# yl4579/StyleTTS2

Measured on AMD Instinct MI355X. Metric: audio-seconds/sec (RTF^-1) end-to-end, 10 s utterance batch, higher is better.
Workload: dtype f32 (convs/linears: f16 hi/lo split, 3 MFMA products, fp32 accumulate)

## Files before the change

include/st2.h:

```cpp
#ifndef ST2_H
#define ST2_H

#include <stdint.h>

#ifdef __cplusplus
extern "C" {
#endif

#define ST2_ABI_VERSION 23

int st2_abi_version(void);
const char* st2_last_error(void);
int st2_device_info(int dev, char* name, int cap);

#define ST2_STATUS_F16_RANGE 1
#define ST2_STATUS_LSTM_TIMEOUT 2
#define ST2_STATUS_DURATION_SUM 4
#define ST2_STATUS_LSTM_RECOVERED 8
int st2_status(int clear);

enum st2_prologue {
  ST2_PRO_NONE = 0,
  ST2_PRO_LEAKY = 1,
  ST2_PRO_ADAIN_LEAKY = 2,
// ... 168 lines not shown
                    int32_t B, int32_t C, int32_t N, void* stream);
int st2_mean_tokens_len(const float* x, int64_t x_bs, int32_t x_cs, float* m, int64_t m_bs,
                        int32_t B, int32_t C, int32_t N, const int32_t* len, void* stream);
int st2_time_features(float t, const float* w, int32_t H2, int32_t B, float* out, void* stream);
int st2_tokens_to_channels(const float* e, int64_t e_bs, int32_t B, int32_t N, int32_t E, float* y, int64_t y_bs,
                           int32_t y_cs, void* stream);
int st2_broadcast_cols(const float* x, int64_t x_bs, float* y, int64_t y_bs, int32_t y_cs, int32_t B, int32_t C,
                       int32_t N, void* stream);
int st2_copy_ncl(const float* x, int64_t x_bs, int32_t x_cs, float* y, int64_t y_bs, int32_t y_cs, int32_t B, int32_t C,
                 int32_t L, void* stream);

int st2_embed_tokens(const int64_t* tokens, int32_t B, int32_t N, const float* table, int32_t V, int32_t E,
                     const float* add, const float* pos, const int32_t* len, float* y, int64_t y_bs, int32_t y_cs,
                     void* stream);
int st2_mask_tail(float* x, int64_t x_bs, int32_t x_cs, int32_t B, int32_t C, int32_t L, const int32_t* len, void* stream);

int st2_duration_head(const float* x, int64_t x_bs, int32_t x_cs, const float* w, const float* bias, int32_t B,
                      int32_t K, int32_t J, int32_t N, const int32_t* len, int32_t tail, int64_t* dur, float* dsum,
                      void* stream);
int st2_expand_by_durations(const float* x, int64_t x_bs, int32_t x_cs, const int64_t* dur, int32_t B, int32_t C,
                            int32_t N, int32_t T, int32_t shift, float* y, int64_t y_bs, int32_t y_cs, void* stream);
int st2_expand_by_durations_len(const float* x, int64_t x_bs, int32_t x_cs, const int64_t* dur, int32_t B, int32_t C,
                                int32_t N, int32_t T, int32_t shift, float* y, int64_t y_bs, int32_t y_cs, const int32_t* len,
                                void* stream);

int st2_stft_frames(const float* wave, int64_t w_bs, int32_t B, int32_t L, int32_t n_win, int32_t hop, int32_t shift,
                    float* frames, int64_t f_bs, int32_t f_cs, void* stream);
int st2_power_spectrum(const float* y, int64_t y_bs, int32_t y_cs, int32_t B, int32_t K, int32_t M, float* p,
                       int64_t p_bs, int32_t p_cs, void* stream);
int st2_log_norm(float* x, int64_t n, float eps, float mean, float stdv, void* stream);
int st2_dwconv3x3s2(const float* x, int64_t x_bs, int64_t x_hs, int32_t x_cs, const float* w, const float* bias,
                    int32_t B, int32_t C, int32_t H, int32_t W, float* y, int64_t y_bs, int64_t y_hs, int32_t y_cs,
                    void* stream);
int st2_avgpool2x2(const float* x, int64_t x_bs, int64_t x_hs, int32_t x_cs, int32_t B, int32_t C, int32_t H, int32_t W,
                   float* y, int64_t y_bs, int64_t y_hs, int32_t y_cs, void* stream);

int st2_axpbypcz(const float* x, float a, const float* y, float b, const float* z, float c,
                 float* out, int64_t n, void* stream);

typedef struct st2_engine st2_engine;

typedef struct st2_model_config {
  int32_t decoder_kind;
  int32_t dim_in;
  int32_t style_dim;
  int32_t upsample_initial_channel;
  int32_t n_upsamples;  int32_t upsample_rates[4];  int32_t upsample_kernel_sizes[4];
  int32_t n_resblock_kernels;  int32_t resblock_kernel_sizes[4];  int32_t resblock_dilations[4][3];
  int32_t gen_istft_n_fft, gen_istft_hop;
  int32_t multispeaker;
  int32_t dn_layers, dn_heads, dn_head_features, dn_multiplier;
  int32_t dn_channels;
  int32_t dn_embedding;
  int32_t dn_context_features;
  int32_t dn_max_length;
  int32_t pred_hidden;
  int32_t bert_layers;
  float bert_ln_eps;
} st2_model_config;

int st2_create(const st2_model_config* cfg, st2_engine** out);
int st2_destroy(st2_engine* e);
int st2_load_weights(st2_engine* e, const char* name, const float* data, const int64_t* shape, int32_t ndim);
int st2_finalize_weights(st2_engine* e, int32_t which);

typedef struct st2_decoder_taps {
  float* encode;
  float* front;
  float* har_source;
  float* har;
  float* stage[4];
  float* spec_phase;
} st2_decoder_taps;

int64_t st2_decoder_workspace_bytes(st2_engine* e, int32_t B, int32_t T);
int st2_decoder_forward(st2_engine* e, const float* asr, const float* f0, const float* n, const float* s,
                        const float* sine_noise, const float* har_inject, int32_t B, int32_t T, float* wave,
                        void* workspace, int64_t workspace_bytes, const st2_decoder_taps* taps, void* stream);
int st2_decoder_forward_ragged(st2_engine* e, const float* asr, const float* f0, const float* n, const float* s,
                               const float* sine_noise, const float* har_inject, const int32_t* frames, int32_t B,
                               int32_t T_max, float* wave, void* workspace, int64_t workspace_bytes,
                               const st2_decoder_taps* taps, void* stream);

#define ST2_SAMPLER_TABLE_COLS 11
int st2_sampler_table(int32_t steps, double sigma_min, double sigma_max, double rho, double sigma_data, double* table,
                      double* sigma0);
int64_t st2_sampler_workspace_bytes(st2_engine* e, int32_t B, int32_t N, int32_t steps, double embedding_scale);
int st2_sampler_run(st2_engine* e, const float* noise, const float* embedding, const float* features,
                    const float* step_noise, const int32_t* lengths, int32_t B, int32_t N, int32_t steps,
                    double embedding_scale, const double* table, double sigma0, float* out, void* workspace,
                    int64_t workspace_bytes, float* step_taps, void* stream);

int64_t st2_prosody_workspace_bytes(st2_engine* e, int32_t B, int32_t N, int32_t T);
int st2_prosody_forward(st2_engine* e, const float* d_cm, const float* t_en, const int64_t* durations, const float* s,
                        int32_t B, int32_t N, int32_t T, int32_t shift, float* asr, float* f0, float* n, void* workspace,
                        int64_t workspace_bytes, void* stream);
int st2_prosody_forward_ragged(st2_engine* e, const float* d_cm, const float* t_en, const int64_t* durations,
                               const float* s, const int32_t* frames, int32_t B, int32_t N, int32_t T_max, int32_t shift,
                               float* asr, float* f0, float* n, void* workspace, int64_t workspace_bytes, void* stream);

int64_t st2_text_workspace_bytes(st2_engine* e, int32_t B, int32_t N);
int st2_text_forward(st2_engine* e, const int64_t* tokens, const int32_t* lengths, int32_t B, int32_t N, float* t_en,
                     void* workspace, int64_t workspace_bytes, void* stream);

int64_t st2_duration_workspace_bytes(st2_engine* e, int32_t B, int32_t N);
int st2_duration_forward(st2_engine* e, const float* d_en, const float* s, const int32_t* lengths, int32_t B, int32_t N,
                         int32_t tail, float* d_cm, int64_t* durations, void* workspace, int64_t workspace_bytes,
                         void* stream);

int64_t st2_bert_workspace_bytes(st2_engine* e, int32_t B, int32_t N);
int st2_bert_forward(st2_engine* e, const int64_t* tokens, const int32_t* lengths, int32_t B, int32_t N, float* hidden_cm,
                     void* workspace, int64_t workspace_bytes, void* stream);

typedef struct st2_front_args {
  const int64_t* tokens;
  const int32_t* lengths;
  const float* noise;
  const float* step_noise;
  const float* ref_s;
  const float* s_prev;
  int32_t B, N, steps;
  int32_t tail;
  double embedding_scale;
  const double* table;
  double sigma0;
  double alpha, beta, t;
  float* t_en;
  float* d_cm;
  float* s;
  float* ref;
  float* s_pred_out;
  int64_t* durations;
  int32_t carry;
} st2_front_args;
int st2_sizeof_front_args(void);
int64_t st2_front_workspace_bytes(st2_engine* e, const st2_front_args* a);
int st2_front_forward(st2_engine* e, const st2_front_args* a, void* workspace, int64_t workspace_bytes, void* stream);

int64_t st2_style_workspace_bytes(st2_engine* e, int32_t which, int32_t B, int32_t n_mels, int32_t T);
int st2_style_forward(st2_engine* e, int32_t which, const float* mel, int32_t B, int32_t n_mels, int32_t T, float* style,
                      void* workspace, int64_t workspace_bytes, void* stream);

int st2_conv_timing(int enable);
int st2_conv_timing_read(double* rows, int32_t cap_rows);

int st2_conv_tune(int mode);
int st2_conv_tune_set(int32_t ks, int32_t C_in, int32_t C_out, int32_t L_out, int32_t B, int32_t variant);
int st2_conv_tune_read(double* rows, int32_t cap_rows);

#define ST2_HEADROOM_COLS 12
int st2_debug_headroom(int enable);
int st2_debug_headroom_read(double* rows, int32_t cap_rows);

#define ST2_CALIBRATION_COLS 5
int st2_calibrate(st2_engine* e, int32_t margin_bits, int32_t* n_clamped);
int st2_calibration_read(st2_engine* e, double* rows, int32_t cap_rows);
int st2_calibration_site_name(st2_engine* e, int32_t site, char* name, int32_t cap);
int st2_calibration_write(st2_engine* e, const float* scales, int32_t n);
float st2_calibration_scale(float max_abs, int32_t margin_bits);

int st2_probe_box(char* json, int32_t cap, int32_t level);

int st2_probe_cu_health(char* json, int32_t cap, uint32_t* mask_out, int32_t mask_words, int32_t* n_excluded);

int st2_probe_mfma_stream(int32_t kind, int32_t workgroups, int32_t iters, void* stream);

int st2_stream_create_cu_mask(const uint32_t* mask, int32_t n_words, void** stream);
int st2_stream_destroy(void* stream);

enum st2_backend_slot {
  ST2_BE_CONV1D_F16S = 0, ST2_BE_CONV1D_XS, ST2_BE_ACT_SPLIT, ST2_BE_STATS_FINALIZE, ST2_BE_CONV1D_DIRECT,
  ST2_BE_PHASE_SPLIT, ST2_BE_INSTNORM_STATS, ST2_BE_COLNORM_STATS, ST2_BE_STYLE_FC, ST2_BE_CONVT_INTERLEAVE_STATS,
  ST2_BE_ADAIN_LEAKY_POOL, ST2_BE_HAR_SOURCE, ST2_BE_STFT_MAG_PHASE, ST2_BE_ISTFT, ST2_BE_ATTENTION_KEYLEN,
  ST2_BE_ADD_CHANVEC, ST2_BE_MEAN_TOKENS_LEN, ST2_BE_AXPBYPCZ, ST2_BE_TIME_FEATURES, ST2_BE_TOKENS_TO_CHANNELS,
  ST2_BE_BROADCAST_COLS, ST2_BE_COPY_NCL, ST2_BE_EXPAND_BY_DURATIONS,
  ST2_BE_LSTM_BIDIR,
  ST2_BE_COLNORM_APPLY, ST2_BE_DURATION_HEAD, ST2_BE_MASK_TAIL, ST2_BE_EMBED_TOKENS, ST2_BE_DWCONV3X3S2, ST2_BE_AVGPOOL2X2,
  ST2_BE_DEV_ALLOC,
  ST2_BE_DEV_FREE,
  ST2_BE_UPLOAD,
  ST2_BACKEND_ENTRIES_V22,
  ST2_BE_ACT_SPLIT_LEN = ST2_BACKEND_ENTRIES_V22, ST2_BE_INSTNORM_STATS_LEN, ST2_BE_STATS_FINALIZE_LEN,
  ST2_BE_CONV1D_DIRECT_LEN, ST2_BE_ADAIN_LEAKY_POOL_LEN, ST2_BE_CONVT_INTERLEAVE_STATS_LEN, ST2_BE_HAR_SOURCE_LEN,
  ST2_BE_STFT_MAG_PHASE_LEN, ST2_BE_ISTFT_LEN, ST2_BE_RAGGED_LENGTHS, ST2_BE_EXPAND_BY_DURATIONS_LEN,
  ST2_BACKEND_ENTRIES
};
int st2_debug_set_backend(void* const* table, int32_t entries);

#ifdef __cplusplus
}
#endif
#endif
```

styletts2_amd/_lib.py:

```python
import ctypes as C
import os

import torch

_HERE = os.path.dirname(os.path.abspath(__file__))
LIB_PATH = os.path.join(_HERE, "libst2_hip.so")
ABI_VERSION = 23
HEADROOM_COLS, CALIBRATION_COLS = 12, 5

f32p = C.c_void_p

PRO_NONE, PRO_LEAKY, PRO_ADAIN_LEAKY, PRO_ADAIN_SNAKE, PRO_SNAKE, PRO_COLNORM = range(6)
STATUS_F16_RANGE, STATUS_LSTM_TIMEOUT, STATUS_DURATION_SUM, STATUS_LSTM_RECOVERED = 1, 2, 4, 8
ACT_NONE, ACT_GELU, ACT_EXP_SIN, ACT_TANH, ACT_LEAKY, ACT_GELU_TANH = range(6)


class ConvDesc(C.Structure):
    _fields_ = [
        ("B", C.c_int32), ("C_in", C.c_int32), ("C_out", C.c_int32), ("L_in", C.c_int32),
        ("L_out", C.c_int32), ("ks", C.c_int32), ("dil", C.c_int32), ("pad_left", C.c_int32),
        ("x", f32p), ("x_bs", C.c_int64), ("x_cs", C.c_int32),
        ("wt", f32p), ("w_ld", C.c_int32),
        ("bias", f32p),
        ("y", f32p), ("y_bs", C.c_int64), ("y_cs", C.c_int32),
# ... 60 lines not shown
                        "adain_leaky_pool_len", "convt_interleave_stats_len", "har_source_len", "stft_mag_phase_len",
                        "istft_len", "ragged_lengths", "expand_by_durations_len"]

_SIGNATURES = {
    "st2_abi_version": (C.c_int, []),
    "st2_last_error": (C.c_char_p, []),
    "st2_device_info": (C.c_int, [C.c_int, C.c_char_p, C.c_int]),
    "st2_sizeof_conv_desc": (C.c_int, []),
    "st2_status": (C.c_int, [C.c_int]),
    "st2_conv1d": (C.c_int, [C.POINTER(ConvDesc), C.c_void_p]),
    "st2_conv1d_f16s": (C.c_int, [C.POINTER(ConvDesc), C.c_void_p]),
    "st2_conv1d_f16s_splitk_bytes": (C.c_int64, [C.POINTER(ConvDesc)]),
    "st2_conv1d_f16s_chunk": (C.c_int, [C.c_int]),
    "st2_conv1d_f16s_co_block": (C.c_int, [C.c_int]),
    "st2_conv1d_f16s_set_variant": (None, [C.c_int]),
    "st2_conv1d_xs": (C.c_int, [C.POINTER(ConvDesc), C.c_void_p]),
    "st2_act_split": (C.c_int, [f32p, C.c_int64, C.c_int32, C.c_int32, C.c_int32, C.c_int32, C.c_int32, C.c_float,
                                f32p, f32p, f32p, C.c_int64, C.c_int32, C.c_int32, f32p, C.c_float, f32p, C.c_int32,
                                C.c_int32, C.c_int32, C.c_void_p]),
    "st2_stats_finalize": (C.c_int, [f32p, C.c_int32, C.c_int32, C.c_int32, C.c_float, f32p, C.c_int32, C.c_void_p]),
    "st2_conv1d_direct": (C.c_int, [f32p, C.c_int64, C.c_int32, f32p, f32p, f32p, C.c_int64, C.c_int32,
                                    C.c_int32, C.c_int32, C.c_int32, C.c_int32, C.c_int32, C.c_int32, C.c_int32,
                                    C.c_int32, C.c_void_p]),
    "st2_phase_split": (C.c_int, [f32p, C.c_int64, C.c_int32, C.c_int32, C.c_int32, C.c_int32, C.c_int32, C.c_int32,
                                  f32p, C.c_int64, C.c_int32, C.c_int32, C.c_void_p]),
    "st2_instnorm_stats": (C.c_int, [f32p, C.c_int64, C.c_int32, C.c_int32, C.c_int32, C.c_int32, C.c_float, f32p,
                                     C.c_void_p]),
    "st2_colnorm_stats": (C.c_int, [f32p, C.c_int64, C.c_int32, C.c_int32, C.c_int32, C.c_int32, C.c_float, f32p,
                                    C.c_void_p]),
    "st2_style_fc": (C.c_int, [f32p, C.c_int32, C.c_int32, f32p, f32p, C.c_int32, C.c_int32, f32p, C.c_void_p]),
    "st2_convt_interleave": (C.c_int, [f32p, C.c_int64, C.c_int32, C.c_int32, f32p, f32p, C.c_int64, C.c_int32,
                                       f32p, C.c_int64, C.c_int32, C.c_int32, C.c_int32, C.c_int32, C.c_int32,
                                       C.c_int32, C.c_int32, C.c_void_p]),
    "st2_convt_interleave_stats": (C.c_int, [f32p, C.c_int64, C.c_int32, C.c_int32, f32p, f32p, C.c_int64, C.c_int32,
                                             f32p, C.c_int64, C.c_int32, C.c_int32, C.c_int32, C.c_int32, C.c_int32,
                                             C.c_int32, C.c_int32, f32p, C.c_int32, C.c_void_p]),
    "st2_adain_leaky_pool": (C.c_int, [f32p, C.c_int64, C.c_int32, f32p, f32p, f32p, C.c_int64, C.c_float, f32p,
                                       f32p, f32p, C.c_int64, C.c_int32, C.c_int32, C.c_int32, C.c_int32,
                                       C.c_void_p]),
    "st2_har_source": (C.c_int, [f32p, C.c_int32, C.c_int32, C.c_int32, C.c_int32, f32p, f32p, f32p, C.c_float,
                                 C.c_float, C.c_float, C.c_float, f32p, f32p, C.c_void_p]),
    "st2_stft_mag_phase": (C.c_int, [f32p, C.c_int32, C.c_int32, C.c_int32, C.c_int32, f32p, C.c_int64, C.c_int32,
                                     C.c_void_p]),
    "st2_istft": (C.c_int, [f32p, C.c_int64, C.c_int32, C.c_int32, C.c_int32, C.c_int32, C.c_int32, f32p, C.c_int64,
                            C.c_void_p]),
    "st2_attention": (C.c_int, [f32p, f32p, f32p, C.c_int64, C.c_int32, f32p, C.c_int64, C.c_int32, C.c_int32,
                                C.c_int32, C.c_int32, C.c_int32, C.c_float, C.c_void_p]),
    "st2_attention_keylen": (C.c_int, [f32p, f32p, f32p, C.c_int64, C.c_int32, f32p, C.c_int64, C.c_int32, C.c_int32,
                                       C.c_int32, C.c_int32, C.c_int32, C.c_float, C.c_void_p, C.c_void_p]),
    "st2_colnorm_apply": (C.c_int, [f32p, C.c_int64, C.c_int32, f32p, f32p, f32p, C.c_int64, C.c_int32, C.c_int32,
                                    C.c_float, C.c_void_p, f32p, C.c_int64, C.c_int32, C.c_int32, C.c_int32, C.c_int32,
                                    C.c_void_p]),
    "st2_lstm_bidir": (C.c_int, [f32p, C.c_int64, C.c_int32, f32p, C.c_void_p, C.c_int32, C.c_int32, C.c_int32, f32p,
                                 C.c_int64, C.c_int32, C.c_void_p]),
    "st2_lstm_coop_scratch_bytes": (C.c_int64, [C.c_int32]),
    "st2_lstm_coop_set_exchange": (C.c_int, [C.c_int]),
    "st2_lstm_coop_set_spin_limit": (C.c_int, [C.c_int]),
    "st2_lstm_coop_set_block": (C.c_int, [C.c_int]),
    "st2_lstm_bidir_coop": (C.c_int, [f32p, C.c_int64, C.c_int32, f32p, C.c_void_p, C.c_int32, C.c_int32, C.c_int32,
                                      f32p, C.c_int64, C.c_int32, C.c_void_p, C.c_int64, C.c_void_p]),
    "st2_lstm_bidir_coop_recovering": (C.c_int, [f32p, C.c_int64, C.c_int32, f32p, C.c_void_p, C.c_int32, C.c_int32, C.c_int32,
                                                 f32p, C.c_int64, C.c_int32, C.c_void_p, C.c_int64, C.c_void_p]),
    "st2_add_chanvec": (C.c_int, [f32p, C.c_int64, C.c_int32, f32p, C.c_int64, f32p, C.c_int64, C.c_int32,
                                  C.c_int32, C.c_int32, C.c_int32, C.c_void_p]),
    "st2_mean_tokens": (C.c_int, [f32p, C.c_int64, C.c_int32, f32p, C.c_int64, C.c_int32, C.c_int32, C.c_int32,
                                  C.c_void_p]),
    "st2_mean_tokens_len": (C.c_int, [f32p, C.c_int64, C.c_int32, f32p, C.c_int64, C.c_int32, C.c_int32, C.c_int32,
                                      C.c_void_p, C.c_void_p]),
    "st2_time_features": (C.c_int, [C.c_float, f32p, C.c_int32, C.c_int32, f32p, C.c_void_p]),
    "st2_tokens_to_channels": (C.c_int, [f32p, C.c_int64, C.c_int32, C.c_int32, C.c_int32, f32p, C.c_int64, C.c_int32,
                                         C.c_void_p]),
    "st2_broadcast_cols": (C.c_int, [f32p, C.c_int64, f32p, C.c_int64, C.c_int32, C.c_int32, C.c_int32, C.c_int32,
                                     C.c_void_p]),
    "st2_copy_ncl": (C.c_int, [f32p, C.c_int64, C.c_int32, f32p, C.c_int64, C.c_int32, C.c_int32, C.c_int32, C.c_int32,
                               C.c_void_p]),
    "st2_duration_head": (C.c_int, [f32p, C.c_int64, C.c_int32, f32p, f32p, C.c_int32, C.c_int32, C.c_int32, C.c_int32,
                                    C.c_void_p, C.c_int32, C.c_void_p, f32p, C.c_void_p]),
    "st2_expand_by_durations": (C.c_int, [f32p, C.c_int64, C.c_int32, C.c_void_p, C.c_int32, C.c_int32, C.c_int32,
                                          C.c_int32, C.c_int32, f32p, C.c_int64, C.c_int32, C.c_void_p]),
    "st2_create": (C.c_int, [C.POINTER(ModelConfig), C.POINTER(C.c_void_p)]),
    "st2_destroy": (C.c_int, [C.c_void_p]),
    "st2_load_weights": (C.c_int, [C.c_void_p, C.c_char_p, C.c_void_p, C.POINTER(C.c_int64), C.c_int32]),
    "st2_finalize_weights": (C.c_int, [C.c_void_p, C.c_int32]),
    "st2_decoder_workspace_bytes": (C.c_int64, [C.c_void_p, C.c_int32, C.c_int32]),
    "st2_decoder_forward": (C.c_int, [C.c_void_p, f32p, f32p, f32p, f32p, f32p, f32p, C.c_int32, C.c_int32, f32p,
                                      C.c_void_p, C.c_int64, C.POINTER(DecoderTaps), C.c_void_p]),
    "st2_embed_tokens": (C.c_int, [C.c_void_p, C.c_int32, C.c_int32, f32p, C.c_int32, C.c_int32, f32p, f32p, C.c_void_p, f32p,
                                   C.c_int64, C.c_int32, C.c_void_p]),
    "st2_bert_workspace_bytes": (C.c_int64, [C.c_void_p, C.c_int32, C.c_int32]),
    "st2_bert_forward": (C.c_int, [C.c_void_p, C.c_void_p, C.c_void_p, C.c_int32, C.c_int32, f32p, C.c_void_p, C.c_int64,
                                   C.c_void_p]),
    "st2_style_workspace_bytes": (C.c_int64, [C.c_void_p, C.c_int32, C.c_int32, C.c_int32, C.c_int32]),
    "st2_style_forward": (C.c_int, [C.c_void_p, C.c_int32, f32p, C.c_int32, C.c_int32, C.c_int32, f32p, C.c_void_p, C.c_int64,
                                    C.c_void_p]),
    "st2_sizeof_front_args": (C.c_int, []),
    "st2_front_workspace_bytes": (C.c_int64, [C.c_void_p, C.POINTER(FrontArgs)]),
    "st2_front_forward": (C.c_int, [C.c_void_p, C.POINTER(FrontArgs), C.c_void_p, C.c_int64, C.c_void_p]),
    "st2_text_workspace_bytes": (C.c_int64, [C.c_void_p, C.c_int32, C.c_int32]),
    "st2_text_forward": (C.c_int, [C.c_void_p, C.c_void_p, C.c_void_p, C.c_int32, C.c_int32, f32p, C.c_void_p, C.c_int64,
                                   C.c_void_p]),
    "st2_mask_tail": (C.c_int, [f32p, C.c_int64, C.c_int32, C.c_int32, C.c_int32, C.c_int32, C.c_void_p, C.c_void_p]),
    "st2_duration_workspace_bytes": (C.c_int64, [C.c_void_p, C.c_int32, C.c_int32]),
    "st2_duration_forward": (C.c_int, [C.c_void_p, f32p, f32p, C.c_void_p, C.c_int32, C.c_int32, C.c_int32, f32p,
                                       C.c_void_p, C.c_void_p, C.c_int64, C.c_void_p]),
    "st2_decoder_forward_ragged": (C.c_int, [C.c_void_p, f32p, f32p, f32p, f32p, f32p, f32p, C.c_void_p, C.c_int32,
                                             C.c_int32, f32p, C.c_void_p, C.c_int64, C.c_void_p, C.c_void_p]),
    "st2_prosody_forward_ragged": (C.c_int, [C.c_void_p, f32p, f32p, C.c_void_p, f32p, C.c_void_p, C.c_int32, C.c_int32,
                                             C.c_int32, C.c_int32, f32p, f32p, f32p, C.c_void_p, C.c_int64, C.c_void_p]),
    "st2_act_split_len": (C.c_int, [f32p, C.c_int64, C.c_int32, C.c_int32, C.c_int32, C.c_int32, C.c_int32, C.c_float,
                                    f32p, f32p, f32p, C.c_int64, C.c_int32, C.c_int32, f32p, C.c_float, f32p, C.c_int32,
                                    C.c_int32, C.c_int32, C.c_void_p, C.c_void_p]),
    "st2_stats_finalize_len": (C.c_int, [f32p, C.c_int32, C.c_int32, C.c_int32, C.c_float, f32p, C.c_int32, C.c_void_p,
                                         C.c_int32, C.c_void_p]),
    "st2_instnorm_stats_len": (C.c_int, [f32p, C.c_int64, C.c_int32, C.c_int32, C.c_int32, C.c_int32, C.c_float, f32p,
                                         C.c_void_p, C.c_void_p]),
    "st2_conv1d_direct_len": (C.c_int, [f32p, C.c_int64, C.c_int32, f32p, f32p, f32p, C.c_int64, C.c_int32, C.c_int32,
                                        C.c_int32, C.c_int32, C.c_int32, C.c_int32, C.c_int32, C.c_int32, C.c_int32,
                                        C.c_void_p, C.c_void_p, C.c_void_p]),
    "st2_convt_interleave_stats_len": (C.c_int, [f32p, C.c_int64, C.c_int32, C.c_int32, f32p, f32p, C.c_int64, C.c_int32,
                                                 f32p, C.c_int64, C.c_int32, C.c_int32, C.c_int32, C.c_int32, C.c_int32,
                                                 C.c_int32, C.c_int32, f32p, C.c_int32, C.c_void_p, C.c_void_p,
                                                 C.c_void_p]),
    "st2_adain_leaky_pool_len": (C.c_int, [f32p, C.c_int64, C.c_int32, f32p, f32p, f32p, C.c_int64, C.c_float, f32p,
                                           f32p, f32p, C.c_int64, C.c_int32, C.c_int32, C.c_int32, C.c_int32, C.c_void_p,
                                           C.c_void_p]),
    "st2_har_source_len": (C.c_int, [f32p, C.c_int32, C.c_int32, C.c_int32, C.c_int32, f32p, f32p, f32p, C.c_float,
                                     C.c_float, C.c_float, C.c_float, f32p, f32p, C.c_void_p, C.c_void_p]),
    "st2_stft_mag_phase_len": (C.c_int, [f32p, C.c_int32, C.c_int32, C.c_int32, C.c_int32, f32p, C.c_int64, C.c_int32,
                                         C.c_void_p, C.c_void_p]),
    "st2_istft_len": (C.c_int, [f32p, C.c_int64, C.c_int32, C.c_int32, C.c_int32, C.c_int32, C.c_int32, f32p, C.c_int64,
                                C.c_void_p, C.c_void_p]),
    "st2_expand_by_durations_len": (C.c_int, [f32p, C.c_int64, C.c_int32, C.c_void_p, C.c_int32, C.c_int32, C.c_int32,
                                              C.c_int32, C.c_int32, f32p, C.c_int64, C.c_int32, C.c_void_p, C.c_void_p]),
    "st2_ragged_lengths": (C.c_int, [C.c_void_p, C.c_int32, C.c_int32, C.c_int32, C.POINTER(C.c_int32), C.c_void_p,
                                     C.c_void_p]),
    "st2_prosody_workspace_bytes": (C.c_int64, [C.c_void_p, C.c_int32, C.c_int32, C.c_int32]),
    "st2_prosody_forward": (C.c_int, [C.c_void_p, f32p, f32p, C.c_void_p, f32p, C.c_int32, C.c_int32, C.c_int32, C.c_int32,
                                      f32p, f32p, f32p, C.c_void_p, C.c_int64, C.c_void_p]),
    "st2_sampler_table": (C.c_int, [C.c_int32, C.c_double, C.c_double, C.c_double, C.c_double, C.POINTER(C.c_double),
                                    C.POINTER(C.c_double)]),
    "st2_sampler_workspace_bytes": (C.c_int64, [C.c_void_p, C.c_int32, C.c_int32, C.c_int32, C.c_double]),
    "st2_sampler_run": (C.c_int, [C.c_void_p, f32p, f32p, f32p, f32p, C.c_void_p, C.c_int32, C.c_int32, C.c_int32,
                                  C.c_double, C.POINTER(C.c_double), C.c_double, f32p, C.c_void_p, C.c_int64, f32p,
                                  C.c_void_p]),
    "st2_conv_timing": (C.c_int, [C.c_int]),
    "st2_conv_timing_read": (C.c_int, [C.POINTER(C.c_double), C.c_int32]),
    "st2_conv_tune": (C.c_int, [C.c_int]),
    "st2_conv_tune_set": (C.c_int, [C.c_int32, C.c_int32, C.c_int32, C.c_int32, C.c_int32, C.c_int32]),
    "st2_conv_tune_read": (C.c_int, [C.POINTER(C.c_double), C.c_int32]),
    "st2_probe_box": (C.c_int, [C.c_char_p, C.c_int32, C.c_int32]),
    "st2_probe_cu_health": (C.c_int, [C.c_char_p, C.c_int32, C.POINTER(C.c_uint32), C.c_int32, C.POINTER(C.c_int32)]),
    "st2_probe_mfma_stream": (C.c_int, [C.c_int32, C.c_int32, C.c_int32, C.c_void_p]),
    "st2_debug_headroom": (C.c_int, [C.c_int]),
    "st2_debug_headroom_read": (C.c_int, [C.POINTER(C.c_double), C.c_int32]),
    "st2_conv1d_xs_part_cols": (C.c_int, [C.POINTER(ConvDesc)]),
    "st2_conv1d_f16s_set_splitk": (None, [C.c_int, C.c_int]),
    "st2_calibrate": (C.c_int, [C.c_void_p, C.c_int32, C.POINTER(C.c_int32)]),
    "st2_calibration_read": (C.c_int, [C.c_void_p, C.POINTER(C.c_double), C.c_int32]),
    "st2_calibration_site_name": (C.c_int, [C.c_void_p, C.c_int32, C.c_char_p, C.c_int32]),
    "st2_calibration_write": (C.c_int, [C.c_void_p, C.POINTER(C.c_float), C.c_int32]),
    "st2_calibration_scale": (C.c_float, [C.c_float, C.c_int32]),
    "st2_stream_create_cu_mask": (C.c_int, [C.POINTER(C.c_uint32), C.c_int32, C.POINTER(C.c_void_p)]),
    "st2_stream_destroy": (C.c_int, [C.c_void_p]),
    "st2_debug_set_backend": (C.c_int, [C.POINTER(C.c_void_p), C.c_int32]),
    "st2_stft_frames": (C.c_int, [f32p, C.c_int64, C.c_int32, C.c_int32, C.c_int32, C.c_int32, C.c_int32, f32p,
                                  C.c_int64, C.c_int32, C.c_void_p]),
    "st2_power_spectrum": (C.c_int, [f32p, C.c_int64, C.c_int32, C.c_int32, C.c_int32, C.c_int32, f32p, C.c_int64,
                                     C.c_int32, C.c_void_p]),
    "st2_log_norm": (C.c_int, [f32p, C.c_int64, C.c_float, C.c_float, C.c_float, C.c_void_p]),
    "st2_dwconv3x3s2": (C.c_int, [f32p, C.c_int64, C.c_int64, C.c_int32, f32p, f32p, C.c_int32, C.c_int32, C.c_int32,
                                  C.c_int32, f32p, C.c_int64, C.c_int64, C.c_int32, C.c_void_p]),
    "st2_avgpool2x2": (C.c_int, [f32p, C.c_int64, C.c_int64, C.c_int32, C.c_int32, C.c_int32, C.c_int32, C.c_int32, f32p,
                                 C.c_int64, C.c_int64, C.c_int32, C.c_void_p]),
    "st2_axpbypcz": (C.c_int, [f32p, C.c_float, f32p, C.c_float, f32p, C.c_float, f32p, C.c_int64, C.c_void_p]),
}

EXPORTS = tuple(_SIGNATURES)
_lib = None


class St2Error(RuntimeError):
    pass


def load():
    global _lib
    if _lib is not None:
        return _lib
    if not os.path.exists(LIB_PATH):
        raise St2Error("libst2_hip.so is not built (%s missing). Run `python -m styletts2_amd._build`; "
                       "there is no CPU fallback." % LIB_PATH)
    try:
        lib = C.CDLL(LIB_PATH)
    except OSError as e:
        raise St2Error("cannot load %s: %s" % (LIB_PATH, e)) from e
    for name, (res, args) in _SIGNATURES.items():
        try:
            fn = getattr(lib, name)
        except AttributeError as e:
            raise St2Error("libst2_hip.so does not export %s" % name) from e
        fn.restype = res
        fn.argtypes = args
    if lib.st2_abi_version() != ABI_VERSION:
        raise St2Error("ABI mismatch: library %d, binding %d" % (lib.st2_abi_version(), ABI_VERSION))
    if lib.st2_sizeof_conv_desc() != C.sizeof(ConvDesc):
        raise St2Error("st2_conv_desc layout mismatch: library %d B, binding %d B"
                       % (lib.st2_sizeof_conv_desc(), C.sizeof(ConvDesc)))
    if lib.st2_sizeof_front_args() != C.sizeof(FrontArgs):
        raise St2Error("st2_front_args layout mismatch: library %d B, binding %d B"
                       % (lib.st2_sizeof_front_args(), C.sizeof(FrontArgs)))
    _lib = lib
    return lib


def check(status, what):
    if status != 0:
        msg = load().st2_last_error()
        raise St2Error("%s failed: %s" % (what, msg.decode() if msg else "unknown error"))
```

styletts2_amd/csrc/st2_actsplit.hip:

```cpp
#include "st2_common.h"
#include "st2_act.h"
#include <algorithm>
#include <cstring>
#include <type_traits>
#include <vector>

namespace {

struct ActArgs {
  const float* x; int64_t x_bs; int x_cs;
  int C, L;
  float slope;
  const float* stats; const float* gamma; const float* beta; int64_t gb_bs; int gb_seg; int gamma_plus_one;
  const float* alpha;
  float x_scale;
  st2_h8* xs; int xs_cg, Lp, halo;
  const int32_t* len;
  int* status;
};

#ifndef ST2_ACT_NT
#define ST2_ACT_NT 3
#endif
template <int PRO>
__global__ __launch_bounds__(256) void act_split_kernel(const ActArgs a) {
  const int pos = blockIdx.x * 256 + threadIdx.x;
  if (pos >= a.Lp) return;
  const int cg = blockIdx.y;
  const int b = blockIdx.z;
  const int l = pos - a.halo;
  const int Lb = a.len ? min(a.len[b], a.L) : a.L;
  const bool lok = l >= 0 && l < Lb;
  const int lc = min(max(l, 0), a.L - 1);
  const float* xb = a.x + (int64_t)b * a.x_bs + lc;
  float v[8];
#pragma unroll
  for (int e = 0; e < 8; ++e) {
    const int ci = min(cg * 8 + e, a.C - 1);
#if ST2_ACT_NT & 1
    v[e] = __builtin_nontemporal_load(&xb[(int64_t)ci * a.x_cs]);
#else
    v[e] = xb[(int64_t)ci * a.x_cs];
#endif
  }
  float cmean = 0.f, crstd = 1.f;
  if constexpr (PRO == ST2_PRO_COLNORM) {
    const float* st = a.stats + ((int64_t)b * a.L + lc) * 2;
    cmean = st[0];
    crstd = st[1];
  }
  st2_h8 hi, lo;
  bool sat = false;
#pragma unroll
  for (int e = 0; e < 8; ++e) {
    const int ci = cg * 8 + e;
    const int cc = min(ci, a.C - 1);
    float u = v[e];
    if constexpr (PRO == ST2_PRO_LEAKY) {
      u = leaky(u, a.slope);
    } else if constexpr (PRO == ST2_PRO_ADAIN_LEAKY || PRO == ST2_PRO_ADAIN_SNAKE) {
      const float* st = a.stats + ((int64_t)b * a.C + cc) * 2;
      const float g = 1.0f + a.gamma[(int64_t)b * a.gb_bs + cc];
      const float bt = a.beta[(int64_t)b * a.gb_bs + cc];
      float w = (u - st[0]) * st[1];
      w = g * w + bt;
      if constexpr (PRO == ST2_PRO_ADAIN_LEAKY) {
        u = leaky(w, a.slope);
      } else {
        const float al = a.alpha[cc];
        u = snake(w, al, 1.0f / al);
      }
    } else if constexpr (PRO == ST2_PRO_SNAKE) {
      const float al = a.alpha[cc];
      u = snake(u, al, 1.0f / al);
    } else if constexpr (PRO == ST2_PRO_COLNORM) {
      const int64_t row = a.gb_seg > 0 ? (int64_t)(lc / a.gb_seg) : (int64_t)b;
      const float g0 = a.gamma[row * a.gb_bs + cc];
      const float g = a.gamma_plus_one ? 1.0f + g0 : g0;
      const float bt = a.beta[row * a.gb_bs + cc];
      const float w = (u - cmean) * crstd;
      u = w * g + bt;
    }
    u = (lok && ci < a.C) ? u * a.x_scale : 0.f;
    const float uc = st2_clamp_f16(u);
    sat |= uc != u;
    const _Float16 h = (_Float16)uc;
    hi[e] = h;
    lo[e] = (_Float16)(uc - (float)h);
  }
  if (__any(sat) && (threadIdx.x & 63) == 0) st2_raise_status(a.status, ST2_STATUS_F16_RANGE);
  const int64_t plane = (int64_t)a.xs_cg * a.Lp;
  st2_h8* dst = a.xs + ((int64_t)b * 2 * a.xs_cg + cg) * a.Lp + pos;
#if ST2_ACT_NT & 2
  __builtin_nontemporal_store(hi, &dst[0]);
  __builtin_nontemporal_store(lo, &dst[plane]);
#else
  dst[0] = hi;
  dst[plane] = lo;
#endif
}

__global__ __launch_bounds__(256) void stats_finalize_kernel(const float* __restrict__ part, int rows, int nt, int L_max,
                                                             float eps, float* __restrict__ stats, int cols,
                                                             const int32_t* __restrict__ len, int len_div) {
  const int lane = threadIdx.x & 63;
  const int row = blockIdx.x * 4 + (threadIdx.x >> 6);
  if (row >= rows) return;
  const int L = len ? min(max(len[row / len_div], 1), L_max) : L_max;
  const float2* p = reinterpret_cast<const float2*>(part) + (int64_t)row * nt;
  const float* sh = part + (int64_t)rows * nt * 2 + (int64_t)row * nt;
  const int ns = min(nt, (L + cols - 1) / cols);
  double wsum = 0.0;
  for (int i = lane; i < ns; i += 64) {
    const int n = min(cols, L - i * cols);
    wsum += (double)n * (double)sh[i] + (double)p[i].x;
  }
  wsum = st2_wave_sum(wsum);
  const double mean = __shfl(wsum, 0, 64) / (double)L;
  double m2 = 0.0;
  for (int i = lane; i < ns; i += 64) {
    const int n = min(cols, L - i * cols);
    const double s1 = (double)p[i].x, s2 = (double)p[i].y;
    const double mi = (double)sh[i] + s1 / (double)n;
    m2 += (s2 - s1 * s1 / (double)n) + (double)n * (mi - mean) * (mi - mean);
  }
  m2 = st2_wave_sum(m2);
  if (lane == 0) {
    double var = m2 / (double)L;
    if (var < 0.0) var = 0.0;
    stats[(int64_t)row * 2 + 0] = (float)mean;
    stats[(int64_t)row * 2 + 1] = (float)(1.0 / sqrt(var + (double)eps));
  }
}

struct HeadroomSums {
  unsigned max_bits, pad;
  double su2, se2, ssub;
};
__global__ __launch_bounds__(256) void xs_probe_kernel(const st2_h8* __restrict__ xs, int64_t slots_per_item, int64_t item_stride,
                                                       HeadroomSums* out) {
  const st2_h8* hi_p = xs + (int64_t)blockIdx.y * item_stride;
  const st2_h8* lo_p = hi_p + slots_per_item;
  float m = 0.f;
  double su2 = 0.0, se2 = 0.0, ssub = 0.0;
  for (int64_t i = (int64_t)blockIdx.x * 256 + threadIdx.x; i < slots_per_item; i += (int64_t)gridDim.x * 256) {
    const st2_h8 h = hi_p[i], l = lo_p[i];
#pragma unroll
    for (int e = 0; e < 8; ++e) {
      const float hf = (float)h[e], lf = (float)l[e];
      m = fmaxf(m, fabsf(hf));
      if (hf == 0.f && lf == 0.f) continue;
      const float u = hf + lf;
      const float al = fabsf(lf);
      const bool sub = al < 6.103515625e-05f;
      int ex = -14;
      if (!sub) {
        (void)frexpf(al, &ex);
        ex -= 1;
      }
      const float ulp = ldexpf(1.0f, ex - 10);
      su2 += (double)u * u;
      se2 += (double)ulp * ulp * (1.0 / 12.0);
      if (sub) ssub += (double)u * u;
    }
  }
  for (int off = 32; off > 0; off >>= 1) m = fmaxf(m, __shfl_down(m, off, 64));
  su2 = st2_wave_sum(su2);
  se2 = st2_wave_sum(se2);
  ssub = st2_wave_sum(ssub);
  if ((threadIdx.x & 63) == 0) {
    atomicMax(&out->max_bits, __float_as_uint(m));
    atomicAdd(&out->su2, su2);
    atomicAdd(&out->se2, se2);
    atomicAdd(&out->ssub, ssub);
  }
}

struct HeadroomRecord {
  int kind, pro, B, C, L;
  float x_scale;
  const void* engine;
  int site;
};
bool g_headroom = false;
std::vector<HeadroomRecord> g_hr;
HeadroomSums* g_hr_dev = nullptr;
constexpr int HR_CAP = 4096;
void* g_hr_scratch = nullptr;
size_t g_hr_scratch_bytes = 0;
thread_local const void* t_site_engine = nullptr;
thread_local int t_site = -1;

void headroom_record(int kind, const ActArgs& a, int B, hipStream_t s) {
  if ((int)g_hr.size() >= HR_CAP || !g_hr_dev) return;
  hipStreamCaptureStatus cs = hipStreamCaptureStatusNone;
  if (hipStreamIsCapturing(s, &cs) != hipSuccess || cs != hipStreamCaptureStatusNone) {
    (void)hipGetLastError();
    return;
  }
  const int64_t plane = (int64_t)a.xs_cg * a.Lp;
  hipLaunchKernelGGL(xs_probe_kernel, dim3((unsigned)std::min<int64_t>((plane + 255) / 256, 1024), B), dim3(256), 0, s, a.xs, plane,
                     2 * plane, g_hr_dev + g_hr.size());
  g_hr.push_back({kind, 0, B, a.C, a.L, a.x_scale, t_site_engine, t_site});
}

template <int PRO>
void launch_act(const ActArgs& a, int B, hipStream_t s) {
  hipLaunchKernelGGL((act_split_kernel<PRO>), dim3(st2_cdiv(a.Lp, 256), a.xs_cg, B), dim3(256), 0, s, a);
}

}

extern "C" int st2_act_split(const float* x, int64_t x_bs, int32_t x_cs, int32_t B, int32_t C, int32_t L, int32_t pro,
                             float slope, const float* stats, const float* gamma, const float* beta, int64_t gb_bs,
                             int32_t gb_seg, int32_t gamma_plus_one, const float* alpha, float x_scale, void* xs, int32_t xs_cg,
                             int32_t Lp, int32_t halo, void* stream) {
  return st2_act_split_len(x, x_bs, x_cs, B, C, L, pro, slope, stats, gamma, beta, gb_bs, gb_seg, gamma_plus_one, alpha, x_scale,
                           xs, xs_cg, Lp, halo, nullptr, stream);
}

extern "C" int st2_act_split_len(const float* x, int64_t x_bs, int32_t x_cs, int32_t B, int32_t C, int32_t L, int32_t pro,
                                 float slope, const float* stats, const float* gamma, const float* beta, int64_t gb_bs,
                                 int32_t gb_seg, int32_t gamma_plus_one, const float* alpha, float x_scale, void* xs,
                                 int32_t xs_cg, int32_t Lp, int32_t halo, const int32_t* len, void* stream) {
  ST2_REQUIRE(x && xs && B > 0 && C > 0 && L > 0, "st2_act_split: bad arguments");
  ST2_REQUIRE(B <= 65535 && xs_cg <= 65535, "st2_act_split: grid too large");
  ST2_REQUIRE(xs_cg * 8 >= C, "st2_act_split: xs_cg=%d groups cannot hold C=%d channels", xs_cg, C);
  ST2_REQUIRE(halo >= 0 && Lp >= L + halo, "st2_act_split: Lp=%d too small for L=%d + halo=%d", Lp, L, halo);
  ST2_REQUIRE((reinterpret_cast<uintptr_t>(xs) & 15) == 0, "st2_act_split: xs must be 16-byte aligned");
  ST2_REQUIRE(pro >= ST2_PRO_NONE && pro <= ST2_PRO_COLNORM, "st2_act_split: prologue %d not supported", pro);
  if (pro == ST2_PRO_ADAIN_LEAKY || pro == ST2_PRO_ADAIN_SNAKE || pro == ST2_PRO_COLNORM)
    ST2_REQUIRE(stats && gamma && beta, "st2_act_split: prologue %d needs stats/gamma/beta", pro);
  if (pro == ST2_PRO_ADAIN_SNAKE || pro == ST2_PRO_SNAKE) ST2_REQUIRE(alpha, "st2_act_split: snake needs alpha");
  ST2_REQUIRE(x_scale > 0.f, "st2_act_split: x_scale must be set");
  ST2_REQUIRE(gb_seg >= 0 && (gb_seg == 0 || pro == ST2_PRO_COLNORM), "st2_act_split: gb_seg=%d is for ST2_PRO_COLNORM", gb_seg);
  ActArgs a;
  a.x = x; a.x_bs = x_bs; a.x_cs = x_cs; a.C = C; a.L = L; a.slope = slope;
  a.stats = stats; a.gamma = gamma; a.beta = beta; a.gb_bs = gb_bs; a.gb_seg = gb_seg; a.gamma_plus_one = gamma_plus_one;
  a.alpha = alpha; a.x_scale = x_scale;
  a.xs = reinterpret_cast<st2_h8*>(xs); a.xs_cg = xs_cg; a.Lp = Lp; a.halo = halo;
  a.len = len;
  ST2_REQUIRE(!len || pro != ST2_PRO_COLNORM, "st2_act_split_len: per-row lengths are not defined for ST2_PRO_COLNORM");
  a.status = st2_status_device_ptr();
  hipStream_t s = reinterpret_cast<hipStream_t>(stream);
  switch (pro) {
    case ST2_PRO_LEAKY: launch_act<ST2_PRO_LEAKY>(a, B, s); break;
    case ST2_PRO_ADAIN_LEAKY: launch_act<ST2_PRO_ADAIN_LEAKY>(a, B, s); break;
    case ST2_PRO_ADAIN_SNAKE: launch_act<ST2_PRO_ADAIN_SNAKE>(a, B, s); break;
    case ST2_PRO_SNAKE: launch_act<ST2_PRO_SNAKE>(a, B, s); break;
    case ST2_PRO_COLNORM: launch_act<ST2_PRO_COLNORM>(a, B, s); break;
    default: launch_act<ST2_PRO_NONE>(a, B, s); break;
  }
  ST2_CHECK_LAUNCH("st2_act_split");
  if (g_headroom) {
    headroom_record(0, a, B, s);
    if (!g_hr.empty()) g_hr.back().pro = pro;
  }
  return 0;
}

int st2_headroom_of_fused_conv(const st2_conv_desc& d, hipStream_t s) {
  if (!g_headroom || !d.x) return 0;
  {
    hipStreamCaptureStatus cs = hipStreamCaptureStatusNone;
    if (hipStreamIsCapturing(s, &cs) != hipSuccess || cs != hipStreamCaptureStatusNone) {
      (void)hipGetLastError();
      return 0;
    }
  }
  const int cg = (d.C_in + 31) / 32 * 4, halo = 0;
  const int Lp = (d.L_in + 7) / 8 * 8;
  const size_t bytes = (size_t)d.B * 2 * cg * Lp * 16;
  if (bytes > g_hr_scratch_bytes) {
    if (g_hr_scratch) (void)hipFree(g_hr_scratch);
    g_hr_scratch = nullptr;
    g_hr_scratch_bytes = 0;
    if (hipMalloc(&g_hr_scratch, bytes) != hipSuccess) {
      (void)hipGetLastError();
      return 0;
    }
    g_hr_scratch_bytes = bytes;
  }
  const size_t before = g_hr.size();
  const int rc = st2_act_split(d.x, d.x_bs, d.x_cs, d.B, d.C_in, d.L_in, d.pro, d.slope, d.stats, d.gamma, d.beta, d.gb_bs, 0,
                               d.gamma_plus_one, d.alpha, d.x_scale, g_hr_scratch, cg, Lp, halo, s);
  if (rc == 0 && g_hr.size() == before + 1) g_hr.back().kind = 1;
  return rc;
}

extern "C" int st2_debug_headroom(int enable) {
  if (enable) {
    g_hr.clear();
    if (!g_hr_dev && hipMalloc(&g_hr_dev, HR_CAP * sizeof(HeadroomSums)) != hipSuccess) {
      (void)hipGetLastError();
      g_hr_dev = nullptr;
      st2_set_error("st2_debug_headroom: cannot allocate the record buffer");
      return 1;
    }
    if (hipMemset(g_hr_dev, 0, HR_CAP * sizeof(HeadroomSums)) != hipSuccess) {
      st2_set_error("st2_debug_headroom: %s", hipGetErrorString(hipGetLastError()));
      return 1;
    }
  } else if (g_hr_scratch) {
    (void)hipDeviceSynchronize();
    (void)hipFree(g_hr_scratch);
    g_hr_scratch = nullptr;
    g_hr_scratch_bytes = 0;
  }
  g_headroom = enable != 0;
  return 0;
}

void st2_headroom_set_site(const void* engine, int site) {
  t_site_engine = engine;
  t_site = site;
}

extern "C" int st2_debug_headroom_read(double* rows, int32_t cap_rows) {
  ST2_REQUIRE(!g_headroom, "st2_debug_headroom_read: stop the recording first (st2_debug_headroom(0))");
  const int n = (int)g_hr.size();
  if (!rows || n == 0) return n;
  std::vector<HeadroomSums> h(n);
  if (hipDeviceSynchronize() != hipSuccess ||
      hipMemcpy(h.data(), g_hr_dev, n * sizeof(HeadroomSums), hipMemcpyDeviceToHost) != hipSuccess) {
    st2_set_error("st2_debug_headroom_read: %s", hipGetErrorString(hipGetLastError()));
    return -1;
  }
  for (int i = 0; i < n && i < cap_rows; ++i) {
    float m;
    memcpy(&m, &h[i].max_bits, 4);
    double* r = rows + (int64_t)i * ST2_HEADROOM_COLS;
    r[0] = g_hr[i].kind; r[1] = g_hr[i].pro; r[2] = g_hr[i].B; r[3] = g_hr[i].C; r[4] = g_hr[i].L; r[5] = g_hr[i].x_scale;
    r[6] = m; r[7] = m / 65504.0;
    r[8] = h[i].su2 > 0.0 ? sqrt(h[i].se2 / h[i].su2) : 0.0;
    r[9] = h[i].su2 > 0.0 ? h[i].ssub / h[i].su2 : 0.0;
    r[10] = g_hr[i].site;
    r[11] = (double)(uintptr_t)g_hr[i].engine;
  }
  return n;
}

extern "C" int st2_stats_finalize(const float* part, int32_t rows, int32_t nt, int32_t L, float eps, float* stats, int32_t cols,
                                  void* stream) {
  return st2_stats_finalize_len(part, rows, nt, L, eps, stats, cols, nullptr, 1, stream);
}

extern "C" int st2_stats_finalize_len(const float* part, int32_t rows, int32_t nt, int32_t L, float eps, float* stats,
                                      int32_t cols, const int32_t* len, int32_t len_div, void* stream) {
  ST2_REQUIRE(part && stats && rows > 0 && nt > 0 && L > 0, "st2_stats_finalize: bad arguments");
  ST2_REQUIRE(!len || (len_div > 0 && rows % len_div == 0), "st2_stats_finalize_len: len_div=%d does not divide rows=%d", len_div,
              rows);
  ST2_REQUIRE(cols > 0 && (int64_t)nt * cols >= L, "st2_stats_finalize: %d slots of %d columns do not cover L=%d", nt, cols, L);
  ST2_REQUIRE((reinterpret_cast<uintptr_t>(part) & 7) == 0, "st2_stats_finalize: part must be 8-byte aligned");
  hipStream_t s = reinterpret_cast<hipStream_t>(stream);
  hipLaunchKernelGGL(stats_finalize_kernel, dim3(st2_cdiv(rows, 4)), dim3(256), 0, s, part, rows, nt, L, eps, stats, cols, len,
                     len_div);
  ST2_CHECK_LAUNCH("st2_stats_finalize");
  return 0;
}
```

styletts2_amd/csrc/st2_attention.hip:

```cpp
#include "st2_common.h"

typedef float f32x16 __attribute__((ext_vector_type(16)));

namespace {

constexpr int AD = 64;
constexpr int AKT = 128;
constexpr int ALD = AKT + 1;
constexpr int AQB = 128;

__global__ __launch_bounds__(256) void attention_kernel(const float* __restrict__ q, const float* __restrict__ k,
                                                        const float* __restrict__ v, int64_t bs, int cs,
                                                        float* __restrict__ o, int64_t o_bs, int o_cs, int N,
                                                        float scale, const int* __restrict__ key_len) {
  extern __shared__ __attribute__((aligned(16))) float att_smem[];
  float* ks = att_smem;
  float* vs = att_smem + AD * ALD;
  const int tid = threadIdx.x;
  const int lane = tid & 63;
  const int wave = tid >> 6;
  const int half = lane >> 5;
  const int l31 = lane & 31;
  const int h = blockIdx.y;
  const int b = blockIdx.z;
  const int q0 = blockIdx.x * AQB + wave * 32;
  const int64_t base = (int64_t)b * bs + (int64_t)h * AD * cs;
  const int nq = q0 + l31;
  const bool wave_live = q0 < N;
  const int NK = key_len ? max(1, min(key_len[b], N)) : N;

  float qr[AD / 2];
#pragma unroll
  for (int i = 0; i < AD / 2; ++i)
    qr[i] = (wave_live && nq < N) ? q[base + (int64_t)(2 * i + half) * cs + nq] : 0.f;

  f32x16 oacc[2];
#pragma unroll
  for (int t = 0; t < 2; ++t)
#pragma unroll
    for (int r = 0; r < 16; ++r) oacc[t][r] = 0.f;
  float mx = -INFINITY, den = 0.f;

  for (int c0 = 0; c0 < NK; c0 += AKT) {
    const int ct = min(AKT, NK - c0);
    __syncthreads();
    constexpr int ST_U = 8;
    static_assert((AD * AKT) % (256 * ST_U) == 0, "whole batches");
    for (int e0 = tid; e0 < AD * AKT; e0 += 256 * ST_U) {
      float kr[ST_U], vr[ST_U];
#pragma unroll
      for (int u = 0; u < ST_U; ++u) {
        const int e = e0 + u * 256;
        const int d = e / AKT, mm = e % AKT;
        const int64_t off = base + (int64_t)d * cs + c0 + min(mm, ct - 1);
        kr[u] = k[off];
        vr[u] = v[off];
      }
#pragma unroll
      for (int u = 0; u < ST_U; ++u) {
        const int e = e0 + u * 256;
        const int d = e / AKT, mm = e % AKT;
        const bool ok = mm < ct;
        ks[d * ALD + mm] = ok ? kr[u] : 0.f;
        vs[d * ALD + mm] = ok ? vr[u] : 0.f;
      }
    }
    __syncthreads();
    if (!wave_live) continue;
    for (int m0 = 0; m0 < ct; m0 += 32) {
      f32x16 s;
#pragma unroll
      for (int r = 0; r < 16; ++r) s[r] = 0.f;
#pragma unroll
      for (int i = 0; i < AD / 2; ++i) {
        const float a = ks[(2 * i + half) * ALD + m0 + l31];
        s = __builtin_amdgcn_mfma_f32_32x32x2f32(a, qr[i], s, 0, 0, 0);
      }
      float tmx = -INFINITY;
#pragma unroll
      for (int r = 0; r < 16; ++r) {
        const int key = m0 + (r & 3) + 8 * (r >> 2) + 4 * half;
        s[r] = key < ct ? s[r] * scale : -INFINITY;
        tmx = fmaxf(tmx, s[r]);
      }
      tmx = fmaxf(tmx, __shfl_xor(tmx, 32, 64));
      const float nmx = fmaxf(mx, tmx);
      const float corr = expf(mx - nmx);
      mx = nmx;
      float psum = 0.f;
#pragma unroll
      for (int r = 0; r < 16; ++r) {
        s[r] = expf(s[r] - nmx);
        psum += s[r];
      }
      den = den * corr + psum;
#pragma unroll
      for (int t = 0; t < 2; ++t)
#pragma unroll
        for (int r = 0; r < 16; ++r) oacc[t][r] *= corr;
#pragma unroll
      for (int r = 0; r < 16; ++r) {
        const int key = m0 + (r & 3) + 8 * (r >> 2) + 4 * half;
#pragma unroll
        for (int t = 0; t < 2; ++t) {
          const float a = vs[(t * 32 + l31) * ALD + key];
          oacc[t] = __builtin_amdgcn_mfma_f32_32x32x2f32(a, s[r], oacc[t], 0, 0, 0);
        }
      }
    }
  }
  if (!wave_live) return;
  den += __shfl_xor(den, 32, 64);
  if (nq < N) {
    const float inv = 1.0f / den;
    const int64_t ob = (int64_t)b * o_bs + (int64_t)h * AD * o_cs;
#pragma unroll
    for (int t = 0; t < 2; ++t)
#pragma unroll
      for (int r = 0; r < 16; ++r) {
        const int d = t * 32 + (r & 3) + 8 * (r >> 2) + 4 * half;
        o[ob + (int64_t)d * o_cs + nq] = oacc[t][r] * inv;
      }
  }
}

}

extern "C" int st2_attention(const float* q, const float* k, const float* v, int64_t bs, int32_t cs, float* o,
                             int64_t o_bs, int32_t o_cs, int32_t B, int32_t H, int32_t D, int32_t N, float scale,
                             void* stream) {
  return st2_attention_keylen(q, k, v, bs, cs, o, o_bs, o_cs, B, H, D, N, scale, nullptr, stream);
}

extern "C" int st2_attention_keylen(const float* q, const float* k, const float* v, int64_t bs, int32_t cs, float* o,
                                    int64_t o_bs, int32_t o_cs, int32_t B, int32_t H, int32_t D, int32_t N,
                                    float scale, const int32_t* key_len, void* stream) {
  ST2_REQUIRE(q && k && v && o && B > 0 && H > 0 && N > 0, "st2_attention: bad arguments");
  ST2_REQUIRE(D == AD, "st2_attention: head_features=%d unsupported (built for %d)", D, AD);
  ST2_REQUIRE(B <= 65535 && H <= 65535, "st2_attention: grid too large");
  hipStream_t s = reinterpret_cast<hipStream_t>(stream);
  constexpr size_t smem = (size_t)2 * AD * ALD * sizeof(float);
  static std::atomic<uint64_t> attr_done{0};
  st2_once_per_device(attr_done, [&] {
    (void)hipFuncSetAttribute(reinterpret_cast<const void*>(&attention_kernel),
                              hipFuncAttributeMaxDynamicSharedMemorySize, (int)smem);
  });
  hipLaunchKernelGGL(attention_kernel, dim3(st2_cdiv(N, AQB), H, B), dim3(256), smem, s, q, k, v, bs, cs, o, o_bs,
                     o_cs, N, scale, reinterpret_cast<const int*>(key_len));
  ST2_CHECK_LAUNCH("st2_attention");
  return 0;
}
```

styletts2_amd/csrc/st2_common.h:

```cpp
#pragma once
#include <hip/hip_runtime.h>
#include <stdint.h>
#include <atomic>
#include "st2.h"

void st2_set_error(const char* fmt, ...);
int st2_stream_cu_count(void* stream);
void st2_headroom_set_site(const void* engine, int site);
int* st2_status_device_ptr();

__device__ __forceinline__ void st2_raise_status(int* status, int bit) {
  if (status) __hip_atomic_store(status + (bit == ST2_STATUS_F16_RANGE ? 0 : (bit == ST2_STATUS_LSTM_TIMEOUT ? 1 :
                                           (bit == ST2_STATUS_DURATION_SUM ? 2 : 3))), bit,
                                 __ATOMIC_RELAXED, __HIP_MEMORY_SCOPE_SYSTEM);
}

#define ST2_REQUIRE(cond, ...)            \
  do {                                    \
    if (!(cond)) {                        \
      st2_set_error(__VA_ARGS__);         \
      return 1;                           \
    }                                     \
  } while (0)

#define ST2_CHECK_LAUNCH(name)                                   \
  do {                                                           \
    hipError_t e__ = hipGetLastError();                          \
    if (e__ != hipSuccess) {                                     \
      st2_set_error("%s: %s", name, hipGetErrorString(e__));     \
      return 1;                                                  \
    }                                                            \
  } while (0)

static inline int st2_cdiv(int64_t a, int64_t b) { return (int)((a + b - 1) / b); }

template <class F>
static inline void st2_once_per_device(std::atomic<uint64_t>& mask, F&& set_attr) {
  int dev = 0;
  const bool known = hipGetDevice(&dev) == hipSuccess && dev >= 0 && dev < 64;
  if (known && (mask.load(std::memory_order_acquire) & (1ull << dev))) return;
  set_attr();
  if (known) mask.fetch_or(1ull << dev, std::memory_order_release);
}

__device__ __forceinline__ double st2_wave_sum(double v) {
#pragma unroll
  for (int off = 32; off > 0; off >>= 1) v += __shfl_down(v, off, 64);
  return v;
}
__device__ __forceinline__ float st2_wave_sum(float v) {
#pragma unroll
  for (int off = 32; off > 0; off >>= 1) v += __shfl_down(v, off, 64);
  return v;
}
```

styletts2_amd/csrc/st2_engine.hip:

```cpp
#include <math.h>
#include <stdio.h>
#include <string.h>

#include <algorithm>
#include <cmath>
#include <string>
#include <unordered_map>
#include <vector>

#include "st2_common.h"

namespace {

struct Backend {
  decltype(&st2_conv1d_f16s) conv1d_f16s;
  decltype(&st2_conv1d_xs) conv1d_xs;
  decltype(&st2_act_split) act_split;
  decltype(&st2_stats_finalize) stats_finalize;
  decltype(&st2_conv1d_direct) conv1d_direct;
  decltype(&st2_phase_split) phase_split;
  decltype(&st2_instnorm_stats) instnorm_stats;
  decltype(&st2_colnorm_stats) colnorm_stats;
  decltype(&st2_style_fc) style_fc;
  decltype(&st2_convt_interleave_stats) convt_interleave_stats;
  decltype(&st2_adain_leaky_pool) adain_leaky_pool;
  decltype(&st2_har_source) har_source;
  decltype(&st2_stft_mag_phase) stft_mag_phase;
  decltype(&st2_istft) istft;
  decltype(&st2_attention_keylen) attention_keylen;
  decltype(&st2_add_chanvec) add_chanvec;
  decltype(&st2_mean_tokens_len) mean_tokens_len;
  decltype(&st2_axpbypcz) axpbypcz;
  decltype(&st2_time_features) time_features;
  decltype(&st2_tokens_to_channels) tokens_to_channels;
  decltype(&st2_broadcast_cols) broadcast_cols;
  decltype(&st2_copy_ncl) copy_ncl;
  decltype(&st2_expand_by_durations) expand_by_durations;
  int (*lstm_bidir)(const float*, int64_t, int32_t, const float*, const int32_t*, int32_t, int32_t, int32_t, float*, int64_t,
                    int32_t, void*, int64_t, void*);
  decltype(&st2_colnorm_apply) colnorm_apply;
  decltype(&st2_duration_head) duration_head;
  decltype(&st2_mask_tail) mask_tail;
  decltype(&st2_embed_tokens) embed_tokens;
  decltype(&st2_dwconv3x3s2) dwconv3x3s2;
  decltype(&st2_avgpool2x2) avgpool2x2;
  void* (*dev_alloc)(int64_t);
  void (*dev_free)(void*);
  int (*upload)(void*, const void*, int64_t);
  decltype(&st2_act_split_len) act_split_len;
  decltype(&st2_instnorm_stats_len) instnorm_stats_len;
  decltype(&st2_stats_finalize_len) stats_finalize_len;
  decltype(&st2_conv1d_direct_len) conv1d_direct_len;
  decltype(&st2_adain_leaky_pool_len) adain_leaky_pool_len;
  decltype(&st2_convt_interleave_stats_len) convt_interleave_stats_len;
  decltype(&st2_har_source_len) har_source_len;
  decltype(&st2_stft_mag_phase_len) stft_mag_phase_len;
  decltype(&st2_istft_len) istft_len;
  decltype(&st2_ragged_lengths) ragged_lengths;
  decltype(&st2_expand_by_durations_len) expand_by_durations_len;
};

void* hip_alloc(int64_t n) {
  void* p = nullptr;
  if (hipMalloc(&p, (size_t)n) != hipSuccess) {
    (void)hipGetLastError();
    return nullptr;
  }
  return p;
}
void hip_free(void* p) { (void)hipFree(p); }
int hip_upload(void* d, const void* s, int64_t n) {
  return hipMemcpy(d, s, (size_t)n, hipMemcpyHostToDevice) == hipSuccess ? 0 : 1;
}

int hip_lstm(const float* G, int64_t g_bs, int32_t g_cs, const float* whh_t, const int32_t* lengths, int32_t B, int32_t H,
             int32_t N, float* Y, int64_t y_bs, int32_t y_cs, void* scratch, int64_t scratch_bytes, void* stream) {
  if (scratch && scratch_bytes > 0) {
    if (st2_lstm_bidir_coop_recovering(G, g_bs, g_cs, whh_t, lengths, B, H, N, Y, y_bs, y_cs, scratch, scratch_bytes, stream) == 0)
      return 0;
    const char* msg = st2_last_error();
    if (!msg || !strstr(msg, "co-resident")) return 1;
  }
  return st2_lstm_bidir(G, g_bs, g_cs, whh_t, lengths, B, H, N, Y, y_bs, y_cs, stream);
}

const Backend kHipBackend = {st2_conv1d_f16s, st2_conv1d_xs, st2_act_split, st2_stats_finalize, st2_conv1d_direct,
                             st2_phase_split, st2_instnorm_stats, st2_colnorm_stats, st2_style_fc,
                             st2_convt_interleave_stats, st2_adain_leaky_pool, st2_har_source, st2_stft_mag_phase,
                             st2_istft, st2_attention_keylen, st2_add_chanvec, st2_mean_tokens_len, st2_axpbypcz,
                             st2_time_features, st2_tokens_to_channels, st2_broadcast_cols, st2_copy_ncl,
                             st2_expand_by_durations, hip_lstm, st2_colnorm_apply, st2_duration_head, st2_mask_tail,
                             st2_embed_tokens, st2_dwconv3x3s2, st2_avgpool2x2, hip_alloc, hip_free, hip_upload,
                             st2_act_split_len, st2_instnorm_stats_len, st2_stats_finalize_len, st2_conv1d_direct_len,
                             st2_adain_leaky_pool_len, st2_convt_interleave_stats_len, st2_har_source_len,
                             st2_stft_mag_phase_len, st2_istft_len, st2_ragged_lengths, st2_expand_by_durations_len};
Backend g_be = kHipBackend;

constexpr int XS_HALO = 32;
constexpr int FUSED_MAX_C = 64, FUSED_K3_MAX_C = 128;
constexpr int XS_MIN_L = 256;
constexpr int XS_MIN_C_PLAIN = 64;
constexpr int CVT_TILE = 1024;

struct Arena {
  char* base = nullptr;
  int64_t off = 0, cap = 0, peak = 0;
  bool dry = false;
  bool overflow = false;
  void* alloc(int64_t bytes) {
    off = (off + 255) & ~(int64_t)255;
    void* p = dry ? reinterpret_cast<void*>((uintptr_t)0x10000 + (uintptr_t)off) : static_cast<void*>(base + off);
    off += bytes;
    peak = std::max(peak, off);
    if (!dry && off > cap) overflow = true;
    return p;
  }
  float* f32(int64_t n) { return static_cast<float*>(alloc(n * 4)); }
};

struct View {
  float* p = nullptr;
  int64_t bs = 0;
  int cs = 0;
  int B = 0, C = 0, L = 0;
  const int32_t* len = nullptr;
  View rows(int c0, int c1) const {
    View v = *this;
    v.p = p + (int64_t)c0 * cs;
    v.C = c1 - c0;
    return v;
  }
  bool ok() const { return p != nullptr; }
  View with_len(const int32_t* l) const {
    View v = *this;
    v.len = l;
    return v;
  }
};

int pitch_of(int L) { return (L + 31) / 32 * 32; }

struct Ctx {
  Arena a;
  void* stream = nullptr;
  int rc = 0;
  bool dry = false;
};

View new_ncl(Ctx& c, int B, int C, int L, bool padded = true) {
  View v;
  v.B = B; v.C = C; v.L = L;
  v.cs = padded ? pitch_of(L) : L;
  v.bs = (int64_t)C * v.cs;
  v.p = c.a.f32((int64_t)B * v.bs);
  return v;
}

View wrap(const float* p, int B, int C, int L) {
  View v;
  v.p = const_cast<float*>(p);
  v.B = B; v.C = C; v.L = L; v.cs = L; v.bs = (int64_t)C * L;
  return v;
}

#define RUN(c, expr)                                   \
  do {                                                 \
    if (!(c).dry && (c).rc == 0 && !(c).a.overflow) {  \
      (c).rc = (expr);                                 \
    }                                                  \
  } while (0)

struct HostTensor {
  std::vector<int64_t> shape;
  std::vector<float> data;
  int64_t numel() const { return (int64_t)data.size(); }
};

struct ConvSite {
  std::string name;
  int C_in = 0, C_out = 0, ks = 0;
};

struct Blob {
  std::vector<char> host;
  std::vector<ConvSite> sites;
  int64_t add(const void* src, int64_t bytes) {
    int64_t off = ((int64_t)host.size() + 255) & ~(int64_t)255;
    host.resize((size_t)(off + bytes));
    if (src) memcpy(host.data() + off, src, (size_t)bytes);
    return off;
  }
  int64_t add_f32(const std::vector<float>& v) { return add(v.data(), (int64_t)v.size() * 4); }
};

struct SplitW {
  int64_t wq = -1, row_scale = -1;
  int C_in = 0, C_out = 0, ks = 0, co_pad = 0, cin_pad = 0;
  int site = -1;
};

struct PConv {
  SplitW w;
  int64_t bias = -1;
  int c_out = 0, ks = 0;
};

struct PResBlock1 {
  int channels = 0, ks = 0;
  int dil[3] = {1, 3, 5};
  PConv c1[3], c2[3];
  int64_t a1[3] = {-1, -1, -1}, a2[3] = {-1, -1, -1};
  int ad1[3] = {0, 0, 0}, ad2[3] = {0, 0, 0};
};

struct PAdainResBlk {
  int dim_in = 0, dim_out = 0;
  bool upsample = false, learned_sc = false;
  PConv conv1, conv2, sc;
  int64_t pool_w = -1, pool_b = -1;
  int n1 = 0, n2 = 0;
};

int f16s_chunk(int ks) { return ks <= 3 ? 32 : 16; }
int f16s_co_block(int C_out) { return C_out > 64 ? 128 : (C_out > 32 ? 64 : 32); }

SplitW pack_split(Blob& blob, const std::string& name, const float* w, int C_out, int C_in, int ks) {
  SplitW r;
  r.C_in = C_in; r.C_out = C_out; r.ks = ks;
  r.site = (int)blob.sites.size();
  blob.sites.push_back({name, C_in, C_out, ks});
  const int cb = f16s_chunk(ks), rb = f16s_co_block(C_out);
  r.cin_pad = (C_in + cb - 1) / cb * cb;
  r.co_pad = (C_out + rb - 1) / rb * rb;
  const int n16 = r.cin_pad / 16;
  std::vector<_Float16> q((size_t)n16 * ks * 2 * r.co_pad * 16, (_Float16)0.0f);
  std::vector<float> rs((size_t)r.co_pad, 1.0f);
  for (int co = 0; co < C_out; ++co) {
    const float* wr = w + (int64_t)co * C_in * ks;
    float amax = 0.f;
    for (int i = 0; i < C_in * ks; ++i) amax = std::max(amax, fabsf(wr[i]));
    float scale = 1.0f;
    if (amax > 0.f) {
      int e = 0;
      (void)frexpf(amax, &e);
      scale = ldexpf(1.0f, std::min(14 - e, 126));
    }
    rs[co] = 1.0f / scale;
    for (int ci = 0; ci < C_in; ++ci)
      for (int t = 0; t < ks; ++t) {
        const float v = wr[(int64_t)ci * ks + t] * scale;
        const _Float16 hi = (_Float16)v;
        const _Float16 lo = (_Float16)(v - (float)hi);
        const int i16 = ci / 16, kg = (ci % 16) / 8, e8 = ci % 8;
        const size_t base = ((((size_t)i16 * ks + t) * 2 + kg) * r.co_pad + co) * 16;
        q[base + e8] = hi;
        q[base + 8 + e8] = lo;
      }
  }
  r.wq = blob.add(q.data(), (int64_t)q.size() * 2);
  r.row_scale = blob.add_f32(rs);
  return r;
}

std::vector<float> polyphase_convt(const float* w, int C_in, int C_out, int stride) {
  const int K = 2 * stride;
  std::vector<float> wp((size_t)stride * C_out * C_in * 2);
  for (int r = 0; r < stride; ++r)
    for (int co = 0; co < C_out; ++co)
      for (int ci = 0; ci < C_in; ++ci) {
        const size_t o = (((size_t)r * C_out + co) * C_in + ci) * 2;
        wp[o + 0] = w[((int64_t)ci * C_out + co) * K + r + stride];
        wp[o + 1] = w[((int64_t)ci * C_out + co) * K + r];
      }
  return wp;
}

std::vector<float> polyphase_strided(const float* w, int C_out, int C_in, int stride) {
  const int K = 2 * stride;
  std::vector<float> wp((size_t)C_out * C_in * stride * 2);
  for (int co = 0; co < C_out; ++co)
    for (int ci = 0; ci < C_in; ++ci)
      for (int r = 0; r < stride; ++r)
        for (int j = 0; j < 2; ++j)
          wp[(((size_t)co * C_in * stride) + (size_t)ci * stride + r) * 2 + j] = w[((int64_t)co * C_in + ci) * K + j * stride + r];
  return wp;
}

struct PGenerator {
  int64_t lin_w = -1, lin_b = -1;
  std::vector<SplitW> noise_wt;
  std::vector<int> noise_stride;
  std::vector<int64_t> noise_b;
  std::vector<PResBlock1> noise_res, resblocks;
  std::vector<SplitW> ups_wt;
  std::vector<int64_t> ups_b;
  PConv post;
  std::vector<int64_t> alphas;
  std::vector<int> channels;
};

// ... 266 lines not shown
  for (int i = 0; i < 4; ++i) {
    const std::string p = D + "decode." + std::to_string(i);
    const bool up = i == 3;
    d.decode[i] = pack_adain_resblk(pk, p, 1024 + 2 + 64, up ? 512 : 1024, up);
    d.decode[i].n1 = bank.add(pk, p + ".norm1", 1024 + 2 + 64);
    d.decode[i].n2 = bank.add(pk, p + ".norm2", up ? 512 : 1024);
  }
  d.f0_w = pk.vec(D + "F0_conv.weight", 3); d.f0_b = pk.vec(D + "F0_conv.bias", 1);
  d.n_w = pk.vec(D + "N_conv.weight", 3);   d.n_b = pk.vec(D + "N_conv.bias", 1);
  d.asr_res = pk.conv(D + "asr_res.0", true, 64, Cin, 1);

  PGenerator& g = d.gen;
  const std::string G = D + "generator.";
  const int nu = cfg.n_upsamples, nk = cfg.n_resblock_kernels;
  const bool ist = cfg.decoder_kind == 0;
  const int c0 = cfg.upsample_initial_channel;
  g.lin_w = pk.vec(G + "m_source.l_linear.weight", 9);
  g.lin_b = pk.vec(G + "m_source.l_linear.bias", 1);
  static const int dil135[3] = {1, 3, 5};
  for (int i = 0; i < nu; ++i) g.channels.push_back(c0 >> (i + 1));
  for (int i = 0; i < nu; ++i) {
    const bool last = i + 1 == nu;
    PResBlock1 r = pack_resblock1(pk, G + "noise_res." + std::to_string(i), g.channels[i], last ? 11 : 7, dil135);
    g.noise_res.push_back(r);
  }
  for (int i = 0; i < nu; ++i)
    for (int k = 0; k < nk; ++k) {
      PResBlock1 r = pack_resblock1(pk, G + "resblocks." + std::to_string(i * nk + k), g.channels[i],
                                    cfg.resblock_kernel_sizes[k], cfg.resblock_dilations[k]);
      g.resblocks.push_back(r);
    }
  for (auto* list : {&g.noise_res, &g.resblocks}) {
    const std::string pre = list == &g.noise_res ? G + "noise_res." : G + "resblocks.";
    for (size_t i = 0; i < list->size(); ++i) {
      PResBlock1& r = (*list)[i];
      for (int j = 0; j < 3; ++j) r.ad1[j] = bank.add(pk, pre + std::to_string(i) + ".adain1." + std::to_string(j), r.channels);
      for (int j = 0; j < 3; ++j) r.ad2[j] = bank.add(pk, pre + std::to_string(i) + ".adain2." + std::to_string(j), r.channels);
    }
  }
  if (pk.ok) bank.pack(pk, sty, &d.bank_wt, &d.bank_b);
  d.J = bank.J;
  for (int i = 0; i < nu; ++i) {
    const int stride_f0 = i + 1 < nu ? prod_from(cfg.upsample_rates, i + 1, nu) : 1;
    const HostTensor* w = pk.get(G + "noise_convs." + std::to_string(i) + ".weight", {g.channels[i], -1, -1});
    g.noise_stride.push_back(stride_f0);
    if (w && w->shape.size() != 3) { pk.fail(G + "noise_convs." + std::to_string(i) + ".weight must be 3-D"); w = nullptr; }
    if (w) {
      const int C_out = (int)w->shape[0], C_in = (int)w->shape[1], K = (int)w->shape[2];
      if (stride_f0 > 1) {
        if (K != 2 * stride_f0) { *err = "noise_convs kernel must be 2*stride"; return 1; }
        std::vector<float> wp = polyphase_strided(w->data.data(), C_out, C_in, stride_f0);
        g.noise_wt.push_back(pack_split(blob, G + "noise_convs." + std::to_string(i) + ".weight", wp.data(), C_out, C_in * stride_f0, 2));
      } else {
        g.noise_wt.push_back(pack_split(blob, G + "noise_convs." + std::to_string(i) + ".weight", w->data.data(), C_out, C_in, K));
      }
    } else {
      g.noise_wt.push_back(SplitW());
    }
    g.noise_b.push_back(pk.vec(G + "noise_convs." + std::to_string(i) + ".bias", g.channels[i]));
  }
  for (int i = 0; i < nu; ++i) {
    const int u = cfg.upsample_rates[i];
    const HostTensor* w = pk.get(G + "ups." + std::to_string(i) + ".weight", {c0 >> i, c0 >> (i + 1), -1});
    if (w && w->shape.size() != 3) { pk.fail(G + "ups." + std::to_string(i) + ".weight must be 3-D"); w = nullptr; }
    if (w) {
      const int C_in = (int)w->shape[0], C_out = (int)w->shape[1], K = (int)w->shape[2];
      if (K != 2 * u) { *err = "ups kernel must be 2*stride"; return 1; }
      std::vector<float> wp = polyphase_convt(w->data.data(), C_in, C_out, u);
      g.ups_wt.push_back(pack_split(blob, G + "ups." + std::to_string(i) + ".weight", wp.data(), u * C_out, C_in, 2));
    } else {
      g.ups_wt.push_back(SplitW());
    }
    g.ups_b.push_back(pk.vec(G + "ups." + std::to_string(i) + ".bias", c0 >> (i + 1)));
  }
  g.post = pk.conv(G + "conv_post", true, ist ? cfg.gen_istft_n_fft + 2 : 1, g.channels.back(), 7);
  if (!ist)
    for (int i = 0; i <= nu; ++i) g.alphas.push_back(pk.vec(G + "alphas." + std::to_string(i), c0 >> i));
  if (!pk.ok) {
    *err = "decoder weights (missing or malformed): " + pk.missing;
    return 1;
  }
  d.ready = true;
  e.dec = d;
  return 0;
}

int pack_denoiser(st2_engine& e, Blob& blob, std::string* err) {
  const st2_model_config& cfg = e.cfg;
  Packer pk{e, blob};
  PDenoiser d;
  const std::string N = "denoiser.";
  d.features = cfg.dn_channels + cfg.dn_embedding;
  d.time_w = pk.vec(N + "to_time.0.0.weights");
  d.time_lin = pk.lin_t(N + "to_time.0.1.weight"); d.time_b = pk.vec(N + "to_time.0.1.bias");
  d.map0 = pk.lin_t(N + "to_mapping.0.weight");    d.map0_b = pk.vec(N + "to_mapping.0.bias");
  d.map2 = pk.lin_t(N + "to_mapping.2.weight");    d.map2_b = pk.vec(N + "to_mapping.2.bias");
  const int F = d.features;
  if (cfg.multispeaker) {
    d.feat = pk.lin_t(N + "to_features.0.weight"); d.feat_b = pk.vec(N + "to_features.0.bias");
    const int Fc = cfg.dn_context_features, J = cfg.dn_layers * 4 * F;
    std::vector<float> wt((size_t)Fc * J), b((size_t)J);
    int off = 0;
    for (int i = 0; i < cfg.dn_layers; ++i)
      for (const char* nm : {".attention.norm", ".attention.norm_context"}) {
        const HostTensor* w = pk.get(N + "blocks." + std::to_string(i) + nm + ".fc.weight", {2 * F, Fc});
        const HostTensor* bb = pk.get(N + "blocks." + std::to_string(i) + nm + ".fc.bias", {2 * F});
        if (w && bb)
          for (int j = 0; j < 2 * F; ++j) {
            for (int k = 0; k < Fc; ++k) wt[(size_t)k * J + off + j] = w->data[(size_t)j * Fc + k];
            b[(size_t)off + j] = bb->data[(size_t)j];
          }
        off += 2 * F;
      }
    d.ada_wt = blob.add_f32(wt);
    d.ada_b = blob.add_f32(b);
  }
  for (int i = 0; i < cfg.dn_layers; ++i) {
    const std::string B = N + "blocks." + std::to_string(i);
    PBlock b;
    if (!cfg.multispeaker) {
      b.n_w = pk.vec(B + ".attention.norm.weight", F);          b.n_b = pk.vec(B + ".attention.norm.bias", F);
      b.nc_w = pk.vec(B + ".attention.norm_context.weight", F); b.nc_b = pk.vec(B + ".attention.norm_context.bias", F);
    }
    const int HD = cfg.dn_heads * cfg.dn_head_features, FM = F * cfg.dn_multiplier;
    b.q = pk.conv_w(B + ".attention.to_q.weight", HD, F, 1);
    b.kv = pk.conv_w(B + ".attention.to_kv.weight", 2 * HD, F, 1);
    b.o = pk.conv_w(B + ".attention.attention.to_out.weight", F, HD, 1); b.o_b = pk.vec(B + ".attention.attention.to_out.bias", F);
    b.f1 = pk.conv_w(B + ".feed_forward.0.weight", FM, F, 1);            b.f1_b = pk.vec(B + ".feed_forward.0.bias", FM);
    b.f1_out = b.f1.C_out;
    b.f2 = pk.conv_w(B + ".feed_forward.2.weight", F, FM, 1);            b.f2_b = pk.vec(B + ".feed_forward.2.bias", F);
    d.blocks.push_back(b);
  }
  {
    const HostTensor* w = pk.get(N + "to_out.1.weight", {cfg.dn_channels, F, 1});
    if (w) {
      const int O = (int)w->shape[0], I = (int)w->shape[1];
      std::vector<float> v((size_t)O * I);
      for (int o = 0; o < O; ++o)
        for (int i = 0; i < I; ++i) v[(size_t)i * O + o] = w->data[(size_t)o * I + i];
      d.out_t = blob.add_f32(v);
    }
    d.out_b = pk.vec(N + "to_out.1.bias", cfg.dn_channels);
  }
  d.fixed = pk.vec(N + "fixed_embedding.embedding.weight", (int64_t)cfg.dn_max_length * cfg.dn_embedding);
  if (!pk.ok) {
    *err = "denoiser weights (missing or malformed): " + pk.missing;
    return 1;
  }
  d.ready = true;
  e.dn = d;
  return 0;
}

struct ConvOpt {
  int dil = 1, pad_left = 0;
  const float* bias = nullptr;
  int pro = ST2_PRO_NONE;
  float slope = 0.f;
  const float* stats = nullptr;
  const float* gamma = nullptr;
  const float* beta = nullptr;
  int64_t gb_bs = 0;
  int gb_seg = 0;
  int gamma_plus_one = 0;
  const float* alpha = nullptr;
  View res; int res_shift = 0;
  View res2;
  float div = 1.0f;
  int act = ST2_ACT_NONE, act_split = 0;
  float act_slope = 0.f;
  float* stats_out = nullptr;
};

float x_scale_for(int pro) {
  return (pro == ST2_PRO_ADAIN_LEAKY || pro == ST2_PRO_ADAIN_SNAKE || pro == ST2_PRO_COLNORM) ? 8.0f : 1.0f;
}
int xs_row_slots(int L) { return XS_HALO + (std::max(L, 1) + 1 + 511) / 512 * 512 + 96; }

void finalize_stats(Ctx& c, float* part, const View& y, int nt, float* stats, int cols) {
  if (y.len)
    RUN(c, g_be.stats_finalize_len(part, y.B * y.C, nt, y.L, 1e-5f, stats, cols, y.len, y.C, c.stream));
  else
    RUN(c, g_be.stats_finalize(part, y.B * y.C, nt, y.L, 1e-5f, stats, cols, c.stream));
}

void instnorm_stats(Ctx& c, const View& x, float* stats) {
  if (x.len)
    RUN(c, g_be.instnorm_stats_len(x.p, x.bs, x.cs, x.B, x.C, x.L, 1e-5f, stats, x.len, c.stream));
  else
    RUN(c, g_be.instnorm_stats(x.p, x.bs, x.cs, x.B, x.C, x.L, 1e-5f, stats, c.stream));
}

void conv(Ctx& c, const st2_engine& e, const View& x, const SplitW& w, const View& y, const ConvOpt& o) {
  st2_conv_desc d;
  memset(&d, 0, sizeof(d));
  d.B = x.B; d.C_in = x.C; d.C_out = y.C; d.L_in = x.L; d.L_out = y.L; d.ks = w.ks; d.dil = o.dil; d.pad_left = o.pad_left;
  d.wq = e.P<const void>(w.wq); d.wq_co_pad = w.co_pad; d.wq_cin_pad = w.cin_pad;
  d.x_scale = e.x_scale(w.site, x_scale_for(o.pro));
  d.out_scale = 1.0f / d.x_scale;
  if (!c.dry) st2_headroom_set_site(&e, w.site);
  d.w_row_scale = e.F(w.row_scale);
  d.bias = o.bias;
  d.y = y.p; d.y_bs = y.bs; d.y_cs = y.cs;
  if (o.res.ok()) { d.res = o.res.p; d.res_bs = o.res.bs; d.res_cs = o.res.cs; d.res_shift = o.res_shift; }
  if (o.res2.ok()) { d.res2 = o.res2.p; d.res2_bs = o.res2.bs; d.res2_cs = o.res2.cs; }
  d.div = o.div;
  d.act = o.act; d.act_split = o.act_split; d.act_slope = o.act_slope;
  d.x_len = x.len; d.y_len = y.len;
  if (w.C_in != x.C || w.C_out != y.C) {
    if (c.rc == 0) { st2_set_error("engine: conv weight is %d->%d, call has %d->%d", w.C_in, w.C_out, x.C, y.C); c.rc = 1; }
    return;
  }
  const bool prefer_fused = o.pro != ST2_PRO_NONE && (x.C <= FUSED_MAX_C || (w.ks <= 3 && x.C <= FUSED_K3_MAX_C));
  const bool use_xs = o.pad_left <= XS_HALO && x.L >= XS_MIN_L && (o.pro != ST2_PRO_NONE || x.C >= XS_MIN_C_PLAIN) &&
                      !prefer_fused;
  const int64_t mark = c.a.off;
  if (use_xs) {
    const int cg = (x.C + 31) / 32 * 32 / 8;
    const int Lp = xs_row_slots(x.L);
    void* xs = c.a.alloc((int64_t)x.B * 2 * cg * Lp * 16);
    if (x.len)
      RUN(c, g_be.act_split_len(x.p, x.bs, x.cs, x.B, x.C, x.L, o.pro, o.slope, o.stats, o.gamma, o.beta, o.gb_bs, o.gb_seg,
                                o.gamma_plus_one, o.alpha, d.x_scale, xs, cg, Lp, XS_HALO, x.len, c.stream));
    else
      RUN(c, g_be.act_split(x.p, x.bs, x.cs, x.B, x.C, x.L, o.pro, o.slope, o.stats, o.gamma, o.beta, o.gb_bs, o.gb_seg,
                            o.gamma_plus_one, o.alpha, d.x_scale, xs, cg, Lp, XS_HALO, c.stream));
    d.xs = xs; d.xs_cg = cg; d.xs_lp = Lp; d.xs_halo = XS_HALO;
    float* part = nullptr;
    int nt = 0;
    if (o.stats_out) {
      const int pc = st2_conv1d_xs_part_cols(&d);
      nt = (y.L + pc - 1) / pc;
      part = c.a.f32((int64_t)y.B * y.C * nt * 3);
      d.part = part; d.part_nt = nt; d.part_cols = pc;
    }
    RUN(c, g_be.conv1d_xs(&d, c.stream));
    if (o.stats_out) finalize_stats(c, part, y, nt, o.stats_out, d.part_cols);
  } else {
    if (o.gb_seg > 0) {
      if (c.rc == 0) { st2_set_error("engine: a per-segment affine (gb_seg) needs the act_split + xs path"); c.rc = 1; }
      return;
    }
    d.x = x.p; d.x_bs = x.bs; d.x_cs = x.cs;
    d.pro = o.pro; d.slope = o.slope;
    d.stats = o.stats; d.gamma = o.gamma; d.beta = o.beta; d.gb_bs = o.gb_bs; d.gamma_plus_one = o.gamma_plus_one;
    d.alpha = o.alpha;
    float* part = nullptr;
    int nt = 0;
    if (o.stats_out) {
      nt = (y.L + 127) / 128;
      part = c.a.f32((int64_t)y.B * y.C * nt * 3);
      d.part = part; d.part_nt = nt;
    } else {
      const int64_t skb = st2_conv1d_f16s_splitk_bytes(&d);
      if (skb > 0) {
        d.splitk_ws = c.a.alloc(skb);
        d.splitk_ws_bytes = skb;
      }
    }
    RUN(c, g_be.conv1d_f16s(&d, c.stream));
    if (o.stats_out) finalize_stats(c, part, y, nt, o.stats_out, 128);
  }
  c.a.off = mark;
  if (!c.dry) st2_headroom_set_site(nullptr, -1);
}

float* new_stats(Ctx& c, int B, int C) { return c.a.f32((int64_t)B * C * 2); }

int64_t ragged_table_bytes(int B, int n) { return ((int64_t)n * B * 4 + 255) & ~(int64_t)255; }

#include "st2_plan_decoder.inc"
#include "st2_plan_sampler.inc"
#include "st2_plan_prosody.inc"
#include "st2_plan_duration.inc"
#include "st2_plan_text.inc"
#include "st2_plan_front.inc"
#include "st2_plan_style.inc"

}

extern "C" int st2_debug_set_backend(void* const* table, int32_t entries) {
  if (!table) {
    g_be = kHipBackend;
    return 0;
  }
  ST2_REQUIRE(entries == ST2_BACKEND_ENTRIES || entries == ST2_BACKEND_ENTRIES_V22,
              "st2_debug_set_backend: %d entries, expected %d (or %d: the slots before ABI v23)", entries,
              (int)ST2_BACKEND_ENTRIES, (int)ST2_BACKEND_ENTRIES_V22);
  for (int i = 0; i < entries; ++i) ST2_REQUIRE(table[i] != nullptr, "st2_debug_set_backend: entry %d is null", i);
#define SLOT(field, slot) g_be.field = reinterpret_cast<decltype(g_be.field)>(table[slot])
  SLOT(conv1d_f16s, ST2_BE_CONV1D_F16S); SLOT(conv1d_xs, ST2_BE_CONV1D_XS); SLOT(act_split, ST2_BE_ACT_SPLIT);
  SLOT(stats_finalize, ST2_BE_STATS_FINALIZE); SLOT(conv1d_direct, ST2_BE_CONV1D_DIRECT);
  SLOT(phase_split, ST2_BE_PHASE_SPLIT); SLOT(instnorm_stats, ST2_BE_INSTNORM_STATS);
  SLOT(colnorm_stats, ST2_BE_COLNORM_STATS); SLOT(style_fc, ST2_BE_STYLE_FC);
  SLOT(convt_interleave_stats, ST2_BE_CONVT_INTERLEAVE_STATS); SLOT(adain_leaky_pool, ST2_BE_ADAIN_LEAKY_POOL);
  SLOT(har_source, ST2_BE_HAR_SOURCE); SLOT(stft_mag_phase, ST2_BE_STFT_MAG_PHASE); SLOT(istft, ST2_BE_ISTFT);
  SLOT(attention_keylen, ST2_BE_ATTENTION_KEYLEN); SLOT(add_chanvec, ST2_BE_ADD_CHANVEC);
  SLOT(mean_tokens_len, ST2_BE_MEAN_TOKENS_LEN); SLOT(axpbypcz, ST2_BE_AXPBYPCZ);
  SLOT(time_features, ST2_BE_TIME_FEATURES); SLOT(tokens_to_channels, ST2_BE_TOKENS_TO_CHANNELS);
  SLOT(broadcast_cols, ST2_BE_BROADCAST_COLS); SLOT(copy_ncl, ST2_BE_COPY_NCL);
  SLOT(expand_by_durations, ST2_BE_EXPAND_BY_DURATIONS); SLOT(lstm_bidir, ST2_BE_LSTM_BIDIR);
  SLOT(colnorm_apply, ST2_BE_COLNORM_APPLY); SLOT(duration_head, ST2_BE_DURATION_HEAD); SLOT(mask_tail, ST2_BE_MASK_TAIL);
  SLOT(embed_tokens, ST2_BE_EMBED_TOKENS); SLOT(dwconv3x3s2, ST2_BE_DWCONV3X3S2); SLOT(avgpool2x2, ST2_BE_AVGPOOL2X2);
  SLOT(dev_alloc, ST2_BE_DEV_ALLOC); SLOT(dev_free, ST2_BE_DEV_FREE); SLOT(upload, ST2_BE_UPLOAD);
  const Backend& h = kHipBackend;
  g_be.act_split_len = h.act_split_len; g_be.instnorm_stats_len = h.instnorm_stats_len;
  g_be.stats_finalize_len = h.stats_finalize_len; g_be.conv1d_direct_len = h.conv1d_direct_len;
  g_be.adain_leaky_pool_len = h.adain_leaky_pool_len; g_be.convt_interleave_stats_len = h.convt_interleave_stats_len;
  g_be.har_source_len = h.har_source_len; g_be.stft_mag_phase_len = h.stft_mag_phase_len; g_be.istft_len = h.istft_len;
  g_be.ragged_lengths = h.ragged_lengths; g_be.expand_by_durations_len = h.expand_by_durations_len;
  if (entries == ST2_BACKEND_ENTRIES) {
    SLOT(act_split_len, ST2_BE_ACT_SPLIT_LEN); SLOT(instnorm_stats_len, ST2_BE_INSTNORM_STATS_LEN);
    SLOT(stats_finalize_len, ST2_BE_STATS_FINALIZE_LEN); SLOT(conv1d_direct_len, ST2_BE_CONV1D_DIRECT_LEN);
    SLOT(adain_leaky_pool_len, ST2_BE_ADAIN_LEAKY_POOL_LEN);
    SLOT(convt_interleave_stats_len, ST2_BE_CONVT_INTERLEAVE_STATS_LEN); SLOT(har_source_len, ST2_BE_HAR_SOURCE_LEN);
    SLOT(stft_mag_phase_len, ST2_BE_STFT_MAG_PHASE_LEN); SLOT(istft_len, ST2_BE_ISTFT_LEN);
    SLOT(ragged_lengths, ST2_BE_RAGGED_LENGTHS); SLOT(expand_by_durations_len, ST2_BE_EXPAND_BY_DURATIONS_LEN);
  }
#undef SLOT
  return 0;
}

extern "C" int st2_create(const st2_model_config* cfg, st2_engine** out) {
  ST2_REQUIRE(cfg && out, "st2_create: null argument");
  ST2_REQUIRE(check_cfg(*cfg), "st2_create: invalid model configuration");
  st2_engine* e = new (std::nothrow) st2_engine();
  ST2_REQUIRE(e, "st2_create: out of memory");
  e->cfg = *cfg;
  *out = e;
  return 0;
}

extern "C" int st2_destroy(st2_engine* e) {
  if (!e) return 0;
  if (e->wbase) g_be.dev_free(e->wbase);
  delete e;
  return 0;
}

extern "C" int st2_load_weights(st2_engine* e, const char* name, const float* data, const int64_t* shape, int32_t ndim) {
  ST2_REQUIRE(e && name && data && shape && ndim >= 0 && ndim <= 4, "st2_load_weights: bad arguments");
  HostTensor t;
  int64_t n = 1;
  for (int i = 0; i < ndim; ++i) {
    ST2_REQUIRE(shape[i] > 0, "st2_load_weights: %s has a non-positive dimension", name);
    t.shape.push_back(shape[i]);
    n *= shape[i];
  }
  t.data.assign(data, data + n);
  e->host[std::string(name)] = std::move(t);
  return 0;
}

struct PackedSet {
  PDecoder dec;
  PDenoiser dn;
  PPredictor pred;
  PDuration dur;
  PText text;
  PBert bert;
  PStyleEnc style[2];
  int64_t zeros = -1;
  std::vector<ConvSite> sites;
  std::vector<float> site_scale, site_seen;
};

namespace {
PackedSet packed_of(const st2_engine& e) {
  PackedSet p;
  p.sites = e.sites; p.site_scale = e.site_scale; p.site_seen = e.site_seen;
  p.dec = e.dec; p.dn = e.dn; p.pred = e.pred; p.dur = e.dur; p.text = e.text; p.bert = e.bert;
  p.style[0] = e.style[0]; p.style[1] = e.style[1]; p.zeros = e.zeros;
  return p;
}
void commit_packed(st2_engine& e, const PackedSet& p) {
  e.sites = p.sites; e.site_scale = p.site_scale; e.site_seen = p.site_seen;
  e.dec = p.dec; e.dn = p.dn; e.pred = p.pred; e.dur = p.dur; e.text = p.text; e.bert = p.bert;
  e.style[0] = p.style[0]; e.style[1] = p.style[1]; e.zeros = p.zeros;
}
}

extern "C" int st2_finalize_weights(st2_engine* e, int32_t which) {
  ST2_REQUIRE(e && (which & 63) != 0, "st2_finalize_weights: bad arguments");
  const PackedSet saved = packed_of(*e);
  Blob blob;
  std::string err;
  auto pack_all = [&]() -> int {
    if (which & 1) { if (pack_decoder(*e, blob, &err)) return 1; }
    else e->dec.ready = false;
    if (which & 2) { if (pack_denoiser(*e, blob, &err)) return 1; }
    else e->dn.ready = false;
    if (which & 4) { if (pack_predictor(*e, blob, &err)) return 1; }
    else e->pred.ready = false;
    e->dur.ready = false;
    if ((which & 4) && e->host.count("predictor.text_encoder.lstms.0.weight_ih_l0"))
      if (pack_duration(*e, blob, &err)) return 1;
    if (which & 8) { if (pack_text(*e, blob, &err)) return 1; }
    else e->text.ready = false;
    if (which & 16) { if (pack_bert(*e, blob, &err)) return 1; }
    else e->bert.ready = false;
    e->style[0].ready = e->style[1].ready = false;
    if (which & 32) {
      int found = 0;
      for (int k = 0; k < 2; ++k)
        if (e->host.count(std::string(k == 0 ? "style_encoder." : "predictor_encoder.") + "shared.0.weight")) {
          if (pack_style(*e, blob, k, &err)) return 1;
          ++found;
        }
      if (!found) { err = "no style_encoder.* / predictor_encoder.* parameters were loaded"; return 1; }
      e->zeros = blob.add_f32(std::vector<float>((size_t)STYLE_ZEROS, 0.0f));
    }
    return 0;
  };
  if (pack_all() != 0) {
    commit_packed(*e, saved);
    st2_set_error("st2_finalize_weights: %s", err.c_str());
    return 1;
  }
  const int64_t bytes = (int64_t)blob.host.size();
  void* p = g_be.dev_alloc(bytes);
  if (!p) {
    commit_packed(*e, saved);
    st2_set_error("st2_finalize_weights: device allocation of %lld B failed", (long long)bytes);
    return 1;
  }
  if (g_be.upload(p, blob.host.data(), bytes) != 0) {
    g_be.dev_free(p);
    commit_packed(*e, saved);
    st2_set_error("st2_finalize_weights: upload failed");
    return 1;
  }
  if (e->wbase) g_be.dev_free(e->wbase);
  e->wbase = static_cast<char*>(p);
  e->wbytes = bytes;
  e->sites = blob.sites;
  e->site_scale.assign(e->sites.size(), 0.f);
  e->site_seen.assign(e->sites.size(), 0.f);
  return 0;
}

extern "C" float st2_calibration_scale(float max_abs, int32_t margin_bits) {
  if (!(max_abs > 0.f) || !std::isfinite(max_abs)) return 0.f;
  margin_bits = std::min(std::max(margin_bits, 0), 10);
  int ex = 0;
  (void)frexpf(max_abs, &ex);
  return ldexpf(1.0f, std::min(std::max(16 - margin_bits - ex, -60), 60));
}

extern "C" int st2_calibrate(st2_engine* e, int32_t margin_bits, int32_t* n_clamped) {
  if (!e) { st2_set_error("st2_calibrate: null engine"); return -1; }
  const int n = st2_debug_headroom_read(nullptr, 0);
  if (n < 0) return -1;
  std::vector<double> rows((size_t)std::max(n, 1) * ST2_HEADROOM_COLS);
  if (n > 0 && st2_debug_headroom_read(rows.data(), n) < 0) return -1;
  const double me = (double)(uintptr_t)e;
  std::vector<float> seen(e->sites.size(), 0.f);
  std::vector<char> free_range(e->sites.size(), 0);
  int clamped = 0;
  for (int i = 0; i < n; ++i) {
    const double* r = rows.data() + (size_t)i * ST2_HEADROOM_COLS;
    const int site = (int)r[10];
    if (r[11] != me || site < 0 || site >= (int)seen.size() || !(r[5] > 0.0)) continue;
    if (r[6] >= 65504.0) ++clamped;
    seen[(size_t)site] = std::max(seen[(size_t)site], (float)(r[6] / r[5]));
    if (x_scale_for((int)r[1]) == 1.0f) free_range[(size_t)site] = 1;
  }
  e->site_scale.resize(e->sites.size(), 0.f);
  e->site_seen.resize(e->sites.size(), 0.f);
  int set = 0;
  for (size_t i = 0; i < seen.size(); ++i) {
    if (!(seen[i] > 0.f)) continue;
    e->site_seen[i] = std::max(e->site_seen[i], seen[i]);
    e->site_scale[i] = st2_calibration_scale(e->site_seen[i], margin_bits + (free_range[i] ? 2 : 0));
    ++set;
  }
  if (n_clamped) *n_clamped = clamped;
  return set;
}

extern "C" int st2_calibration_read(st2_engine* e, double* rows, int32_t cap_rows) {
  if (!e) return -1;
  const int n = (int)e->sites.size();
  for (int i = 0; rows && i < n && i < cap_rows; ++i) {
    double* r = rows + (size_t)i * ST2_CALIBRATION_COLS;
    r[0] = e->sites[(size_t)i].C_in; r[1] = e->sites[(size_t)i].C_out; r[2] = e->sites[(size_t)i].ks;
    r[3] = i < (int)e->site_scale.size() ? e->site_scale[(size_t)i] : 0.0;
    r[4] = i < (int)e->site_seen.size() ? e->site_seen[(size_t)i] : 0.0;
  }
  return n;
}

extern "C" int st2_calibration_site_name(st2_engine* e, int32_t site, char* name, int32_t cap) {
  ST2_REQUIRE(e && name && cap > 0 && site >= 0 && site < (int)e->sites.size(), "st2_calibration_site_name: bad arguments");
  snprintf(name, (size_t)cap, "%s", e->sites[(size_t)site].name.c_str());
  return 0;
}

extern "C" int st2_calibration_write(st2_engine* e, const float* scales, int32_t n) {
  ST2_REQUIRE(e && (n == 0 || scales) && n >= 0, "st2_calibration_write: bad arguments");
  if (n == 0) {
    e->site_scale.assign(e->sites.size(), 0.f);
    e->site_seen.assign(e->sites.size(), 0.f);
    return 0;
  }
  ST2_REQUIRE(n == (int)e->sites.size(), "st2_calibration_write: %d scales for %d conv sites (another model layout?)", n,
              (int)e->sites.size());
  for (int i = 0; i < n; ++i) {
    int ex = 0;
    const bool pow2 = scales[i] == 0.f || (scales[i] > 0.f && std::isfinite(scales[i]) && frexpf(scales[i], &ex) == 0.5f);
    ST2_REQUIRE(pow2, "st2_calibration_write: scale %d = %g is not a power of two (0 = by rule)", i, (double)scales[i]);
  }
  e->site_scale.assign(scales, scales + n);
  e->site_seen.assign(e->sites.size(), 0.f);
  return 0;
}

extern "C" int64_t st2_decoder_workspace_bytes(st2_engine* e, int32_t B, int32_t T) {
  if (!e || !e->dec.ready || B <= 0 || T <= 0) return -1;
  Ctx c;
  c.dry = true;
  c.a.dry = true;
  decoder_plan(c, *e, nullptr, nullptr, nullptr, nullptr, nullptr, nullptr, B, T, nullptr, nullptr);
  return c.a.peak + 256 + ragged_table_bytes(B, 16);
}

extern "C" int st2_decoder_forward(st2_engine* e, const float* asr, const float* f0, const float* n, const float* s,
                                   const float* sine_noise, const float* har_inject, int32_t B, int32_t T, float* wave,
                                   void* workspace, int64_t workspace_bytes, const st2_decoder_taps* taps, void* stream) {
  ST2_REQUIRE(e && e->dec.ready, "st2_decoder_forward: decoder weights not finalized");
  ST2_REQUIRE(asr && f0 && n && s && wave && workspace && B > 0 && T > 0, "st2_decoder_forward: bad arguments");
  ST2_REQUIRE(sine_noise || har_inject, "st2_decoder_forward: sine_noise (or har_inject) is required");
  ST2_REQUIRE((reinterpret_cast<uintptr_t>(workspace) & 255) == 0, "st2_decoder_forward: workspace must be 256-byte aligned");
  Ctx c;
  c.stream = stream;
  c.a.base = static_cast<char*>(workspace);
  c.a.cap = workspace_bytes;
  const int rc = decoder_plan(c, *e, asr, f0, n, s, sine_noise, har_inject, B, T, wave, taps);
  ST2_REQUIRE(!c.a.overflow, "st2_decoder_forward: workspace of %lld B is too small (need %lld B, see "
              "st2_decoder_workspace_bytes)", (long long)workspace_bytes, (long long)c.a.peak);
  return rc;
}

extern "C" int st2_decoder_forward_ragged(st2_engine* e, const float* asr, const float* f0, const float* n, const float* s,
                                          const float* sine_noise, const float* har_inject, const int32_t* frames, int32_t B,
                                          int32_t T_max, float* wave, void* workspace, int64_t workspace_bytes,
                                          const st2_decoder_taps* taps, void* stream) {
  ST2_REQUIRE(frames, "st2_decoder_forward_ragged: frames (int32 [B] on the device) is required");
  ST2_REQUIRE(B > 0 && T_max > 0, "st2_decoder_forward_ragged: bad geometry B=%d T_max=%d", B, T_max);
  ST2_REQUIRE(e && e->dec.ready, "st2_decoder_forward_ragged: decoder weights not finalized");
  ST2_REQUIRE(asr && f0 && n && s && wave && workspace, "st2_decoder_forward_ragged: bad arguments");
  ST2_REQUIRE(sine_noise || har_inject, "st2_decoder_forward_ragged: sine_noise (or har_inject) is required");
  ST2_REQUIRE(!taps, "st2_decoder_forward_ragged: taps are not supported (pass NULL)");
  ST2_REQUIRE((reinterpret_cast<uintptr_t>(workspace) & 255) == 0,
              "st2_decoder_forward_ragged: workspace must be 256-byte aligned");
  Ctx c;
  c.stream = stream;
  c.a.base = static_cast<char*>(workspace);
  c.a.cap = workspace_bytes;
  const int rc = decoder_plan(c, *e, asr, f0, n, s, sine_noise, har_inject, B, T_max, wave, taps, frames);
  ST2_REQUIRE(!c.a.overflow, "st2_decoder_forward_ragged: workspace of %lld B is too small (need %lld B, see "
              "st2_decoder_workspace_bytes)", (long long)workspace_bytes, (long long)c.a.peak);
  return rc;
}

extern "C" int64_t st2_text_workspace_bytes(st2_engine* e, int32_t B, int32_t N) {
  if (!e || !e->text.ready || B <= 0 || N <= 0) return -1;
  Ctx c;
  c.dry = true;
  c.a.dry = true;
  text_plan(c, *e, nullptr, nullptr, B, N, nullptr);
  return c.a.peak + 256;
}

extern "C" int st2_text_forward(st2_engine* e, const int64_t* tokens, const int32_t* lengths, int32_t B, int32_t N,
                                float* t_en, void* workspace, int64_t workspace_bytes, void* stream) {
  ST2_REQUIRE(e && e->text.ready, "st2_text_forward: text-encoder weights not finalized");
  ST2_REQUIRE(tokens && t_en && workspace && B > 0 && N > 0, "st2_text_forward: bad arguments");
  ST2_REQUIRE((reinterpret_cast<uintptr_t>(workspace) & 255) == 0, "st2_text_forward: workspace must be 256-byte aligned");
  Ctx c;
  c.stream = stream;
  c.a.base = static_cast<char*>(workspace);
  c.a.cap = workspace_bytes;
  const int rc = text_plan(c, *e, tokens, lengths, B, N, t_en);
  ST2_REQUIRE(!c.a.overflow, "st2_text_forward: workspace of %lld B is too small (need %lld B, see st2_text_workspace_bytes)",
              (long long)workspace_bytes, (long long)c.a.peak);
  return rc;
}

extern "C" int64_t st2_bert_workspace_bytes(st2_engine* e, int32_t B, int32_t N) {
  if (!e || !e->bert.ready || B <= 0 || N <= 0) return -1;
  Ctx c;
  c.dry = true;
  c.a.dry = true;
  bert_plan(c, *e, nullptr, nullptr, B, N);
  return c.a.peak + 256;
}

extern "C" int st2_bert_forward(st2_engine* e, const int64_t* tokens, const int32_t* lengths, int32_t B, int32_t N,
                                float* hidden_cm, void* workspace, int64_t workspace_bytes, void* stream) {
  ST2_REQUIRE(e && e->bert.ready, "st2_bert_forward: PL-BERT weights not finalized");
  ST2_REQUIRE(tokens && hidden_cm && workspace && B > 0 && N > 0, "st2_bert_forward: bad arguments");
  ST2_REQUIRE(N <= e->bert.P, "st2_bert_forward: N=%d tokens exceed the %d rows of the position table", N, e->bert.P);
  ST2_REQUIRE((reinterpret_cast<uintptr_t>(workspace) & 255) == 0, "st2_bert_forward: workspace must be 256-byte aligned");
  Ctx c;
  c.stream = stream;
  c.a.base = static_cast<char*>(workspace);
  c.a.cap = workspace_bytes;
  View X = bert_plan(c, *e, tokens, lengths, B, N);
  View dst = wrap(hidden_cm, B, e->bert.H, N);
  RUN(c, g_be.copy_ncl(X.p, X.bs, X.cs, dst.p, dst.bs, dst.cs, B, e->bert.H, N, c.stream));
  ST2_REQUIRE(!c.a.overflow, "st2_bert_forward: workspace of %lld B is too small (need %lld B, see st2_bert_workspace_bytes)",
              (long long)workspace_bytes, (long long)c.a.peak);
  return c.rc;
}

extern "C" int64_t st2_style_workspace_bytes(st2_engine* e, int32_t which, int32_t B, int32_t n_mels, int32_t T) {
  if (!e || which < 0 || which > 1 || !e->style[which].ready || B <= 0 || n_mels != 80 || T < 80) return -1;
  Ctx c;
  c.dry = true;
  c.a.dry = true;
  style_plan(c, *e, e->style[which], nullptr, B, n_mels, T, nullptr);
  return c.a.peak + 256;
}

extern "C" int st2_style_forward(st2_engine* e, int32_t which, const float* mel, int32_t B, int32_t n_mels, int32_t T,
                                 float* style, void* workspace, int64_t workspace_bytes, void* stream) {
  ST2_REQUIRE(e && which >= 0 && which <= 1 && e->style[which].ready, "st2_style_forward: style-encoder weights not finalized");
  ST2_REQUIRE(mel && style && workspace && B > 0, "st2_style_forward: bad arguments");
  ST2_REQUIRE(n_mels == 80 && T >= 80, "st2_style_forward: needs an 80-bin mel of >= 80 frames (four halvings, then the 5x5 "
              "valid conv), got %d x %d", n_mels, T);
  ST2_REQUIRE((reinterpret_cast<uintptr_t>(workspace) & 255) == 0, "st2_style_forward: workspace must be 256-byte aligned");
  Ctx c;
  c.stream = stream;
  c.a.base = static_cast<char*>(workspace);
  c.a.cap = workspace_bytes;
  const int rc = style_plan(c, *e, e->style[which], mel, B, n_mels, T, style);
  ST2_REQUIRE(!c.a.overflow, "st2_style_forward: workspace of %lld B is too small (need %lld B, see st2_style_workspace_bytes)",
              (long long)workspace_bytes, (long long)c.a.peak);
  return rc;
}

extern "C" int st2_sizeof_front_args(void) { return (int)sizeof(st2_front_args); }

namespace {
const char* front_ready(const st2_engine* e) {
  if (!e) return "null engine";
  if (!e->text.ready) return "text-encoder weights not finalized (bit 3)";
  if (!e->bert.ready || !e->bert.has_enc) return "PL-BERT / bert_encoder weights not finalized (bit 4)";
  if (!e->dn.ready) return "denoiser weights not finalized (bit 1)";
  if (!e->dur.ready) return "duration-encoder weights not finalized (bit 2)";
  if (e->cfg.dn_channels != 2 * e->cfg.style_dim) return "cfg.dn_channels != 2 * cfg.style_dim";
  if (e->cfg.dn_embedding != e->bert.H) return "cfg.dn_embedding != PL-BERT hidden size";
  if (e->bert.enc.C_out != e->cfg.pred_hidden) return "bert_encoder width != cfg.pred_hidden";
  return nullptr;
}
}

extern "C" int64_t st2_front_workspace_bytes(st2_engine* e, const st2_front_args* a) {
  if (front_ready(e) || !a || a->B <= 0 || a->N <= 0 || a->steps < 2) return -1;
  Ctx c;
  c.dry = true;
  c.a.dry = true;
  std::vector<double> table((size_t)(a->steps - 1) * ST2_SAMPLER_TABLE_COLS, 0.0);
  static const float dummy = 0.f;
  static int64_t dummy_dur;
  st2_front_args q = *a;
  q.table = table.data();
  if (e->cfg.multispeaker) q.ref_s = &dummy;
  if (a->durations) q.durations = &dummy_dur;
  front_plan(c, *e, q);
  return c.a.peak + 256;
}

extern "C" int st2_front_forward(st2_engine* e, const st2_front_args* a, void* workspace, int64_t workspace_bytes,
                                 void* stream) {
  const char* why = front_ready(e);
  ST2_REQUIRE(!why, "st2_front_forward: %s", why);
  ST2_REQUIRE(a && a->tokens && a->noise && a->step_noise && a->table && a->t_en && a->d_cm && a->s && a->ref && workspace &&
              a->B > 0 && a->N > 0 && a->steps >= 2 && a->tail >= 0, "st2_front_forward: bad arguments");
  ST2_REQUIRE(!e->cfg.multispeaker || a->ref_s, "st2_front_forward: the multispeaker denoiser needs ref_s");
  ST2_REQUIRE(a->N <= e->bert.P && a->N <= e->cfg.dn_max_length && a->N <= 512,
              "st2_front_forward: N=%d tokens exceed the position / fixed-embedding tables", a->N);
  ST2_REQUIRE((reinterpret_cast<uintptr_t>(workspace) & 255) == 0, "st2_front_forward: workspace must be 256-byte aligned");
  Ctx c;
  c.stream = stream;
  c.a.base = static_cast<char*>(workspace);
  c.a.cap = workspace_bytes;
  const int rc = front_plan(c, *e, *a);
  ST2_REQUIRE(!c.a.overflow, "st2_front_forward: workspace of %lld B is too small (need %lld B, see "
              "st2_front_workspace_bytes)", (long long)workspace_bytes, (long long)c.a.peak);
  return rc;
}

extern "C" int64_t st2_duration_workspace_bytes(st2_engine* e, int32_t B, int32_t N) {
  if (!e || !e->dur.ready || B <= 0 || N <= 0) return -1;
  Ctx c;
  c.dry = true;
  c.a.dry = true;
  static int64_t dummy_dur;
  duration_plan(c, *e, wrap(nullptr, B, e->cfg.pred_hidden, N), nullptr, nullptr, B, N, 0, nullptr, &dummy_dur);
  return c.a.peak + 256;
}

extern "C" int st2_duration_forward(st2_engine* e, const float* d_en, const float* s, const int32_t* lengths, int32_t B,
                                    int32_t N, int32_t tail, float* d_cm, int64_t* durations, void* workspace,
                                    int64_t workspace_bytes, void* stream) {
  ST2_REQUIRE(e && e->dur.ready, "st2_duration_forward: duration-encoder weights not finalized");
  ST2_REQUIRE(d_en && s && d_cm && workspace && B > 0 && N > 0 && tail >= 0, "st2_duration_forward: bad arguments");
  ST2_REQUIRE(N <= 512, "st2_duration_forward: N=%d tokens exceed the 512 of PL-BERT's position table", N);
  ST2_REQUIRE((reinterpret_cast<uintptr_t>(workspace) & 255) == 0, "st2_duration_forward: workspace must be 256-byte aligned");
  Ctx c;
  c.stream = stream;
  c.a.base = static_cast<char*>(workspace);
  c.a.cap = workspace_bytes;
  const int rc = duration_plan(c, *e, wrap(d_en, B, e->cfg.pred_hidden, N), s, lengths, B, N, tail, d_cm, durations);
  ST2_REQUIRE(!c.a.overflow, "st2_duration_forward: workspace of %lld B is too small (need %lld B, see "
              "st2_duration_workspace_bytes)", (long long)workspace_bytes, (long long)c.a.peak);
  return rc;
}

extern "C" int64_t st2_prosody_workspace_bytes(st2_engine* e, int32_t B, int32_t N, int32_t T) {
  if (!e || !e->pred.ready || B <= 0 || N <= 0 || T <= 0) return -1;
  Ctx c;
  c.dry = true;
  c.a.dry = true;
  prosody_plan(c, *e, nullptr, nullptr, nullptr, nullptr, B, N, T, 0, nullptr, nullptr, nullptr);
  return c.a.peak + 256 + ragged_table_bytes(B, 2);
}

extern "C" int st2_prosody_forward(st2_engine* e, const float* d_cm, const float* t_en, const int64_t* durations,
                                   const float* s, int32_t B, int32_t N, int32_t T, int32_t shift, float* asr, float* f0,
                                   float* n, void* workspace, int64_t workspace_bytes, void* stream) {
  ST2_REQUIRE(e && e->pred.ready, "st2_prosody_forward: predictor weights not finalized");
  ST2_REQUIRE(d_cm && t_en && durations && s && asr && f0 && n && workspace && B > 0 && N > 0 && T > 0,
              "st2_prosody_forward: bad arguments");
  ST2_REQUIRE(N <= 512, "st2_prosody_forward: N=%d tokens exceed the 512 of PL-BERT's position table", N);
  ST2_REQUIRE((reinterpret_cast<uintptr_t>(workspace) & 255) == 0, "st2_prosody_forward: workspace must be 256-byte aligned");
  Ctx c;
  c.stream = stream;
  c.a.base = static_cast<char*>(workspace);
  c.a.cap = workspace_bytes;
  const int rc = prosody_plan(c, *e, d_cm, t_en, durations, s, B, N, T, shift, asr, f0, n);
  ST2_REQUIRE(!c.a.overflow, "st2_prosody_forward: workspace of %lld B is too small (need %lld B, see "
              "st2_prosody_workspace_bytes)", (long long)workspace_bytes, (long long)c.a.peak);
  return rc;
}

extern "C" int st2_prosody_forward_ragged(st2_engine* e, const float* d_cm, const float* t_en, const int64_t* durations,
                                          const float* s, const int32_t* frames, int32_t B, int32_t N, int32_t T_max,
                                          int32_t shift, float* asr, float* f0, float* n, void* workspace,
                                          int64_t workspace_bytes, void* stream) {
  ST2_REQUIRE(frames, "st2_prosody_forward_ragged: frames (int32 [B] on the device) is required");
  ST2_REQUIRE(B > 0 && N > 0 && T_max > 0, "st2_prosody_forward_ragged: bad geometry B=%d N=%d T_max=%d", B, N, T_max);
  ST2_REQUIRE(e && e->pred.ready, "st2_prosody_forward_ragged: predictor weights not finalized");
  ST2_REQUIRE(d_cm && t_en && durations && s && asr && f0 && n && workspace, "st2_prosody_forward_ragged: bad arguments");
  ST2_REQUIRE(N <= 512, "st2_prosody_forward_ragged: N=%d tokens exceed the 512 of PL-BERT's position table", N);
  ST2_REQUIRE((reinterpret_cast<uintptr_t>(workspace) & 255) == 0,
              "st2_prosody_forward_ragged: workspace must be 256-byte aligned");
  Ctx c;
  c.stream = stream;
  c.a.base = static_cast<char*>(workspace);
  c.a.cap = workspace_bytes;
  const int rc = prosody_plan(c, *e, d_cm, t_en, durations, s, B, N, T_max, shift, asr, f0, n, frames);
  ST2_REQUIRE(!c.a.overflow, "st2_prosody_forward_ragged: workspace of %lld B is too small (need %lld B, see "
              "st2_prosody_workspace_bytes)", (long long)workspace_bytes, (long long)c.a.peak);
  return rc;
}

extern "C" int st2_sampler_table(int32_t steps, double sigma_min, double sigma_max, double rho, double sigma_data,
                                 double* table, double* sigma0) {
  ST2_REQUIRE(steps >= 2 && table && sigma0 && rho > 0, "st2_sampler_table: bad arguments");
  std::vector<float> sig((size_t)steps + 1, 0.f);
  const double rinv = 1.0 / rho;
  for (int i = 0; i < steps; ++i) {
    const float frac = (float)i / (float)(steps - 1);
    const float base = (float)pow(sigma_max, rinv) + frac * (float)(pow(sigma_min, rinv) - pow(sigma_max, rinv));
    sig[(size_t)i] = powf(base, (float)rho);
  }
  *sigma0 = (double)sig[0];
  auto weights = [&](double sigma, double* w4) {
    const float s = (float)sigma, sd = (float)sigma_data;
    w4[3] = (double)(logf(s) * 0.25f);
    w4[0] = (double)((sd * sd) / (s * s + sd * sd));
    w4[1] = (double)(s * sd * (1.0f / sqrtf(sd * sd + s * s)));
    w4[2] = (double)(1.0f / sqrtf(s * s + sd * sd));
  };
  for (int i = 0; i + 1 < steps; ++i) {
    double* row = table + (int64_t)i * ST2_SAMPLER_TABLE_COLS;
    const double s = (double)sig[(size_t)i], sn = (double)sig[(size_t)i + 1];
    const double up = sqrt(sn * sn * (s * s - sn * sn) / (s * s));
    const double down = sqrt(sn * sn - up * up);
    const double mid = (s + down) / 2.0;
    weights(s, row + 0);
    weights(mid, row + 4);
    row[8] = (mid - s) / s;
    row[9] = (down - s) / mid;
    row[10] = up;
  }
  return 0;
}

extern "C" int64_t st2_sampler_workspace_bytes(st2_engine* e, int32_t B, int32_t N, int32_t steps, double embedding_scale) {
  if (!e || !e->dn.ready || B <= 0 || N <= 0 || steps < 2) return -1;
  Ctx c;
  c.dry = true;
  c.a.dry = true;
  std::vector<double> table((size_t)(steps - 1) * ST2_SAMPLER_TABLE_COLS, 0.0);
  static const float dummy = 0.f;
  sampler_plan(c, *e, nullptr, nullptr, nullptr, &dummy, nullptr, nullptr, B, N, steps, embedding_scale, table.data(), 1.0, nullptr,
               nullptr);
  return c.a.peak + 256;
}

extern "C" int st2_sampler_run(st2_engine* e, const float* noise, const float* embedding, const float* features,
                               const float* step_noise, const int32_t* lengths, int32_t B, int32_t N, int32_t steps,
                               double embedding_scale, const double* table, double sigma0, float* out, void* workspace,
                               int64_t workspace_bytes, float* step_taps, void* stream) {
  ST2_REQUIRE(e && e->dn.ready, "st2_sampler_run: denoiser weights not finalized");
  ST2_REQUIRE(noise && embedding && step_noise && table && out && workspace && B > 0 && N > 0 && steps >= 2,
              "st2_sampler_run: bad arguments");
  ST2_REQUIRE(N <= e->cfg.dn_max_length, "st2_sampler_run: N=%d exceeds the fixed-embedding length %d", N,
              e->cfg.dn_max_length);
  ST2_REQUIRE((reinterpret_cast<uintptr_t>(workspace) & 255) == 0, "st2_sampler_run: workspace must be 256-byte aligned");
  Ctx c;
  c.stream = stream;
  c.a.base = static_cast<char*>(workspace);
  c.a.cap = workspace_bytes;
  const int rc = sampler_plan(c, *e, noise, embedding, nullptr, features, step_noise, lengths, B, N, steps, embedding_scale, table,
                              sigma0, out, step_taps);
  ST2_REQUIRE(!c.a.overflow, "st2_sampler_run: workspace of %lld B is too small (need %lld B, see "
              "st2_sampler_workspace_bytes)", (long long)workspace_bytes, (long long)c.a.peak);
  return rc;
}
```

styletts2_amd/csrc/st2_plan_front.inc:

```

int pack_bert(st2_engine& e, Blob& blob, std::string* err) {
  Packer pk{e, blob};
  PBert b;
  const std::string R = "bert.", L = R + "encoder.albert_layer_groups.0.albert_layers.0.";
  const HostTensor* w = pk.get(R + "embeddings.word_embeddings.weight");
  const HostTensor* p = pk.get(R + "embeddings.position_embeddings.weight");
  const HostTensor* tt = pk.get(R + "embeddings.token_type_embeddings.weight");
  const HostTensor* q = pk.get(L + "attention.query.weight");
  const HostTensor* k = pk.get(L + "attention.key.weight");
  const HostTensor* v = pk.get(L + "attention.value.weight");
  const HostTensor* qb = pk.get(L + "attention.query.bias");
  const HostTensor* kb = pk.get(L + "attention.key.bias");
  const HostTensor* vb = pk.get(L + "attention.value.bias");
  if (!pk.ok || w->shape.size() != 2 || p->shape.size() != 2 || tt->shape.size() != 2 || q->shape.size() != 2) {
    *err = "PL-BERT parameter missing or malformed: " + pk.missing;
    return 1;
  }
  b.V = (int)w->shape[0]; b.E = (int)w->shape[1]; b.P = (int)p->shape[0]; b.H = (int)q->shape[0];
  if (p->shape[1] != b.E || tt->shape[1] != b.E || q->shape[1] != b.H || k->numel() != q->numel() ||
      v->numel() != q->numel() || qb->numel() != b.H || kb->numel() != b.H || vb->numel() != b.H || b.H % 64 != 0 ||
      e.cfg.bert_layers <= 0) {
    *err = "PL-BERT: inconsistent shapes (64-wide heads, one shared layer) or cfg.bert_layers == 0";
    return 1;
  }
  b.word = blob.add_f32(w->data);
  b.pos = blob.add_f32(p->data);
  b.tok0 = blob.add_f32(std::vector<float>(tt->data.begin(), tt->data.begin() + b.E));
  b.eln_w = pk.vec(R + "embeddings.LayerNorm.weight", b.E); b.eln_b = pk.vec(R + "embeddings.LayerNorm.bias", b.E);
  b.map = pk.conv_w(R + "encoder.embedding_hidden_mapping_in.weight", b.H, b.E, 1);
  b.map_b = pk.vec(R + "encoder.embedding_hidden_mapping_in.bias", b.H);
  {
    const size_t HH = (size_t)b.H * b.H;
    std::vector<float> cat(3 * HH), bias((size_t)3 * b.H);
    std::copy(q->data.begin(), q->data.end(), cat.begin());
    std::copy(k->data.begin(), k->data.end(), cat.begin() + HH);
    std::copy(v->data.begin(), v->data.end(), cat.begin() + 2 * HH);
    std::copy(qb->data.begin(), qb->data.end(), bias.begin());
    std::copy(kb->data.begin(), kb->data.end(), bias.begin() + b.H);
    std::copy(vb->data.begin(), vb->data.end(), bias.begin() + 2 * b.H);
    b.qkv = pack_split(blob, L + "attention.query|key|value.weight", cat.data(), 3 * b.H, b.H, 1);
    b.qkv_b = blob.add_f32(bias);
  }
  b.dense = pk.conv_w(L + "attention.dense.weight", b.H, b.H, 1); b.dense_b = pk.vec(L + "attention.dense.bias", b.H);
  b.aln_w = pk.vec(L + "attention.LayerNorm.weight", b.H);        b.aln_b = pk.vec(L + "attention.LayerNorm.bias", b.H);
  b.ffn = pk.conv_w(L + "ffn.weight", -1, b.H, 1);
  b.I = b.ffn.C_out;
  b.ffn_b = pk.vec(L + "ffn.bias", b.I > 0 ? b.I : -1);
  b.out = pk.conv_w(L + "ffn_output.weight", b.H, b.I > 0 ? b.I : -1, 1); b.out_b = pk.vec(L + "ffn_output.bias", b.H);
  b.fln_w = pk.vec(L + "full_layer_layer_norm.weight", b.H);      b.fln_b = pk.vec(L + "full_layer_layer_norm.bias", b.H);
  if (pk.has("bert_encoder.weight")) {
    b.enc = pk.conv_w("bert_encoder.weight", -1, b.H, 1);
    b.enc_b = pk.vec("bert_encoder.bias", b.enc.C_out > 0 ? b.enc.C_out : -1);
    b.has_enc = true;
  }
  if (!pk.ok) { *err = "PL-BERT parameter missing or malformed: " + pk.missing; return 1; }
  b.ready = true;
  e.bert = b;
  return 0;
}

View bert_plan(Ctx& c, const st2_engine& e, const int64_t* tokens, const int32_t* lens, int B, int N) {
  const PBert& p = e.bert;
  const float eps = e.cfg.bert_ln_eps;
  const int H = p.H, heads = H / 64;
  Sess s{c, e, B, N, true, lens, {}, 0, nullptr, nullptr, 1.0};
  View X = dn_alloc(s, H), Xn = dn_alloc(s, H);
  {
    const int64_t mark = c.a.off;
    View E = dn_alloc(s, p.E);
    RUN(c, g_be.embed_tokens(tokens, B, N, e.F(p.word), p.V, p.E, e.F(p.tok0), e.F(p.pos), nullptr, E.p, E.bs, E.cs,
                             c.stream));
    float* st = c.a.f32((int64_t)B * N * 2);
    RUN(c, g_be.colnorm_stats(E.p, E.bs, E.cs, B, p.E, N, eps, st, c.stream));
    ConvOpt o;
    o.bias = e.F(p.map_b); o.pro = ST2_PRO_COLNORM; o.stats = st; o.gamma = e.F(p.eln_w); o.beta = e.F(p.eln_b);
    conv(c, e, dn_cv(s, E), p.map, dn_cv(s, X), o);
    c.a.off = mark;
  }
  for (int l = 0; l < e.cfg.bert_layers; ++l) {
    const int64_t mark = c.a.off;
    View qkv = dn_alloc(s, 3 * H);
    {
      ConvOpt o;
      o.bias = e.F(p.qkv_b);
      conv(c, e, dn_cv(s, X), p.qkv, dn_cv(s, qkv), o);
    }
    View ctx = dn_alloc(s, H);
    View q = qkv.rows(0, H), k = qkv.rows(H, 2 * H), v = qkv.rows(2 * H, 3 * H);
    RUN(c, g_be.attention_keylen(q.p, k.p, v.p, q.bs, q.cs, ctx.p, ctx.bs, ctx.cs, B, heads, 64, N, 0.125f, lens, c.stream));
    View Y = dn_alloc(s, H);
    {
      ConvOpt o;
      o.bias = e.F(p.dense_b); o.res = dn_cv(s, X);
      conv(c, e, dn_cv(s, ctx), p.dense, dn_cv(s, Y), o);
    }
    float* st1 = c.a.f32((int64_t)B * N * 2);
    RUN(c, g_be.colnorm_stats(Y.p, Y.bs, Y.cs, B, H, N, eps, st1, c.stream));
    View X1 = dn_alloc(s, H);
    RUN(c, g_be.colnorm_apply(Y.p, Y.bs, Y.cs, st1, e.F(p.aln_w), e.F(p.aln_b), 0, 0, ST2_ACT_NONE, 0.f, nullptr, X1.p, X1.bs,
                              X1.cs, B, H, N, c.stream));
    View Hm = dn_alloc(s, p.I);
    {
      ConvOpt o;
      o.bias = e.F(p.ffn_b); o.act = ST2_ACT_GELU_TANH;
      conv(c, e, dn_cv(s, X1), p.ffn, dn_cv(s, Hm), o);
    }
    View Z = dn_alloc(s, H);
    {
      ConvOpt o;
      o.bias = e.F(p.out_b); o.res = dn_cv(s, X1);
      conv(c, e, dn_cv(s, Hm), p.out, dn_cv(s, Z), o);
    }
    float* st2 = c.a.f32((int64_t)B * N * 2);
    RUN(c, g_be.colnorm_stats(Z.p, Z.bs, Z.cs, B, H, N, eps, st2, c.stream));
    RUN(c, g_be.colnorm_apply(Z.p, Z.bs, Z.cs, st2, e.F(p.fln_w), e.F(p.fln_b), 0, 0, ST2_ACT_NONE, 0.f, nullptr, Xn.p, Xn.bs,
                              Xn.cs, B, H, N, c.stream));
    std::swap(X, Xn);
    c.a.off = mark;
  }
  return X;
}

int front_plan(Ctx& c, const st2_engine& e, const st2_front_args& a) {
  const st2_model_config& cfg = e.cfg;
  const int B = a.B, N = a.N, sty = cfg.style_dim, C2 = cfg.dn_channels, dh = cfg.pred_hidden;
  text_plan(c, e, a.tokens, a.lengths, B, N, a.t_en);
  View X = bert_plan(c, e, a.tokens, a.lengths, B, N);
  Sess s0{c, e, B, N, true, a.lengths, {}, 0, nullptr, nullptr, 1.0};
  View D = dn_alloc(s0, dh);
  {
    ConvOpt o;
    o.bias = e.F(e.bert.enc_b);
    conv(c, e, dn_cv(s0, X), e.bert.enc, dn_cv(s0, D), o);
  }
  const int64_t n = (int64_t)B * C2;
  float* sp = c.a.f32(n);
  {
    const int64_t mark = c.a.off;
    if (sampler_plan(c, e, a.noise, nullptr, &X, a.ref_s, a.step_noise, a.lengths, B, N, a.steps, a.embedding_scale, a.table,
                     a.sigma0, sp, nullptr) != 0 && c.rc == 0)
      c.rc = 1;
    c.a.off = mark;
  }
  if (a.carry && B > 1) {
    float* mixed = a.s_pred_out ? a.s_pred_out : c.a.f32(n);
    float* m = c.a.f32(C2);
    float* ma = c.a.f32(C2);
    float* mb = c.a.f32(C2);
    for (int k = 0; k < B; ++k) {
      const float* prev = k ? mixed + (int64_t)(k - 1) * C2 : a.s_prev;
      const float* cur = sp + (int64_t)k * C2;
      if (prev) {
        RUN(c, g_be.axpbypcz(prev, (float)a.t, cur, (float)(1.0 - a.t), nullptr, 0.f, m, C2, c.stream));
        cur = m;
      }
      const float* ref_src = cur;
      const float* s_src = cur + sty;
      if (a.ref_s) {
        const float* rs = a.ref_s + (int64_t)k * C2;
        RUN(c, g_be.axpbypcz(cur, (float)a.alpha, rs, (float)(1.0 - a.alpha), nullptr, 0.f, ma, C2, c.stream));
        RUN(c, g_be.axpbypcz(cur, (float)a.beta, rs, (float)(1.0 - a.beta), nullptr, 0.f, mb, C2, c.stream));
        ref_src = ma;
        s_src = mb + sty;
      }
      RUN(c, g_be.copy_ncl(ref_src, C2, sty, mixed + (int64_t)k * C2, C2, sty, 1, 1, sty, c.stream));
      RUN(c, g_be.copy_ncl(s_src, C2, sty, mixed + (int64_t)k * C2 + sty, C2, sty, 1, 1, sty, c.stream));
    }
    RUN(c, g_be.copy_ncl(mixed, C2, sty, a.ref, sty, sty, B, 1, sty, c.stream));
    RUN(c, g_be.copy_ncl(mixed + sty, C2, sty, a.s, sty, sty, B, 1, sty, c.stream));
    duration_plan(c, e, D, a.s, a.lengths, B, N, a.tail, a.d_cm, a.durations);
    return c.rc;
  }
  const float* cur = sp;
  if (a.s_prev) {
    float* m = c.a.f32(n);
    RUN(c, g_be.axpbypcz(a.s_prev, (float)a.t, cur, (float)(1.0 - a.t), nullptr, 0.f, m, n, c.stream));
    cur = m;
  }
  const float* ref_src = cur;
  const float* s_src = cur + sty;
  if (a.ref_s) {
    float* ma = c.a.f32(n);
    float* mb = c.a.f32(n);
    RUN(c, g_be.axpbypcz(cur, (float)a.alpha, a.ref_s, (float)(1.0 - a.alpha), nullptr, 0.f, ma, n, c.stream));
    RUN(c, g_be.axpbypcz(cur, (float)a.beta, a.ref_s, (float)(1.0 - a.beta), nullptr, 0.f, mb, n, c.stream));
    ref_src = ma;
    s_src = mb + sty;
  }
  RUN(c, g_be.copy_ncl(ref_src, C2, sty, a.ref, sty, sty, B, 1, sty, c.stream));
  RUN(c, g_be.copy_ncl(s_src, C2, sty, a.s, sty, sty, B, 1, sty, c.stream));
  if (a.s_pred_out) {
    RUN(c, g_be.copy_ncl(ref_src, C2, sty, a.s_pred_out, C2, sty, B, 1, sty, c.stream));
    RUN(c, g_be.copy_ncl(s_src, C2, sty, a.s_pred_out + sty, C2, sty, B, 1, sty, c.stream));
  }
  duration_plan(c, e, D, a.s, a.lengths, B, N, a.tail, a.d_cm, a.durations);
  return c.rc;
}
```

styletts2_amd/csrc/st2_plan_sampler.inc:

```

struct Sess {
  Ctx& c;
  const st2_engine& e;
  int B, N;
  bool merged;
  const int32_t* key_len;
  View bases[2];
  int nbases;
  const float* feat_map;
  const float* ada;
  double scale;
};

View dn_alloc(Sess& s, int C) {
  View v;
  v.B = s.B; v.C = C; v.L = s.N;
  v.p = s.c.a.f32((int64_t)s.B * C * s.N);
  if (s.merged) { v.bs = s.N; v.cs = s.B * s.N; } else { v.bs = (int64_t)C * s.N; v.cs = s.N; }
  return v;
}
View dn_cv(const Sess& s, const View& t) {
  if (!s.merged) return t;
  View v = t;
  v.B = 1; v.L = s.B * s.N; v.bs = (int64_t)t.C * v.L; v.cs = v.L;
  return v;
}

const float* dn_mapping(Sess& s, float c_noise) {
  Ctx& c = s.c;
  const st2_engine& e = s.e;
  const PDenoiser& d = e.dn;
  const int F = d.features, H2 = e.cfg.dn_channels / 2;
  float* four = c.a.f32((int64_t)s.B * (1 + 2 * H2));
  RUN(c, g_be.time_features(c_noise, e.F(d.time_w), H2, s.B, four, c.stream));
  float* m = c.a.f32((int64_t)s.B * F);
  RUN(c, g_be.style_fc(four, s.B, 1 + 2 * H2, e.F(d.time_lin), e.F(d.time_b), F, ST2_ACT_GELU, m, c.stream));
  if (s.feat_map) {
    float* m2 = c.a.f32((int64_t)s.B * F);
    RUN(c, g_be.axpbypcz(m, 1.0f, s.feat_map, 1.0f, nullptr, 0.0f, m2, (int64_t)s.B * F, c.stream));
    m = m2;
  }
  float* m3 = c.a.f32((int64_t)s.B * F);
  RUN(c, g_be.style_fc(m, s.B, F, e.F(d.map0), e.F(d.map0_b), F, ST2_ACT_GELU, m3, c.stream));
  float* m4 = c.a.f32((int64_t)s.B * F);
  RUN(c, g_be.style_fc(m3, s.B, F, e.F(d.map2), e.F(d.map2_b), F, ST2_ACT_GELU, m4, c.stream));
  return m4;
}

void dn_run(Sess& s, View base, const float* x, const float* m, float* out) {
  Ctx& c = s.c;
  const st2_engine& e = s.e;
  const PDenoiser& d = e.dn;
  const st2_model_config& cfg = e.cfg;
  const int B = s.B, N = s.N, Fz = d.features, C = cfg.dn_channels;
  const int mid = cfg.dn_heads * cfg.dn_head_features;
  const int64_t mark = c.a.off;
  View b0 = base.rows(0, C);
  RUN(c, g_be.broadcast_cols(x, C, b0.p, b0.bs, b0.cs, B, C, N, c.stream));
  View X = dn_alloc(s, Fz);
  RUN(c, g_be.add_chanvec(base.p, base.bs, base.cs, m, Fz, X.p, X.bs, X.cs, B, Fz, N, c.stream));
  const int nblk = (int)d.blocks.size();
  for (int i = 0; i < nblk; ++i) {
    const PBlock& b = d.blocks[(size_t)i];
    float* st = c.a.f32((int64_t)B * N * 2);
    RUN(c, g_be.colnorm_stats(X.p, X.bs, X.cs, B, Fz, N, 1e-5f, st, c.stream));
    View qkv = dn_alloc(s, 3 * mid);
    ConvOpt o1, o2;
    o1.pro = o2.pro = ST2_PRO_COLNORM;
    o1.stats = o2.stats = st;
    if (cfg.multispeaker) {
      const int64_t J = (int64_t)nblk * 4 * Fz;
      const float* a = s.ada + (int64_t)4 * Fz * i;
      o1.gamma = a;          o1.beta = a + Fz;     o1.gb_bs = J; o1.gamma_plus_one = 1;
      o2.gamma = a + 2 * Fz; o2.beta = a + 3 * Fz; o2.gb_bs = J; o2.gamma_plus_one = 1;
    } else {
      o1.gamma = e.F(b.n_w);  o1.beta = e.F(b.n_b);
      o2.gamma = e.F(b.nc_w); o2.beta = e.F(b.nc_b);
    }
    const bool seg = cfg.multispeaker && s.merged && B > 1 && (int64_t)B * N >= XS_MIN_L && Fz > FUSED_K3_MAX_C;
    if (seg) o1.gb_seg = o2.gb_seg = N;
    const bool per_utt = cfg.multispeaker && !seg;
    View Xv = per_utt ? X : dn_cv(s, X), qv = per_utt ? qkv : dn_cv(s, qkv);
    conv(c, e, Xv, b.q, qv.rows(0, mid), o1);
    conv(c, e, Xv, b.kv, qv.rows(mid, 3 * mid), o2);
    View att = dn_alloc(s, mid);
    View q = qkv.rows(0, mid), k = qkv.rows(mid, 2 * mid), v = qkv.rows(2 * mid, 3 * mid);
    RUN(c, g_be.attention_keylen(q.p, k.p, v.p, q.bs, q.cs, att.p, att.bs, att.cs, B, cfg.dn_heads, cfg.dn_head_features,
                                 N, (float)pow((double)cfg.dn_head_features, -0.5), s.key_len, c.stream));
    View X1 = dn_alloc(s, Fz), hmid = dn_alloc(s, b.f1_out), X2 = dn_alloc(s, Fz);
    ConvOpt oo;
    oo.bias = e.F(b.o_b); oo.res = dn_cv(s, X);
    conv(c, e, dn_cv(s, att), b.o, dn_cv(s, X1), oo);
    ConvOpt of1;
    of1.bias = e.F(b.f1_b); of1.act = ST2_ACT_GELU;
    conv(c, e, dn_cv(s, X1), b.f1, dn_cv(s, hmid), of1);
    ConvOpt of2;
    of2.bias = e.F(b.f2_b); of2.res = dn_cv(s, X1);
    conv(c, e, dn_cv(s, hmid), b.f2, dn_cv(s, X2), of2);
    if (i + 1 < nblk) {
      View Xn = dn_alloc(s, Fz);
      RUN(c, g_be.add_chanvec(X2.p, X2.bs, X2.cs, m, Fz, Xn.p, Xn.bs, Xn.cs, B, Fz, N, c.stream));
      X = Xn;
    } else {
      X = X2;
    }
  }
  float* mean = c.a.f32((int64_t)B * Fz);
  RUN(c, g_be.mean_tokens_len(X.p, X.bs, X.cs, mean, Fz, B, Fz, N, s.key_len, c.stream));
  RUN(c, g_be.style_fc(mean, B, Fz, e.F(d.out_t), e.F(d.out_b), C, ST2_ACT_NONE, out, c.stream));
  c.a.off = mark;
}

void dn_denoise(Sess& s, const float* x, const double* w4, float* out) {
  Ctx& c = s.c;
  const int C = s.e.cfg.dn_channels;
  const int64_t n = (int64_t)s.B * C;
  const int64_t mark = c.a.off;
  const float c_skip = (float)w4[0], c_out = (float)w4[1], c_in = (float)w4[2], c_noise = (float)w4[3];
  float* x_in = c.a.f32(n);
  RUN(c, g_be.axpbypcz(x, c_in, nullptr, 0.f, nullptr, 0.f, x_in, n, c.stream));
  const float* m = dn_mapping(s, c_noise);
  float* pred = c.a.f32(n);
  dn_run(s, s.bases[0], x_in, m, pred);
  if (s.nbases > 1) {
    float* pm = c.a.f32(n);
    dn_run(s, s.bases[1], x_in, m, pm);
    float* mix = c.a.f32(n);
    RUN(c, g_be.axpbypcz(pm, (float)(1.0 - s.scale), pred, (float)s.scale, nullptr, 0.f, mix, n, c.stream));
    pred = mix;
  }
  RUN(c, g_be.axpbypcz(x, c_skip, pred, c_out, nullptr, 0.f, out, n, c.stream));
  c.a.off = mark;
}

int sampler_plan(Ctx& c, const st2_engine& e, const float* noise, const float* embedding, const View* emb_cm,
                 const float* features, const float* step_noise, const int32_t* lengths, int B, int N, int steps, double scale,
                 const double* table, double sigma0, float* out, float* step_taps) {
  const st2_model_config& cfg = e.cfg;
  const PDenoiser& d = e.dn;
  const int C = cfg.dn_channels, E = cfg.dn_embedding, Fz = d.features;
  Sess s{c, e, B, N, true, lengths, {}, 1, nullptr, nullptr, scale};
  s.bases[0] = dn_alloc(s, Fz);
  {
    View dst = s.bases[0].rows(C, Fz);
    if (emb_cm)
      RUN(c, g_be.copy_ncl(emb_cm->p, emb_cm->bs, emb_cm->cs, dst.p, dst.bs, dst.cs, B, E, N, c.stream));
    else
      RUN(c, g_be.tokens_to_channels(embedding, (int64_t)N * E, B, N, E, dst.p, dst.bs, dst.cs, c.stream));
  }
  if (scale != 1.0) {
    s.nbases = 2;
    s.bases[1] = dn_alloc(s, Fz);
    View dst = s.bases[1].rows(C, Fz);
    RUN(c, g_be.tokens_to_channels(e.F(d.fixed), 0, B, N, E, dst.p, dst.bs, dst.cs, c.stream));
  }
  if (cfg.multispeaker) {
    if (!features) { st2_set_error("st2_sampler_run: the multispeaker denoiser needs `features`"); return 1; }
    float* fm = c.a.f32((int64_t)B * Fz);
    RUN(c, g_be.style_fc(features, B, cfg.dn_context_features, e.F(d.feat), e.F(d.feat_b), Fz, ST2_ACT_GELU, fm, c.stream));
    const int J = cfg.dn_layers * 4 * Fz;
    float* ada = c.a.f32((int64_t)B * J);
    RUN(c, g_be.style_fc(features, B, cfg.dn_context_features, e.F(d.ada_wt), e.F(d.ada_b), J, ST2_ACT_NONE, ada, c.stream));
    s.feat_map = fm;
    s.ada = ada;
  }
  const int64_t n = (int64_t)B * C;
  float* xa = c.a.f32(n);
  float* xb = c.a.f32(n);
  float* x = xa;
  RUN(c, g_be.axpbypcz(noise, (float)sigma0, nullptr, 0.f, nullptr, 0.f, x, n, c.stream));
  for (int i = 0; i + 1 < steps; ++i) {
    const double* row = table + (int64_t)i * ST2_SAMPLER_TABLE_COLS;
    const int64_t mark = c.a.off;
    float* den = c.a.f32(n);
    dn_denoise(s, x, row + 0, den);
    const double k = row[8];
    float* x_mid = c.a.f32(n);
    RUN(c, g_be.axpbypcz(x, (float)(1.0 + k), den, (float)(-k), nullptr, 0.f, x_mid, n, c.stream));
    float* den_mid = c.a.f32(n);
    dn_denoise(s, x_mid, row + 4, den_mid);
    const double k2 = row[9];
    float* d_mid = c.a.f32(n);
    RUN(c, g_be.axpbypcz(x_mid, (float)k2, den_mid, (float)(-k2), nullptr, 0.f, d_mid, n, c.stream));
    float* xn = (x == xa) ? xb : xa;
    RUN(c, g_be.axpbypcz(x, 1.0f, d_mid, 1.0f, step_noise + (int64_t)i * n, (float)row[10], xn, n, c.stream));
    x = xn;
    if (step_taps) RUN(c, g_be.axpbypcz(x, 1.0f, nullptr, 0.f, nullptr, 0.f, step_taps + (int64_t)i * n, n, c.stream));
    c.a.off = mark;
  }
  RUN(c, g_be.axpbypcz(x, 1.0f, nullptr, 0.f, nullptr, 0.f, out, n, c.stream));
  return c.rc;
}
```

styletts2_amd/ops.py:

```python
import ctypes as C
import json
import warnings

import torch

from . import _hooks, _lib
from .weights import F16S_X_SCALE, SplitConvWeight
from ._lib import (ACT_EXP_SIN, ACT_GELU, ACT_GELU_TANH, ACT_LEAKY, ACT_NONE, ACT_TANH, PRO_ADAIN_LEAKY, PRO_ADAIN_SNAKE,
                   PRO_COLNORM, PRO_LEAKY, PRO_NONE, PRO_SNAKE, ConvDesc)


def _stream():
    return C.c_void_p(torch.cuda.current_stream().cuda_stream)


_AUX_STREAMS = {}


def aux_stream(dev, priority=0, index=0):
    dev = torch.device(dev)
    key = (dev.index if dev.index is not None else torch.cuda.current_device(), int(priority), int(index))
    if key not in _AUX_STREAMS:
        _AUX_STREAMS[key] = torch.cuda.Stream(dev, priority=int(priority))
    return _AUX_STREAMS[key]
# ... 69 lines not shown

_PRO_NORM = (PRO_ADAIN_LEAKY, PRO_ADAIN_SNAKE, PRO_COLNORM)
_PRO_SNAKE = (PRO_ADAIN_SNAKE, PRO_SNAKE)


def _chk_prologue(pro, B, Cc, L, stats, gamma, beta, alpha, gb_seg):
    gbs = 0
    if pro in _PRO_NORM:
        _chk(stats, "stats", 3)
        _chk(gamma, "gamma", 2)
        _chk(beta, "beta", 2)
        want = (B, L, 2) if pro == PRO_COLNORM else (B, Cc, 2)
        assert tuple(stats.shape) == want and stats.is_contiguous(), (stats.shape, want)
        assert gamma.shape[1] == Cc and beta.shape[1] == Cc
        gbs = gamma.stride(0) if gamma.shape[0] > 1 else 0
        bbs = beta.stride(0) if beta.shape[0] > 1 else 0
        if gb_seg:
            assert pro == PRO_COLNORM and B == 1 and gamma.shape[0] * gb_seg >= L and beta.shape[0] == gamma.shape[0]
            assert gbs == bbs
        else:
            assert gamma.shape[0] in (1, B) and beta.shape[0] == gamma.shape[0] and gbs == bbs
    if pro in _PRO_SNAKE:
        _chk(alpha, "alpha", 1)
        assert alpha.numel() == Cc and alpha.is_contiguous()
    return gbs


def _chk_split_weight(wt, C_in, C_out, ks):
    if (wt.C_in, wt.C_out, wt.ks) != (C_in, C_out, ks) or not wt.wq.is_cuda or not wt.wq.is_contiguous():
        raise _lib.St2Error("split weight is for (C_in=%d, C_out=%d, ks=%d) on %s, call has (%d, %d, %d)" % (
            wt.C_in, wt.C_out, wt.ks, wt.wq.device, C_in, C_out, ks))


def x_scale_for(pro):
    return F16S_X_SCALE if pro in _PRO_NORM else 1.0


def calibrated_x_scale(max_abs, margin_bits=3):
    return float(_lib.load().st2_calibration_scale(float(max_abs), int(margin_bits)))


def status(clear=False):
    return _lib.load().st2_status(1 if clear else 0)


lstm_recoveries = 0


def check_status(ignore=0):
    st = status(clear=True)
    if st > 0:
        st &= ~int(ignore)
    if st > 0 and st & _lib.STATUS_LSTM_RECOVERED:
        global lstm_recoveries
        lstm_recoveries += 1
        warnings.warn("a cooperative BiLSTM group was not co-resident in time; the call was re-run on the single-CU kernel "
                      "in-stream (results valid; ST2_STATUS_LSTM_RECOVERED)", RuntimeWarning, stacklevel=2)
        st &= ~_lib.STATUS_LSTM_RECOVERED
    if st <= 0:
        return
    msgs = []
    if st & _lib.STATUS_F16_RANGE:
        msgs.append("a split-f16 conv operand exceeded the f16 range (|x * x_scale| > 65504) and was clamped: the "
                    "result is finite but wrong; calibrate the operand scales for this checkpoint (pipeline.calibrate / st2_calibrate) and "
                    "check it with tools/validate_checkpoint.py, which names the conv site and its headroom")
    if st & _lib.STATUS_LSTM_TIMEOUT:
        msgs.append("a cooperative BiLSTM group timed out (its workgroups were not co-resident in time) on a launch without "
                    "the recovery pass: outputs of that call are invalid")
    if st & _lib.STATUS_DURATION_SUM:
        msgs.append("a row of the supplied durations does not sum to the frame count given with it (`total_frames`): the "
                    "alignment of that call repeated its last phoneme")
    raise _lib.St2Error("device-side status 0x%x: %s" % (st, "; ".join(msgs)))


class conv_autotune:

    def __init__(self, reset=False):
        self.reset = reset

    def __enter__(self):
        lib = _lib.load()
        if self.reset:
            _lib.check(lib.st2_conv_tune(-1), "st2_conv_tune")
        _lib.check(lib.st2_conv_tune(1), "st2_conv_tune")
        return self

    def __exit__(self, *exc):
        torch.cuda.synchronize()
        _lib.check(_lib.load().st2_conv_tune(0), "st2_conv_tune")
        return False


TUNE_VARIANT_BITS = {1: "128x256 tiles, 2 wg/CU", 2: "XCD-aware tile order"}


def tune_variant_name(v):
    if v < 0:
        return "rule"
    names = [n for b, n in TUNE_VARIANT_BITS.items() if v & b]
    return " + ".join(names) if names else "128x128 tiles, 3 wg/CU, dispatch order"


def conv_tune_table():
    lib = _lib.load()
    n = lib.st2_conv_tune_read(None, 0)
    rows = (C.c_double * (24 * max(n, 1)))()
    n = min(n, lib.st2_conv_tune_read(rows, n))
    out = []
    for i in range(n):
        r = rows[24 * i:24 * i + 24]
        cands = [{"variant": int(r[8 + 2 * j]), "name": tune_variant_name(int(r[8 + 2 * j])), "ms": round(r[9 + 2 * j], 5)}
                 for j in range(int(r[7]))]
        out.append({"ks": int(r[0]), "C_in": int(r[1]), "C_out": int(r[2]), "L": int(r[3]), "B": int(r[4]),
                    "chosen": int(r[6]), "chosen_name": tune_variant_name(int(r[6])), "candidates": cands})
    return out


def conv_tune_set(ks, C_in, C_out, L_out, B, variant):
    _lib.check(_lib.load().st2_conv_tune_set(ks, C_in, C_out, L_out, B, variant), "st2_conv_tune_set")


def probe_cu_health():
    buf = C.create_string_buffer(16384)
    mask = (C.c_uint32 * 16)()
    n = C.c_int32(0)
    _lib.check(_lib.load().st2_probe_cu_health(buf, len(buf), mask, 16, C.byref(n)), "st2_probe_cu_health")
    rep = json.loads(buf.value.decode())
    words = (rep["cus"] + 31) // 32
    return rep, [int(mask[i]) for i in range(words)], int(n.value)


class headroom:

    def __enter__(self):
        _lib.check(_lib.load().st2_debug_headroom(1), "st2_debug_headroom")
        self.rows = []
        return self

    def __exit__(self, *exc):
        lib = _lib.load()
        torch.cuda.synchronize()
        _lib.check(lib.st2_debug_headroom(0), "st2_debug_headroom")
        n = lib.st2_debug_headroom_read(None, 0)
        W = _lib.HEADROOM_COLS
        buf = (C.c_double * (W * max(n, 1)))()
        n = min(n, lib.st2_debug_headroom_read(buf, n))
        pro_names = ["none", "leaky", "adain+leaky", "adain+snake", "snake", "layernorm"]
        for i in range(max(n, 0)):
            r = buf[W * i:W * i + W]
            self.rows.append({"index": i, "kind": "fused conv" if int(r[0]) else "act_split", "pro": pro_names[int(r[1])],
                              "B": int(r[2]), "C": int(r[3]), "L": int(r[4]), "x_scale": r[5], "max_abs": r[6], "frac": r[7],
                              "rel_err": r[8], "sub_share": r[9], "site": int(r[10]), "engine": int(r[11])})
        return False


def probe_box(level=0):
    buf = C.create_string_buffer(16384)
    _lib.check(_lib.load().st2_probe_box(buf, len(buf), level), "st2_probe_box")
    return json.loads(buf.value.decode())


XS_HALO = 32
FUSED_MAX_C, FUSED_K3_MAX_C = 64, 128
XS_MIN_L = 256
XS_MIN_C_PLAIN = 64


def prefer_fused(pro, C_in, ks):
    return pro != PRO_NONE and (C_in <= FUSED_MAX_C or (ks <= 3 and C_in <= FUSED_K3_MAX_C))


def conv_path():
    return _hooks.conv_path


class XsTensor:

    def __init__(self, data, C, L, halo, x_scale=F16S_X_SCALE):
        self.data, self.C, self.L, self.halo, self.x_scale = data, C, L, halo, x_scale

    @property
    def cg(self):
        return self.data.shape[2]

    @property
    def Lp(self):
        return self.data.shape[3]


def xs_row_slots(L):
    return XS_HALO + (max(L, 1) + 1 + 511) // 512 * 512 + 96


def activate(x, *, pro=PRO_NONE, slope=0.0, stats=None, gamma=None, beta=None, gamma_plus_one=False, alpha=None,
              c_pad=32, gb_seg=0, x_scale=None, lengths=None):
    lp = _chk_len(lengths, "lengths", _nb(x), x)
    if lengths is not None and pro == PRO_COLNORM:
        raise _lib.St2Error("activate: per-row lengths are not defined for PRO_COLNORM (st2_act_split_len)")
    lib = _lib.load()
    _chk(x, "x", 3)
    B, Cc, L = x.shape
    cg = (Cc + c_pad - 1) // c_pad * c_pad // 8
    Lp = xs_row_slots(L)
    data = torch.empty((B, 2, cg, Lp, 8), device=x.device, dtype=torch.float16)
    gbs = _chk_prologue(pro, B, Cc, L, stats, gamma, beta, alpha, gb_seg)
    xsc = float(x_scale) if x_scale else x_scale_for(pro)
    _lib.check(lib.st2_act_split_len(x.data_ptr(), x.stride(0), x.stride(1), B, Cc, L, pro, slope, _ptr(stats),
                                     _ptr(gamma), _ptr(beta), gbs, int(gb_seg), 1 if gamma_plus_one else 0, _ptr(alpha),
                                     xsc, data.data_ptr(), cg, Lp, XS_HALO, lp, _stream()), "st2_act_split_len")
    return XsTensor(data, Cc, L, XS_HALO, xsc)


def new_part(B, C, nt, device):
    return torch.empty((B * C * nt * 3,), device=device, dtype=torch.float32)


def stats_finalize(part, B, C, nt, L, cols=128, eps=1e-5, out=None, lengths=None, len_div=1):
    if lengths is None:
        len_div = 1
    elif len_div <= 0 or (B * C) % len_div:
        raise _lib.St2Error("stats_finalize: len_div=%d does not divide the %d rows" % (len_div, B * C))
    lp = _chk_len(lengths, "lengths", B * C // len_div, part)
    lib = _lib.load()
    assert part.numel() >= B * C * nt * 3 and part.is_contiguous()
    if out is None:
        out = torch.empty((B, C, 2), device=part.device, dtype=torch.float32)
    _lib.check(lib.st2_stats_finalize_len(part.data_ptr(), B * C, nt, L, eps, out.data_ptr(), int(cols), lp, int(len_div),
                                          _stream()), "st2_stats_finalize_len")
    return out


def conv1d_xs(xs, wt, C_out, ks, *, dil=1, pad_left=0, L_out=None, bias=None, out=None, res=None, res_shift=0,
              res2=None, div=1.0, act=ACT_NONE, act_split=0, act_slope=0.0, want_stats=False, part_cols=None, y_len=None):
    if y_len is not None:
        _chk_len(y_len, "y_len", xs.data.shape[0] if isinstance(xs, XsTensor) else -1, xs.data if isinstance(xs, XsTensor) else None)
    lib = _lib.load()
    assert isinstance(xs, XsTensor) and isinstance(wt, SplitConvWeight)
    B, C_in, L_in = xs.data.shape[0], xs.C, xs.L
    _chk_split_weight(wt, C_in, C_out, ks)
    if L_out is None:
        L_out = L_in
    if out is None:
        out = torch.empty((B, C_out, L_out), device=xs.data.device, dtype=torch.float32)
    _chk(out, "out", 3)
    assert out.shape == (B, C_out, L_out), (out.shape, (B, C_out, L_out))
    d = ConvDesc()
    d.B, d.C_in, d.C_out, d.L_in, d.L_out, d.ks, d.dil, d.pad_left = B, C_in, C_out, L_in, L_out, ks, dil, pad_left
    d.xs, d.xs_cg, d.xs_lp, d.xs_halo = xs.data.data_ptr(), xs.cg, xs.Lp, xs.halo
    d.wq, d.wq_co_pad, d.wq_cin_pad = wt.wq.data_ptr(), wt.co_pad, wt.cin_pad
    d.x_scale, d.out_scale, d.w_row_scale = xs.x_scale, 1.0 / xs.x_scale, wt.row_scale.data_ptr()
    _chk(bias, "bias", 1)
    d.bias = _ptr(bias)
    d.y, d.y_bs, d.y_cs = out.data_ptr(), out.stride(0), out.stride(1)
    d.y_len = _ptr(y_len)
    _fill_epilogue(d, B, C_out, L_out, res, res_shift, res2, div, act, act_split, act_slope)
    part = None
    if want_stats:
        pc = part_cols or lib.st2_conv1d_xs_part_cols(C.byref(d))
        nt = (L_out + pc - 1) // pc
        part = new_part(B, C_out, nt, out.device)
        d.part, d.part_nt, d.part_cols = part.data_ptr(), nt, pc
    _launch_conv(lib.st2_conv1d_xs, "st2_conv1d_xs", d)
    if want_stats:
        return out, stats_finalize(part, B, C_out, nt, L_out, cols=d.part_cols or 128, lengths=y_len, len_div=C_out)
    return out


def _fill_epilogue(d, B, C_out, L_out, res, res_shift, res2, div, act, act_split, act_slope):
    if res is not None:
        _chk(res, "res", 3)
        assert res.shape[0] == B and res.shape[1] == C_out and res.shape[2] == (L_out + (1 << res_shift) - 1 >> res_shift)
        d.res, d.res_bs, d.res_cs, d.res_shift = res.data_ptr(), res.stride(0), res.stride(1), res_shift
    if res2 is not None:
        _chk(res2, "res2", 3)
        assert res2.shape == (B, C_out, L_out)
        d.res2, d.res2_bs, d.res2_cs = res2.data_ptr(), res2.stride(0), res2.stride(1)
    d.div = div
    d.act, d.act_split, d.act_slope = act, act_split, act_slope


def _launch_conv(fn, fname, d):
    _lib.check(fn(C.byref(d), _stream()), fname)


def conv1d(x, wt, C_out, ks, *, dil=1, pad_left=0, L_out=None, bias=None, out=None,
           pro=PRO_NONE, slope=0.0, stats=None, gamma=None, beta=None, gamma_plus_one=False, alpha=None,
           res=None, res_shift=0, res2=None, div=1.0, act=ACT_NONE, act_split=0, act_slope=0.0, want_stats=False,
           gb_seg=0, x_scale=None, x_len=None, y_len=None):
    _chk_len(x_len, "x_len", _nb(x), x)
    _chk_len(y_len, "y_len", _nb(x), x)
    lib = _lib.load()
    _chk(x, "x", 3)
    B, C_in, L_in = x.shape
    split = isinstance(wt, SplitConvWeight)
    if (split and pad_left <= XS_HALO and L_in >= XS_MIN_L and (pro != PRO_NONE or C_in >= XS_MIN_C_PLAIN)
            and conv_path() == "xs" and not prefer_fused(pro, C_in, ks)):
        xs = activate(x, pro=pro, slope=slope, stats=stats, gamma=gamma, beta=beta,
                      gamma_plus_one=gamma_plus_one, alpha=alpha, gb_seg=gb_seg, x_scale=x_scale, lengths=x_len)
        return conv1d_xs(xs, wt, C_out, ks, dil=dil, pad_left=pad_left, L_out=L_out, bias=bias, out=out, res=res,
                         res_shift=res_shift, res2=res2, div=div, act=act, act_split=act_split, act_slope=act_slope,
                         want_stats=want_stats, y_len=y_len)
    if gb_seg:
        raise _lib.St2Error("gb_seg (per-segment affine of a token-merged view) exists on the st2_act_split + "
                            "st2_conv1d_xs path only; this call routes to the fused kernel")
    if split:
        _chk_split_weight(wt, C_in, C_out, ks)
# ... 503 lines not shown
```

Before: 5088.

## Write f16 hi/lo conv input planes directly from attention and layernorm producers

Attention and the BERT layernorm-apply kernels now emit the split f16 hi/lo input planes consumed by the following 1x1 convs, so those convs skip their own act_split pass and the attention output no longer needs an fp32 round trip. The change covers BERT qkv, dense, ffn and encoder projections and the sampler attention output projection in merged mode. Workspace sizing takes the peak over both routes, and a mismatch check guards the conv geometry. It adds plane-padding zeroing inside the attention kernel and a dual write in the layernorm path, plus more coupling between producers and consumers.

```diff
diff --git a/include/st2.h b/include/st2.h
--- a/include/st2.h
+++ b/include/st2.h
@@ -344,6 +344,8 @@
 int st2_debug_headroom(int enable);
 int st2_debug_headroom_read(double* rows, int32_t cap_rows);
 
+int st2_debug_producer_planes(int enable);
+
 #define ST2_CALIBRATION_COLS 5
 int st2_calibrate(st2_engine* e, int32_t margin_bits, int32_t* n_clamped);
 int st2_calibration_read(st2_engine* e, double* rows, int32_t cap_rows);
diff --git a/styletts2_amd/_lib.py b/styletts2_amd/_lib.py
--- a/styletts2_amd/_lib.py
+++ b/styletts2_amd/_lib.py
@@ -236,6 +236,7 @@
     "st2_probe_cu_health": (C.c_int, [C.c_char_p, C.c_int32, C.POINTER(C.c_uint32), C.c_int32, C.POINTER(C.c_int32)]),
     "st2_probe_mfma_stream": (C.c_int, [C.c_int32, C.c_int32, C.c_int32, C.c_void_p]),
     "st2_debug_headroom": (C.c_int, [C.c_int]),
+    "st2_debug_producer_planes": (C.c_int, [C.c_int]),
     "st2_debug_headroom_read": (C.c_int, [C.POINTER(C.c_double), C.c_int32]),
     "st2_conv1d_xs_part_cols": (C.c_int, [C.POINTER(ConvDesc)]),
     "st2_conv1d_f16s_set_splitk": (None, [C.c_int, C.c_int]),
diff --git a/styletts2_amd/csrc/st2_actsplit.hip b/styletts2_amd/csrc/st2_actsplit.hip
--- a/styletts2_amd/csrc/st2_actsplit.hip
+++ b/styletts2_amd/csrc/st2_actsplit.hip
@@ -17,12 +17,13 @@
   st2_h8* xs; int xs_cg, Lp, halo;
   const int32_t* len;
   int* status;
+  float* y; int64_t y_bs; int y_cs;
 };
 
 #ifndef ST2_ACT_NT
 #define ST2_ACT_NT 3
 #endif
-template <int PRO>
+template <int PRO, bool SIDE = false>
 __global__ __launch_bounds__(256) void act_split_kernel(const ActArgs a) {
   const int pos = blockIdx.x * 256 + threadIdx.x;
   if (pos >= a.Lp) return;
@@ -80,6 +81,9 @@
       const float bt = a.beta[row * a.gb_bs + cc];
       const float w = (u - cmean) * crstd;
       u = w * g + bt;
+      if constexpr (SIDE) {
+        if (lok && ci < a.C) a.y[(int64_t)b * a.y_bs + (int64_t)ci * a.y_cs + l] = u;
+      }
     }
     u = (lok && ci < a.C) ? u * a.x_scale : 0.f;
     const float uc = st2_clamp_f16(u);
@@ -192,7 +196,7 @@
 thread_local int t_site = -1;
 
 void headroom_record(int kind, const ActArgs& a, int B, hipStream_t s) {
-  if ((int)g_hr.size() >= HR_CAP || !g_hr_dev) return;
+  if (!g_headroom || (int)g_hr.size() >= HR_CAP || !g_hr_dev) return;
   hipStreamCaptureStatus cs = hipStreamCaptureStatusNone;
   if (hipStreamIsCapturing(s, &cs) != hipSuccess || cs != hipStreamCaptureStatusNone) {
     (void)hipGetLastError();
@@ -240,6 +244,7 @@
   a.alpha = alpha; a.x_scale = x_scale;
   a.xs = reinterpret_cast<st2_h8*>(xs); a.xs_cg = xs_cg; a.Lp = Lp; a.halo = halo;
   a.len = len;
+  a.y = nullptr; a.y_bs = 0; a.y_cs = 0;
   ST2_REQUIRE(!len || pro != ST2_PRO_COLNORM, "st2_act_split_len: per-row lengths are not defined for ST2_PRO_COLNORM");
   a.status = st2_status_device_ptr();
   hipStream_t s = reinterpret_cast<hipStream_t>(stream);
@@ -257,6 +262,39 @@
     if (!g_hr.empty()) g_hr.back().pro = pro;
   }
   return 0;
+}
+
+int st2_act_split_side(const float* x, int64_t x_bs, int32_t x_cs, int32_t B, int32_t C, int32_t L, const float* stats,
+                       const float* gamma, const float* beta, float x_scale, void* xs, int32_t xs_cg, int32_t Lp, int32_t halo,
+                       float* y, int64_t y_bs, int32_t y_cs, void* stream) {
+  ST2_REQUIRE(x && xs && y && stats && gamma && beta && B > 0 && C > 0 && L > 0, "st2_act_split_side: bad arguments");
+  ST2_REQUIRE(B <= 65535 && xs_cg <= 65535 && xs_cg * 8 >= C, "st2_act_split_side: bad plane geometry");
+  ST2_REQUIRE(halo >= 0 && Lp >= L + halo, "st2_act_split_side: Lp=%d too small for L=%d + halo=%d", Lp, L, halo);
+  ST2_REQUIRE((reinterpret_cast<uintptr_t>(xs) & 15) == 0 && x_scale > 0.f, "st2_act_split_side: xs alignment / x_scale");
+  ActArgs a;
+  a.x = x; a.x_bs = x_bs; a.x_cs = x_cs; a.C = C; a.L = L; a.slope = 0.f;
+  a.stats = stats; a.gamma = gamma; a.beta = beta; a.gb_bs = 0; a.gb_seg = 0; a.gamma_plus_one = 0;
+  a.alpha = nullptr; a.x_scale = x_scale;
+  a.xs = reinterpret_cast<st2_h8*>(xs); a.xs_cg = xs_cg; a.Lp = Lp; a.halo = halo;
+  a.len = nullptr;
+  a.status = st2_status_device_ptr();
+  a.y = y; a.y_bs = y_bs; a.y_cs = y_cs;
+  hipLaunchKernelGGL((act_split_kernel<ST2_PRO_COLNORM, true>), dim3(st2_cdiv(Lp, 256), xs_cg, B), dim3(256), 0,
+                     reinterpret_cast<hipStream_t>(stream), a);
+  ST2_CHECK_LAUNCH("st2_act_split_side");
+  return 0;
+}
+
+void st2_headroom_probe_planes(const void* xs, int32_t xs_cg, int32_t Lp, int32_t B, int32_t C, int32_t L, float x_scale,
+                               void* stream) {
+  if (!g_headroom) return;
+  ActArgs a;
+  memset(&a, 0, sizeof(a));
+  a.C = C; a.L = L; a.x_scale = x_scale;
+  a.xs = reinterpret_cast<st2_h8*>(const_cast<void*>(xs)); a.xs_cg = xs_cg; a.Lp = Lp;
+  const size_t before = g_hr.size();
+  headroom_record(0, a, B, reinterpret_cast<hipStream_t>(stream));
+  if (g_hr.size() == before + 1) g_hr.back().pro = ST2_PRO_NONE;
 }
 
 int st2_headroom_of_fused_conv(const st2_conv_desc& d, hipStream_t s) {
diff --git a/styletts2_amd/csrc/st2_attention.hip b/styletts2_amd/csrc/st2_attention.hip
--- a/styletts2_amd/csrc/st2_attention.hip
+++ b/styletts2_amd/csrc/st2_attention.hip
@@ -1,4 +1,5 @@
 #include "st2_common.h"
+#include "st2_act.h"
 
 typedef float f32x16 __attribute__((ext_vector_type(16)));
 
@@ -9,10 +10,18 @@
 constexpr int ALD = AKT + 1;
 constexpr int AQB = 128;
 
+struct AttPlanes {
+  st2_h8* xs; int xs_cg, Lp, halo;
+  float x_scale;
+  int* status;
+};
+typedef _Float16 st2_h4 __attribute__((ext_vector_type(4)));
+
+template <bool PLANES>
 __global__ __launch_bounds__(256) void attention_kernel(const float* __restrict__ q, const float* __restrict__ k,
                                                         const float* __restrict__ v, int64_t bs, int cs,
                                                         float* __restrict__ o, int64_t o_bs, int o_cs, int N,
-                                                        float scale, const int* __restrict__ key_len) {
+                                                        float scale, const int* __restrict__ key_len, const AttPlanes pl) {
   extern __shared__ __attribute__((aligned(16))) float att_smem[];
   float* ks = att_smem;
   float* vs = att_smem + AD * ALD;
@@ -28,6 +37,23 @@
   const int nq = q0 + l31;
   const bool wave_live = q0 < N;
   const int NK = key_len ? max(1, min(key_len[b], N)) : N;
+  if constexpr (PLANES) {
+    if (blockIdx.x == 0 && b == 0) {
+      const int used = pl.halo + (int)gridDim.z * N;
+      const int npad = pl.halo + (pl.Lp - used);
+      const int64_t plane = (int64_t)pl.xs_cg * pl.Lp;
+      st2_h8 z;
+#pragma unroll
+      for (int e = 0; e < 8; ++e) z[e] = (_Float16)0.0f;
+      for (int i = tid; i < 8 * npad; i += 256) {
+        const int g = i / npad, pp = i % npad;
+        const int pos = pp < pl.halo ? pp : used + (pp - pl.halo);
+        st2_h8* dst = pl.xs + (int64_t)(h * (AD / 8) + g) * pl.Lp + pos;
+        dst[0] = z;
+        dst[plane] = z;
+      }
+    }
+  }
 
   float qr[AD / 2];
 #pragma unroll
@@ -111,16 +137,44 @@
   }
   if (!wave_live) return;
   den += __shfl_xor(den, 32, 64);
+  bool sat = false;
   if (nq < N) {
     const float inv = 1.0f / den;
     const int64_t ob = (int64_t)b * o_bs + (int64_t)h * AD * o_cs;
-#pragma unroll
-    for (int t = 0; t < 2; ++t)
-#pragma unroll
-      for (int r = 0; r < 16; ++r) {
-        const int d = t * 32 + (r & 3) + 8 * (r >> 2) + 4 * half;
-        o[ob + (int64_t)d * o_cs + nq] = oacc[t][r] * inv;
-      }
+    if (!PLANES || o) {
+#pragma unroll
+      for (int t = 0; t < 2; ++t)
+#pragma unroll
+        for (int r = 0; r < 16; ++r) {
+          const int d = t * 32 + (r & 3) + 8 * (r >> 2) + 4 * half;
+          o[ob + (int64_t)d * o_cs + nq] = oacc[t][r] * inv;
+        }
+    }
+    if constexpr (PLANES) {
+      const int64_t plane = (int64_t)pl.xs_cg * pl.Lp;
+      const int pos = pl.halo + b * N + nq;
+#pragma unroll
+      for (int t = 0; t < 2; ++t)
+#pragma unroll
+        for (int g = 0; g < 4; ++g) {
+          st2_h4 hi, lo;
+#pragma unroll
+          for (int e = 0; e < 4; ++e) {
+            const float u = (oacc[t][4 * g + e] * inv) * pl.x_scale;
+            const float uc = st2_clamp_f16(u);
+            sat |= uc != u;
+            const _Float16 hh = (_Float16)uc;
+            hi[e] = hh;
+            lo[e] = (_Float16)(uc - (float)hh);
+          }
+          st2_h4* dst = reinterpret_cast<st2_h4*>(pl.xs + (int64_t)(h * (AD / 8) + t * 4 + g) * pl.Lp + pos) + half;
+          dst[0] = hi;
+          dst[2 * plane] = lo;
+        }
+    }
+  }
+  if constexpr (PLANES) {
+    if (__any(sat) && lane == 0) st2_raise_status(pl.status, ST2_STATUS_F16_RANGE);
   }
 }
 
@@ -130,6 +184,25 @@
                              int64_t o_bs, int32_t o_cs, int32_t B, int32_t H, int32_t D, int32_t N, float scale,
                              void* stream) {
   return st2_attention_keylen(q, k, v, bs, cs, o, o_bs, o_cs, B, H, D, N, scale, nullptr, stream);
+}
+
+namespace {
+template <bool PLANES>
+int launch_attention(const float* q, const float* k, const float* v, int64_t bs, int32_t cs, float* o, int64_t o_bs,
+                     int32_t o_cs, int32_t B, int32_t H, int32_t N, float scale, const int32_t* key_len, const AttPlanes& pl,
+                     void* stream) {
+  hipStream_t s = reinterpret_cast<hipStream_t>(stream);
+  constexpr size_t smem = (size_t)2 * AD * ALD * sizeof(float);
+  static std::atomic<uint64_t> attr_done{0};
+  st2_once_per_device(attr_done, [&] {
+    (void)hipFuncSetAttribute(reinterpret_cast<const void*>(&attention_kernel<PLANES>),
+                              hipFuncAttributeMaxDynamicSharedMemorySize, (int)smem);
+  });
+  hipLaunchKernelGGL((attention_kernel<PLANES>), dim3(st2_cdiv(N, AQB), H, B), dim3(256), smem, s, q, k, v, bs, cs, o, o_bs,
+                     o_cs, N, scale, reinterpret_cast<const int*>(key_len), pl);
+  ST2_CHECK_LAUNCH("st2_attention");
+  return 0;
+}
 }
 
 extern "C" int st2_attention_keylen(const float* q, const float* k, const float* v, int64_t bs, int32_t cs, float* o,
@@ -138,15 +211,21 @@
   ST2_REQUIRE(q && k && v && o && B > 0 && H > 0 && N > 0, "st2_attention: bad arguments");
   ST2_REQUIRE(D == AD, "st2_attention: head_features=%d unsupported (built for %d)", D, AD);
   ST2_REQUIRE(B <= 65535 && H <= 65535, "st2_attention: grid too large");
-  hipStream_t s = reinterpret_cast<hipStream_t>(stream);
-  constexpr size_t smem = (size_t)2 * AD * ALD * sizeof(float);
-  static std::atomic<uint64_t> attr_done{0};
-  st2_once_per_device(attr_done, [&] {
-    (void)hipFuncSetAttribute(reinterpret_cast<const void*>(&attention_kernel),
-                              hipFuncAttributeMaxDynamicSharedMemorySize, (int)smem);
-  });
-  hipLaunchKernelGGL(attention_kernel, dim3(st2_cdiv(N, AQB), H, B), dim3(256), smem, s, q, k, v, bs, cs, o, o_bs,
-                     o_cs, N, scale, reinterpret_cast<const int*>(key_len));
-  ST2_CHECK_LAUNCH("st2_attention");
-  return 0;
-}
+  return launch_attention<false>(q, k, v, bs, cs, o, o_bs, o_cs, B, H, N, scale, key_len, AttPlanes{}, stream);
+}
+
+int st2_attention_planes(const float* q, const float* k, const float* v, int64_t bs, int32_t cs, float* o, int64_t o_bs,
+                         int32_t o_cs, int32_t B, int32_t H, int32_t D, int32_t N, float scale, const int32_t* key_len,
+                         float x_scale, void* xs, int32_t xs_cg, int32_t Lp, int32_t halo, void* stream) {
+  ST2_REQUIRE(q && k && v && xs && B > 0 && H > 0 && N > 0, "st2_attention_planes: bad arguments");
+  ST2_REQUIRE(D == AD, "st2_attention_planes: head_features=%d unsupported (built for %d)", D, AD);
+  ST2_REQUIRE(B <= 65535 && H <= 65535, "st2_attention_planes: grid too large");
+  ST2_REQUIRE(xs_cg == H * (AD / 8) && halo >= 0 && (int64_t)halo + (int64_t)B * N <= Lp,
+              "st2_attention_planes: planes of %d groups x %d slots cannot hold %d channels x (%d + %d x %d) columns", xs_cg, Lp,
+              H * AD, halo, B, N);
+  ST2_REQUIRE((reinterpret_cast<uintptr_t>(xs) & 15) == 0 && x_scale > 0.f, "st2_attention_planes: xs alignment / x_scale");
+  AttPlanes pl;
+  pl.xs = reinterpret_cast<st2_h8*>(xs); pl.xs_cg = xs_cg; pl.Lp = Lp; pl.halo = halo; pl.x_scale = x_scale;
+  pl.status = st2_status_device_ptr();
+  return launch_attention<true>(q, k, v, bs, cs, o, o_bs, o_cs, B, H, N, scale, key_len, pl, stream);
+}
diff --git a/styletts2_amd/csrc/st2_common.h b/styletts2_amd/csrc/st2_common.h
--- a/styletts2_amd/csrc/st2_common.h
+++ b/styletts2_amd/csrc/st2_common.h
@@ -7,6 +7,14 @@
 void st2_set_error(const char* fmt, ...);
 int st2_stream_cu_count(void* stream);
 void st2_headroom_set_site(const void* engine, int site);
+int st2_act_split_side(const float* x, int64_t x_bs, int32_t x_cs, int32_t B, int32_t C, int32_t L, const float* stats,
+                       const float* gamma, const float* beta, float x_scale, void* xs, int32_t xs_cg, int32_t Lp, int32_t halo,
+                       float* y, int64_t y_bs, int32_t y_cs, void* stream);
+void st2_headroom_probe_planes(const void* xs, int32_t xs_cg, int32_t Lp, int32_t B, int32_t C, int32_t L, float x_scale,
+                               void* stream);
+int st2_attention_planes(const float* q, const float* k, const float* v, int64_t bs, int32_t cs, float* o, int64_t o_bs,
+                         int32_t o_cs, int32_t B, int32_t H, int32_t D, int32_t N, float scale, const int32_t* key_len,
+                         float x_scale, void* xs, int32_t xs_cg, int32_t Lp, int32_t halo, void* stream);
 int* st2_status_device_ptr();
 
 __device__ __forceinline__ void st2_raise_status(int* status, int bit) {
diff --git a/styletts2_amd/csrc/st2_engine.hip b/styletts2_amd/csrc/st2_engine.hip
--- a/styletts2_amd/csrc/st2_engine.hip
+++ b/styletts2_amd/csrc/st2_engine.hip
@@ -95,6 +95,8 @@
                              st2_adain_leaky_pool_len, st2_convt_interleave_stats_len, st2_har_source_len,
                              st2_stft_mag_phase_len, st2_istft_len, st2_ragged_lengths, st2_expand_by_durations_len};
 Backend g_be = kHipBackend;
+bool g_be_native = true;
+bool g_producer_planes = true;
 
 constexpr int XS_HALO = 32;
 constexpr int FUSED_MAX_C = 64, FUSED_K3_MAX_C = 128;
@@ -145,7 +147,22 @@
   void* stream = nullptr;
   int rc = 0;
   bool dry = false;
-};
+  bool planes = g_be_native && g_producer_planes;
+};
+
+template <class F>
+int64_t dry_peak(F&& plan) {
+  int64_t peak = 0;
+  for (int route = 0; route < 2; ++route) {
+    Ctx c;
+    c.dry = true;
+    c.a.dry = true;
+    c.planes = route != 0;
+    plan(c);
+    peak = std::max(peak, c.a.peak);
+  }
+  return peak;
+}
 
 View new_ncl(Ctx& c, int B, int C, int L, bool padded = true) {
   View v;
@@ -718,6 +735,12 @@
   return 0;
 }
 
+struct XsPlanes {
+  void* xs = nullptr;
+  int cg = 0, Lp = 0, C = 0, L = 0;
+  float scale = 0.f;
+};
+
 struct ConvOpt {
   int dil = 1, pad_left = 0;
   const float* bias = nullptr;
@@ -736,6 +759,7 @@
   int act = ST2_ACT_NONE, act_split = 0;
   float act_slope = 0.f;
   float* stats_out = nullptr;
+  const XsPlanes* planes = nullptr;
 };
 
 float x_scale_for(int pro) {
@@ -755,6 +779,17 @@
     RUN(c, g_be.instnorm_stats_len(x.p, x.bs, x.cs, x.B, x.C, x.L, 1e-5f, stats, x.len, c.stream));
   else
     RUN(c, g_be.instnorm_stats(x.p, x.bs, x.cs, x.B, x.C, x.L, 1e-5f, stats, c.stream));
+}
+
+XsPlanes producer_planes(Ctx& c, const st2_engine& e, const SplitW& w, int C, int L) {
+  XsPlanes p;
+  if (!c.planes || w.ks != 1 || L < XS_MIN_L || C < XS_MIN_C_PLAIN) return p;
+  p.cg = (C + 31) / 32 * 32 / 8;
+  p.Lp = xs_row_slots(L);
+  p.C = C; p.L = L;
+  p.scale = e.x_scale(w.site, x_scale_for(ST2_PRO_NONE));
+  p.xs = c.a.alloc((int64_t)2 * p.cg * p.Lp * 16);
+  return p;
 }
 
 void conv(Ctx& c, const st2_engine& e, const View& x, const SplitW& w, const View& y, const ConvOpt& o) {
@@ -781,11 +816,23 @@
   const bool use_xs = o.pad_left <= XS_HALO && x.L >= XS_MIN_L && (o.pro != ST2_PRO_NONE || x.C >= XS_MIN_C_PLAIN) &&
                       !prefer_fused;
   const int64_t mark = c.a.off;
+  const bool given = o.planes && o.planes->xs;
+  if (given) {
+    const XsPlanes& p = *o.planes;
+    const bool fits = use_xs && o.pro == ST2_PRO_NONE && x.B == 1 && !x.len && w.ks == 1 && p.C == x.C && p.L == x.L &&
+                      p.cg == (x.C + 31) / 32 * 32 / 8 && p.Lp == xs_row_slots(x.L) && p.scale == d.x_scale;
+    if (!fits) {
+      if (c.rc == 0) { st2_set_error("engine: producer-written planes do not match the conv that consumes them"); c.rc = 1; }
+      return;
+    }
+  }
   if (use_xs) {
     const int cg = (x.C + 31) / 32 * 32 / 8;
     const int Lp = xs_row_slots(x.L);
-    void* xs = c.a.alloc((int64_t)x.B * 2 * cg * Lp * 16);
-    if (x.len)
+    void* xs = given ? o.planes->xs : c.a.alloc((int64_t)x.B * 2 * cg * Lp * 16);
+    if (given) {
+      if (!c.dry && c.rc == 0) st2_headroom_probe_planes(xs, cg, Lp, x.B, x.C, x.L, d.x_scale, c.stream);
+    } else if (x.len)
       RUN(c, g_be.act_split_len(x.p, x.bs, x.cs, x.B, x.C, x.L, o.pro, o.slope, o.stats, o.gamma, o.beta, o.gb_bs, o.gb_seg,
                                 o.gamma_plus_one, o.alpha, d.x_scale, xs, cg, Lp, XS_HALO, x.len, c.stream));
     else
@@ -848,6 +895,7 @@
 extern "C" int st2_debug_set_backend(void* const* table, int32_t entries) {
   if (!table) {
     g_be = kHipBackend;
+    g_be_native = true;
     return 0;
   }
   ST2_REQUIRE(entries == ST2_BACKEND_ENTRIES || entries == ST2_BACKEND_ENTRIES_V22,
@@ -884,6 +932,12 @@
     SLOT(ragged_lengths, ST2_BE_RAGGED_LENGTHS); SLOT(expand_by_durations_len, ST2_BE_EXPAND_BY_DURATIONS_LEN);
   }
 #undef SLOT
+  g_be_native = false;
+  return 0;
+}
+
+extern "C" int st2_debug_producer_planes(int enable) {
+  g_producer_planes = enable != 0;
   return 0;
 }
 
@@ -1155,11 +1209,7 @@
 
 extern "C" int64_t st2_bert_workspace_bytes(st2_engine* e, int32_t B, int32_t N) {
   if (!e || !e->bert.ready || B <= 0 || N <= 0) return -1;
-  Ctx c;
-  c.dry = true;
-  c.a.dry = true;
-  bert_plan(c, *e, nullptr, nullptr, B, N);
-  return c.a.peak + 256;
+  return dry_peak([&](Ctx& c) { bert_plan(c, *e, nullptr, nullptr, B, N); }) + 256;
 }
 
 extern "C" int st2_bert_forward(st2_engine* e, const int64_t* tokens, const int32_t* lengths, int32_t B, int32_t N,
@@ -1224,9 +1274,6 @@
 
 extern "C" int64_t st2_front_workspace_bytes(st2_engine* e, const st2_front_args* a) {
   if (front_ready(e) || !a || a->B <= 0 || a->N <= 0 || a->steps < 2) return -1;
-  Ctx c;
-  c.dry = true;
-  c.a.dry = true;
   std::vector<double> table((size_t)(a->steps - 1) * ST2_SAMPLER_TABLE_COLS, 0.0);
   static const float dummy = 0.f;
   static int64_t dummy_dur;
@@ -1234,8 +1281,7 @@
   q.table = table.data();
   if (e->cfg.multispeaker) q.ref_s = &dummy;
   if (a->durations) q.durations = &dummy_dur;
-  front_plan(c, *e, q);
-  return c.a.peak + 256;
+  return dry_peak([&](Ctx& c) { front_plan(c, *e, q); }) + 256;
 }
 
 extern "C" int st2_front_forward(st2_engine* e, const st2_front_args* a, void* workspace, int64_t workspace_bytes,
@@ -1368,14 +1414,12 @@
 
 extern "C" int64_t st2_sampler_workspace_bytes(st2_engine* e, int32_t B, int32_t N, int32_t steps, double embedding_scale) {
   if (!e || !e->dn.ready || B <= 0 || N <= 0 || steps < 2) return -1;
-  Ctx c;
-  c.dry = true;
-  c.a.dry = true;
   std::vector<double> table((size_t)(steps - 1) * ST2_SAMPLER_TABLE_COLS, 0.0);
   static const float dummy = 0.f;
-  sampler_plan(c, *e, nullptr, nullptr, nullptr, &dummy, nullptr, nullptr, B, N, steps, embedding_scale, table.data(), 1.0, nullptr,
-               nullptr);
-  return c.a.peak + 256;
+  return dry_peak([&](Ctx& c) {
+    sampler_plan(c, *e, nullptr, nullptr, nullptr, &dummy, nullptr, nullptr, B, N, steps, embedding_scale, table.data(), 1.0,
+                 nullptr, nullptr);
+  }) + 256;
 }
 
 extern "C" int st2_sampler_run(st2_engine* e, const float* noise, const float* embedding, const float* features,
diff --git a/styletts2_amd/csrc/st2_plan_front.inc b/styletts2_amd/csrc/st2_plan_front.inc
--- a/styletts2_amd/csrc/st2_plan_front.inc
+++ b/styletts2_amd/csrc/st2_plan_front.inc
@@ -59,12 +59,30 @@
   return 0;
 }
 
-View bert_plan(Ctx& c, const st2_engine& e, const int64_t* tokens, const int32_t* lens, int B, int N) {
+void bert_norm(Ctx& c, const Sess& s, const View& y, const float* st, const float* g, const float* bt, const View& x,
+               const XsPlanes& pl) {
+  if (pl.xs) {
+    const View ym = dn_cv(s, y), xm = dn_cv(s, x);
+    RUN(c, st2_act_split_side(ym.p, ym.bs, ym.cs, 1, ym.C, ym.L, st, g, bt, pl.scale, pl.xs, pl.cg, pl.Lp, XS_HALO, xm.p, xm.bs,
+                              xm.cs, c.stream));
+  } else {
+    RUN(c, g_be.colnorm_apply(y.p, y.bs, y.cs, st, g, bt, 0, 0, ST2_ACT_NONE, 0.f, nullptr, x.p, x.bs, x.cs, s.B, y.C, s.N,
+                              c.stream));
+  }
+}
+
+View bert_plan(Ctx& c, const st2_engine& e, const int64_t* tokens, const int32_t* lens, int B, int N,
+               const SplitW* tail_w = nullptr, XsPlanes* tail_pl = nullptr) {
   const PBert& p = e.bert;
   const float eps = e.cfg.bert_ln_eps;
   const int H = p.H, heads = H / 64;
+  const int layers = e.cfg.bert_layers;
   Sess s{c, e, B, N, true, lens, {}, 0, nullptr, nullptr, 1.0};
   View X = dn_alloc(s, H), Xn = dn_alloc(s, H);
+  XsPlanes xpl, xpl_next, tpl;
+  if (layers > 1) xpl_next = producer_planes(c, e, p.qkv, H, B * N);
+  if (tail_w) tpl = producer_planes(c, e, *tail_w, H, B * N);
+  if (tail_pl) *tail_pl = tpl;
   {
     const int64_t mark = c.a.off;
     View E = dn_alloc(s, p.E);
@@ -77,32 +95,40 @@
     conv(c, e, dn_cv(s, E), p.map, dn_cv(s, X), o);
     c.a.off = mark;
   }
-  for (int l = 0; l < e.cfg.bert_layers; ++l) {
+  for (int l = 0; l < layers; ++l) {
     const int64_t mark = c.a.off;
     View qkv = dn_alloc(s, 3 * H);
     {
       ConvOpt o;
-      o.bias = e.F(p.qkv_b);
+      o.bias = e.F(p.qkv_b); o.planes = &xpl;
       conv(c, e, dn_cv(s, X), p.qkv, dn_cv(s, qkv), o);
     }
-    View ctx = dn_alloc(s, H);
+    const XsPlanes cpl = producer_planes(c, e, p.dense, H, B * N);
+    View ctx;
     View q = qkv.rows(0, H), k = qkv.rows(H, 2 * H), v = qkv.rows(2 * H, 3 * H);
-    RUN(c, g_be.attention_keylen(q.p, k.p, v.p, q.bs, q.cs, ctx.p, ctx.bs, ctx.cs, B, heads, 64, N, 0.125f, lens, c.stream));
+    if (cpl.xs) {
+      ctx = q;
+      RUN(c, st2_attention_planes(q.p, k.p, v.p, q.bs, q.cs, nullptr, 0, 0, B, heads, 64, N, 0.125f, lens, cpl.scale, cpl.xs,
+                                  cpl.cg, cpl.Lp, XS_HALO, c.stream));
+    } else {
+      ctx = dn_alloc(s, H);
+      RUN(c, g_be.attention_keylen(q.p, k.p, v.p, q.bs, q.cs, ctx.p, ctx.bs, ctx.cs, B, heads, 64, N, 0.125f, lens, c.stream));
+    }
     View Y = dn_alloc(s, H);
     {
       ConvOpt o;
-      o.bias = e.F(p.dense_b); o.res = dn_cv(s, X);
+      o.bias = e.F(p.dense_b); o.res = dn_cv(s, X); o.planes = &cpl;
       conv(c, e, dn_cv(s, ctx), p.dense, dn_cv(s, Y), o);
     }
     float* st1 = c.a.f32((int64_t)B * N * 2);
     RUN(c, g_be.colnorm_stats(Y.p, Y.bs, Y.cs, B, H, N, eps, st1, c.stream));
     View X1 = dn_alloc(s, H);
-    RUN(c, g_be.colnorm_apply(Y.p, Y.bs, Y.cs, st1, e.F(p.aln_w), e.F(p.aln_b), 0, 0, ST2_ACT_NONE, 0.f, nullptr, X1.p, X1.bs,
-                              X1.cs, B, H, N, c.stream));
+    const XsPlanes fpl = producer_planes(c, e, p.ffn, H, B * N);
+    bert_norm(c, s, Y, st1, e.F(p.aln_w), e.F(p.aln_b), X1, fpl);
     View Hm = dn_alloc(s, p.I);
     {
       ConvOpt o;
-      o.bias = e.F(p.ffn_b); o.act = ST2_ACT_GELU_TANH;
+      o.bias = e.F(p.ffn_b); o.act = ST2_ACT_GELU_TANH; o.planes = &fpl;
       conv(c, e, dn_cv(s, X1), p.ffn, dn_cv(s, Hm), o);
     }
     View Z = dn_alloc(s, H);
@@ -113,8 +139,8 @@
     }
     float* st2 = c.a.f32((int64_t)B * N * 2);
     RUN(c, g_be.colnorm_stats(Z.p, Z.bs, Z.cs, B, H, N, eps, st2, c.stream));
-    RUN(c, g_be.colnorm_apply(Z.p, Z.bs, Z.cs, st2, e.F(p.fln_w), e.F(p.fln_b), 0, 0, ST2_ACT_NONE, 0.f, nullptr, Xn.p, Xn.bs,
-                              Xn.cs, B, H, N, c.stream));
+    xpl = l + 1 < layers ? xpl_next : tpl;
+    bert_norm(c, s, Z, st2, e.F(p.fln_w), e.F(p.fln_b), Xn, xpl);
     std::swap(X, Xn);
     c.a.off = mark;
   }
@@ -125,12 +151,13 @@
   const st2_model_config& cfg = e.cfg;
   const int B = a.B, N = a.N, sty = cfg.style_dim, C2 = cfg.dn_channels, dh = cfg.pred_hidden;
   text_plan(c, e, a.tokens, a.lengths, B, N, a.t_en);
-  View X = bert_plan(c, e, a.tokens, a.lengths, B, N);
+  XsPlanes epl;
+  View X = bert_plan(c, e, a.tokens, a.lengths, B, N, &e.bert.enc, &epl);
   Sess s0{c, e, B, N, true, a.lengths, {}, 0, nullptr, nullptr, 1.0};
   View D = dn_alloc(s0, dh);
   {
     ConvOpt o;
-    o.bias = e.F(e.bert.enc_b);
+    o.bias = e.F(e.bert.enc_b); o.planes = &epl;
     conv(c, e, dn_cv(s0, X), e.bert.enc, dn_cv(s0, D), o);
   }
   const int64_t n = (int64_t)B * C2;
diff --git a/styletts2_amd/csrc/st2_plan_sampler.inc b/styletts2_amd/csrc/st2_plan_sampler.inc
--- a/styletts2_amd/csrc/st2_plan_sampler.inc
+++ b/styletts2_amd/csrc/st2_plan_sampler.inc
@@ -83,13 +83,22 @@
     View Xv = per_utt ? X : dn_cv(s, X), qv = per_utt ? qkv : dn_cv(s, qkv);
     conv(c, e, Xv, b.q, qv.rows(0, mid), o1);
     conv(c, e, Xv, b.kv, qv.rows(mid, 3 * mid), o2);
-    View att = dn_alloc(s, mid);
     View q = qkv.rows(0, mid), k = qkv.rows(mid, 2 * mid), v = qkv.rows(2 * mid, 3 * mid);
-    RUN(c, g_be.attention_keylen(q.p, k.p, v.p, q.bs, q.cs, att.p, att.bs, att.cs, B, cfg.dn_heads, cfg.dn_head_features,
-                                 N, (float)pow((double)cfg.dn_head_features, -0.5), s.key_len, c.stream));
+    const float att_scale = (float)pow((double)cfg.dn_head_features, -0.5);
+    const XsPlanes apl = s.merged ? producer_planes(c, e, b.o, mid, B * N) : XsPlanes();
+    View att;
+    if (apl.xs) {
+      att = q;
+      RUN(c, st2_attention_planes(q.p, k.p, v.p, q.bs, q.cs, nullptr, 0, 0, B, cfg.dn_heads, cfg.dn_head_features, N,
+                                  att_scale, s.key_len, apl.scale, apl.xs, apl.cg, apl.Lp, XS_HALO, c.stream));
+    } else {
+      att = dn_alloc(s, mid);
+      RUN(c, g_be.attention_keylen(q.p, k.p, v.p, q.bs, q.cs, att.p, att.bs, att.cs, B, cfg.dn_heads, cfg.dn_head_features,
+                                   N, att_scale, s.key_len, c.stream));
+    }
     View X1 = dn_alloc(s, Fz), hmid = dn_alloc(s, b.f1_out), X2 = dn_alloc(s, Fz);
     ConvOpt oo;
-    oo.bias = e.F(b.o_b); oo.res = dn_cv(s, X);
+    oo.bias = e.F(b.o_b); oo.res = dn_cv(s, X); oo.planes = &apl;
     conv(c, e, dn_cv(s, att), b.o, dn_cv(s, X1), oo);
     ConvOpt of1;
     of1.bias = e.F(b.f1_b); of1.act = ST2_ACT_GELU;
diff --git a/styletts2_amd/ops.py b/styletts2_amd/ops.py
--- a/styletts2_amd/ops.py
+++ b/styletts2_amd/ops.py
@@ -245,6 +245,10 @@
                               "B": int(r[2]), "C": int(r[3]), "L": int(r[4]), "x_scale": r[5], "max_abs": r[6], "frac": r[7],
                               "rel_err": r[8], "sub_share": r[9], "site": int(r[10]), "engine": int(r[11])})
         return False
+
+
+def producer_planes(enable):
+    _lib.check(_lib.load().st2_debug_producer_planes(1 if enable else 0), "st2_debug_producer_planes")
 
 
 def probe_box(level=0):
```

Result: no change. 5099 (median of 6 runs) (+0.2%).
